# sailordiary/m3f.pytorch

Measured on AMD Instinct MI355X. Metric: clips/sec (300-frame A+V, fwd+bwd), higher is better.
Workload: dtype f32 (fp32-accurate products, fp32 accumulate: GEMMs as fp16x3 -- two fp16 terms per scaled operand, three MFMAs, error vs fp64 no larger than an fp32 GEMM's; the forward and backward recurrences at H=512 and H=256 as fp16x3 too (h is bounded; the backward producers split their values under a power-o

## Files before the change

### include/m3t_hip.h

```cpp
#ifndef M3T_HIP_H
#define M3T_HIP_H

#include <stddef.h>
#include <stdint.h>

#ifdef __cplusplus
extern "C" {
#endif

#define M3T_EINVAL 10001
#define M3T_MAX_SCANS 8
#define M3T_ESPIN 10002
#define M3T_SCAN_NO_PERSIST 1
#define M3T_SCAN_WHH 8
#define M3T_SCAN_FP32 4
#define M3T_SCAN_FAULT 16
#define M3T_SCAN_WIDE 32
#define M3T_BF16 2
#define M3T_GEMM_BACKGROUND 1
#define M3T_GEMM_BF16 2
#define M3T_GEMM_HIGH 256
#define M3T_GEMM_F16X3 1024
#define M3T_GEMM_BESIDE_SCAN 512
#define M3T_GEMM_EXCLUSIVE 8
#define M3T_CONV_IMAGES 4096

int m3t_im2col3d(const float* x, int N, int Ci, int T, int H, int W, int kt, int kh, int kw, int st, int sh, int sw,
                 int pt, int ph, int pw, float* out, long long rows_pad, int Kp, unsigned long long* amax_slot, void* stream);

int m3t_conv3d_taps(const float* src, const float* w_taps, float* dst, int N, int C_src, int C_dst, int T, int H, int W,
                    int To, int Ho, int Wo, int kt, int kh, int kw, int base_t, int base_h, int base_w, int sign, int flags,
                    const unsigned long long* amax_src, const unsigned long long* amax_w, float* ws, size_t ws_bytes, float* dst_planes,
                    void* stream);

int m3t_f16x3_split(const float* x, size_t rows, int cols, size_t ld, float* out, size_t ldo, const unsigned long long* slot, void* stream);
int m3t_f16x3_split_perm(const float* w, size_t R, int T, int Cc, size_t sR, size_t sT, size_t sC, float* out, const unsigned long long* slot,
                         void* stream);
int m3t_sgemm_pre(int M, int N, int K, const float* A_img, int lda, const float* B_img, int ldb, float* C, int ldc,
                  const float* bias, int act, int accumulate, const unsigned long long* amax_a, const unsigned long long* amax_b, void* stream);
int m3t_f16x3_image_b(const float* w, int N, int K, size_t ld, float* img, const unsigned long long* slot, void* stream);
int m3t_sgemm_bimg(int M, int N, int K, const float* A, int lda, const float* B_img, float* C, int ldc, const float* bias, int act,
                   int accumulate, float* ws, size_t ws_bytes, const unsigned long long* amax_a, const unsigned long long* amax_b, void* stream);
int m3t_sgemm_ring(int transA, int transB, int M, int N, int K, const float* A, int lda, const float* B, int ldb, float* C, int ldc,
                   const float* bias, int act, int accumulate, int seg_len, int seg_stride, int a_off, int b_off, float* ws, size_t ws_bytes,
                   int splits, const unsigned long long* amax_a, const unsigned long long* amax_b, int variant, void* stream);
int m3t_conv3d_taps_pre(const float* src_img, const float* w_img, float* dst, int N, int C_src, int C_dst, int T, int H, int W,
                        int To, int Ho, int Wo, int kt, int kh, int kw, int base_t, int base_h, int base_w, int sign,
                        const unsigned long long* amax_src, const unsigned long long* amax_w, float* ws, size_t ws_bytes, float* dst_planes,
                    void* stream);

int m3t_planes_to_cl4(const float* x, float* out, int N, int C, long long S, void* stream);
int m3t_conv3d_fwd_taps4(const float* x_img4, const float* w_img, const float* bias, float* y_cl, int N, int Co, int T, int H, int W,
                         int kt, int kh, int kw, int st, int sh, int sw, int pt, int ph, int pw, const unsigned long long* amax_x,
                         const unsigned long long* amax_w, float* ws, size_t ws_bytes, float* y_planes, void* stream);
int m3t_conv3d_fwd_taps(const float* x_img, const float* w_img, const float* bias, float* y_cl, int N, int Ci, int Co, int T, int H, int W,
                        int kt, int kh, int kw, int st, int sh, int sw, int pt, int ph, int pw, const unsigned long long* amax_x,
                        const unsigned long long* amax_w, float* ws, size_t ws_bytes, float* y_planes, void* stream);
int m3t_conv3d_wgrad_taps(const float* x_cl, const float* dy_cl, float* dwt, int N, int Ci, int Co, int T, int H, int W, int kt, int kh, int kw,
                          int st, int sh, int sw, int pt, int ph, int pw, int flags, const unsigned long long* amax_x,
                          const unsigned long long* amax_dy, float* ws, size_t ws_bytes, void* stream);

int m3t_amax_out(unsigned long long* slot);

int m3t_version(void);
int m3t_device_arch(char* arch, int cap);

int m3t_sgemm(int transA, int transB, int M, int N, int K,
              const float* A, int lda, const float* B, int ldb,
              float* C, int ldc, const float* bias, int act, int accumulate,
              int seg_len, int seg_stride, int a_off, int b_off,
              float* ws, size_t ws_bytes, int flags, void* stream);

int m3t_sgemm_scaled(int transA, int transB, int M, int N, int K,
                     const float* A, int lda, const float* B, int ldb,
                     float* C, int ldc, const float* bias, int act, int accumulate,
                     int seg_len, int seg_stride, int a_off, int b_off,
                     float* ws, size_t ws_bytes, int flags,
                     const unsigned long long* amax_a, const unsigned long long* amax_b, void* stream);

int m3t_sgemm_window(int transB, int n_seg, int win_len, int win_stride, int win_off, int N, int K,
                     const float* A, int lda, const float* B, int ldb, float* C, int ldc, const float* bias,
                     int act, int accumulate, int flags, const unsigned long long* amax_a, const unsigned long long* amax_b, void* stream);
#define M3T_WINDOW_BATCH 8
typedef struct {
    const float* A; const float* B; float* C; const float* bias;
    const unsigned long long* amax_a; const unsigned long long* amax_b;
    int accumulate;
} m3t_window_problem;
int m3t_sgemm_window_batch(int n, const m3t_window_problem* problems, int transB, int n_seg, int win_len, int win_stride, int win_off,
                           int N, int K, int lda, int ldb, int ldc, int act, int flags, void* stream);

int m3t_absmax(int n, const float* const* x, const size_t* rows, const int* cols, const size_t* ld,
               unsigned long long* const* slots, void* stream);

int m3t_sgemm_plan(int transA, int M, int N, int K, int seg_len, size_t ws_bytes, int flags, int* kernel, int* splits);

int m3t_colsum(const float* X, int M, int N, int ld, float* out, int accumulate,
               float* ws, size_t ws_bytes, void* stream);

int m3t_transpose(const float* src, int R, int C, int lds, float* dst, int ldd, void* stream);

int m3t_relu_bwd(const float* a, float* dy, size_t n, void* stream);

typedef struct {
    const float* xproj;
    const float* w_hh;
    const float* b_hh;
    float* out;
    float* gates;
    float* h_n;
    int H, reverse, ldx, xoff, ldo, ooff;
} m3t_gru_fwd_desc;

int m3t_gru_scan_fwd(const m3t_gru_fwd_desc* scans, int n_scans, int B, int T,
                     float* ws, size_t ws_bytes, int flags, void* stream);

typedef struct {
    const float* dout;
    const float* out;
    const float* gates;
    const float* w_hh_t;
    const float* dh_n;
    float* dgx;
    float* dgh;
    float* dh;
    float* db_part;
    float* db_ih;
    float* db_hh;
    int H, reverse, ldo, ooff, ldg, goff;
    unsigned long long* amax;
    const float* wfrag;
} m3t_gru_bwd_desc;

size_t m3t_gru_bwd_prepare_floats(int H);
int m3t_gru_bwd_prepare(const float* const* w, int n, int H, int whh_direct, float* const* out, void* stream);

int m3t_gru_scan_workgroups(int n_scans, int H, int B, int T, int flags, int backward);
int m3t_gru_persist_count(void);
int m3t_gru_poll_error(void);
int m3t_gru_error_reset(void);
int m3t_gru_error_defer(int on);
int m3t_gru_inject_error(void* stream);
int m3t_gru_persist_owner(void);
int m3t_gru_scan_arena(void* arena, size_t bytes);
int m3t_gru_scan_arena_reset(void* arena);
int m3t_gru_scan_progress(unsigned* counters, int n_marks, const int* time_bounds, unsigned* need);
int m3t_gru_scan_progress_reset(unsigned* counters);
int m3t_gru_scan_progress_ok(int n_scans, int H, int B, int T, int flags, int backward);
int m3t_stream_wait_progress(const unsigned* counter, unsigned need, void* stream);
int m3t_gru_scan_after(void* event);
int m3t_gru_scan_events(void* start, void* end);
int m3t_gru_persist_profile(unsigned long long* out6);

int m3t_gru_scan_bwd(const m3t_gru_bwd_desc* scans, int n_scans, int B, int T,
                     float* ws, size_t ws_bytes, int flags, void* stream);

int m3t_att_fuse_fwd(const float* s_v, const float* s_a, const float* x_v, const float* x_a,
                     float* f, int rows, int D, void* stream);
int m3t_att_fuse_bwd(const float* df, const float* s_v, const float* s_a,
                     const float* x_v, const float* x_a,
                     float* ds_v, float* ds_a, float* dx_v, float* dx_a,
                     int rows, int D, void* stream);

int m3t_va_loss(const float* y_hat, int rows, int C, int iv, int ia,
                const float* valence, const float* arousal,
                const int64_t* class_expr, const uint8_t* expr_valid, int n_expr,
                float w_v, float w_a, float expr_w, int use_mse,
                float* out_scalars, float* dy, float* ws, size_t ws_bytes, void* stream);
size_t m3t_va_loss_ws_bytes(int rows);

// ... 295 lines not shown
```

### m3f.pytorch_amd/csrc/gru_persist.hip

```cpp
#include "gru_common.h"
#include <cstdio>
#include <cstdlib>
#include <cstring>
#include <mutex>
#include <unordered_map>
#include <fcntl.h>
#include <sys/file.h>
#include <sys/stat.h>
#include <unistd.h>

namespace m3t_gru {

namespace {

constexpr int SPIN_LIMIT_DEFAULT = 1 << 21;
typedef unsigned u32x4 __attribute__((ext_vector_type(4)));

struct ExPtrs {
    void* gran[M3T_MAX_SCANS];
    size_t slot[M3T_MAX_SCANS];
    int poll_fixed;
    int poll_align;
    int spin_limit;
    int fault_step;
// ... 97 lines not shown
    constexpr int ROWS = 16 * RT;
    constexpr int NB = RT == 1 ? 2 : 1;
    constexpr int H = 128 * NC, nch = H >> 4;
    __shared__ float red[NB][NW][3][ROWS][UB + 1];
    const int tid = threadIdx.x, lane = tid & 63, wave = tid >> 6;
    int gid, ub;
    if (!persist_map((int)blockIdx.x, G, ex.slot_map, gid, ub)) return;
    const int s = gid / nrb, rb = gid % nrb;
    const m3t_gru_fwd_desc d = g.d[s];
    const int j0 = ub * UB, r0 = rb * ROWS;

    float4 wf[NC][3];
    {
        const float4* Wf = reinterpret_cast<const float4*>(fp.wfrag[s] + (size_t)ub * nch * 3 * 256);
#pragma unroll
        for (int m = 0; m < NC; ++m)
#pragma unroll
            for (int ct = 0; ct < 3; ++ct) wf[m][ct] = Wf[((size_t)(wave + m * NW) * 3 + ct) * 64 + lane];
    }
    const bool pw = tid < ROWS * UB;
    const int prow = (tid >> 8) * 16 + (tid & 15), pu = ((tid >> 4) & 3) * 4 + ((tid >> 6) & 3);
    const int pb = r0 + prow, pj = j0 + pu;
    const bool pok = pw && pb < B;
    float br = 0.f, bz = 0.f, bn = 0.f, hprev = 0.f;
    if (pw) { br = d.b_hh[pj]; bz = d.b_hh[H + pj]; bn = d.b_hh[2 * H + pj]; }

    constexpr size_t TILE = (size_t)RT * 256;
    unsigned long long* gran = reinterpret_cast<unsigned long long*>(ex.gran[s]);
    const size_t slot = ex.slot[s];
    const size_t grp = (size_t)rb * nch * TILE;
    const size_t pub = grp + (size_t)ub * TILE + tid;
    bool dead = false;
    int poll_delay = ex.poll_fixed >= 0 ? ex.poll_fixed : POLL_DELAY_INIT;
    __shared__ unsigned poll_fail[2];
    __shared__ int pub_step;
    const int l2mode = persist_handshake(ex, gid, ub, H >> 4, tid, err);
    if (tid == 0) pub_step = 0;
    if (tid < 2) poll_fail[tid] = 0;
    const bool stamp = ex.prof != nullptr && blockIdx.x == 0 && tid == ex.prof_tid;
    long long psum[6] = {0, 0, 0, 0, 0, 0}, last = stamp ? clock64() : 0;

    float xrA, xzA, xnA, xrB, xzB, xnB;
    const float* xq = d.xproj + (size_t)(pb < B ? pb : B - 1) * T * d.ldx + d.xoff + pj;
#define M3T_FWD_LOAD_X(step_, XR, XZ, XN)                                                                             \
    do {                                                                                                               \
        const int ls_ = (step_) < T ? (step_) : T - 1;                                                                 \
        const float* xa_ = xq + (size_t)(d.reverse ? T - 1 - ls_ : ls_) * d.ldx;                                       \
        asm volatile("global_load_dword %0, %3, off\n\t"                                                               \
                     "global_load_dword %1, %4, off\n\t"                                                               \
                     "global_load_dword %2, %5, off"                                                                   \
                     : "=&v"(XR), "=&v"(XZ), "=&v"(XN) : "v"(xa_), "v"(xa_ + H), "v"(xa_ + 2 * H) : "memory");         \
    } while (0)
    M3T_FWD_LOAD_X(0, xrA, xzA, xnA);
    asm volatile("s_waitcnt vmcnt(0)" : "+v"(xrA), "+v"(xzA), "+v"(xnA) :: "memory");
    __builtin_amdgcn_s_waitcnt(0x0F70);

    for (int step2 = 0; step2 < T; step2 += 2) {
#define STEPV step2
#define CUR(x) x##A
#define NXT(x) x##B
#include "gru_persist_fwd_step.inc"
#undef STEPV
#undef CUR
#undef NXT
        if (step2 + 1 >= T) break;
#define STEPV (step2 + 1)
#define CUR(x) x##B
#define NXT(x) x##A
#include "gru_persist_fwd_step.inc"
#undef STEPV
#undef CUR
#undef NXT
    }
#undef M3T_FWD_LOAD_X
    asm volatile("s_waitcnt vmcnt(0)" ::: "memory");
    if (stamp)
        for (int i = 0; i < 6; ++i) ex.prof[i] = (unsigned long long)psum[i];
}

typedef __bf16 pbf16x8 __attribute__((ext_vector_type(8)));
typedef unsigned pu32x4 __attribute__((ext_vector_type(4)));

__global__ void wfrag6_prep_kernel(const float* __restrict__ w_hh, unsigned short* __restrict__ wf, int H, int bf16) {
    const int nch = H >> 4, ks = nch >> 4;
    const size_t total = (size_t)3 * H * H;
    for (size_t i = blockIdx.x * (size_t)blockDim.x + threadIdx.x; i < total; i += (size_t)gridDim.x * blockDim.x) {
        const int e = i & 7, l = (i >> 3) & 63;
        size_t r = i >> 9;
        const int ct = r % 3; r /= 3;
        const int s = r % ks; r /= ks;
        const int w = r % NW, ub = r / NW;
        const int q = l >> 4;
        const int unit = 16 * (w + NW * (2 * s + (q >> 1))) + 8 * (q & 1) + e;
        float x = w_hh[((size_t)ct * H + ub * 16 + (l & 15)) * H + unit];
        if (bf16) x = rbf(x);
        const __bf16 b1 = (__bf16)x;
        const float r1 = x - (float)b1;
        const __bf16 b2 = (__bf16)r1;
        const __bf16 b3 = (__bf16)(r1 - (float)b2);
        const size_t base = ((((size_t)(ub * NW + w) * ks + s) * 3 + ct) * 3) * 512 + (size_t)l * 8 + e;
        wf[base] = __builtin_bit_cast(unsigned short, b1);
        wf[base + 512] = __builtin_bit_cast(unsigned short, b2);
        wf[base + 1024] = __builtin_bit_cast(unsigned short, b3);
    }
}

struct Prep3hArgs { const float* w_hh[M3T_MAX_SCANS]; unsigned short* wf[M3T_MAX_SCANS]; float* inv[M3T_MAX_SCANS]; };
constexpr int PREP3H_SPLIT = 8;
__global__ __launch_bounds__(256) void wfrag3h_prep_kernel(Prep3hArgs a, int H) {
    const float* __restrict__ w_hh = a.w_hh[blockIdx.z];
    unsigned short* __restrict__ wf = a.wf[blockIdx.z];
    const int ub = blockIdx.x, nch = H >> 4, ks = nch >> 4;
    __shared__ float red[4];
    float m = 0.f;
    const int h4 = H >> 2, tot4 = 48 * h4;
    auto ld = [&](int i) {
        const int rr = i / h4, c = i - rr * h4;
        return *reinterpret_cast<const float4*>(w_hh + ((size_t)(rr >> 4) * H + ub * 16 + (rr & 15)) * H + 4 * c);
    };
    auto fold = [&](const float4& v) {
        m = fmaxf(fmaxf(m, m3t_fin_abs(v.x)), fmaxf(m3t_fin_abs(v.y), fmaxf(m3t_fin_abs(v.z), m3t_fin_abs(v.w))));
    };
    int i = threadIdx.x;
    for (; i + 768 < tot4; i += 1024) {
        const float4 v0 = ld(i), v1 = ld(i + 256), v2 = ld(i + 512), v3 = ld(i + 768);
        fold(v0); fold(v1); fold(v2); fold(v3);
    }
    for (; i < tot4; i += 256) fold(ld(i));
    m = wave_max(m);
    if ((threadIdx.x & 63) == 0) red[threadIdx.x >> 6] = m;
    __syncthreads();
    m = fmaxf(fmaxf(red[0], red[1]), fmaxf(red[2], red[3]));
    float sc, inv;
    m3t_f16_scale(__float_as_uint(m), sc, inv);
    if (threadIdx.x == 0 && blockIdx.y == 0) a.inv[blockIdx.z][ub] = inv * 6.103515625e-05f;
    const int per = 3 * 16 * H;
    for (int j = blockIdx.y * 256 + threadIdx.x; j < per; j += 256 * PREP3H_SPLIT) {
        const int e = j & 7, l = (j >> 3) & 63;
        int r = j >> 9;
        const int ct = r % 3; r /= 3;
        const int s = r % ks; const int w = r / ks;
        const int q = l >> 4;
        const int unit = 16 * (w + NW * (2 * s + (q >> 1))) + 8 * (q & 1) + e;
        const float x = w_hh[((size_t)ct * H + ub * 16 + (l & 15)) * H + unit] * sc;
        const _Float16 h1 = (_Float16)x;
        const _Float16 h2 = (_Float16)(x - (float)h1);
        const size_t base = ((((size_t)(ub * NW + w) * ks + s) * 3 + ct) * 2) * 512 + (size_t)l * 8 + e;
        wf[base] = __builtin_bit_cast(unsigned short, h1);
        wf[base + 512] = __builtin_bit_cast(unsigned short, h2);
    }
}
typedef _Float16 pf16x8 __attribute__((ext_vector_type(8)));

template <int NC, bool F16 = false, int UW = 1>
__global__ __launch_bounds__(NT) void gru_persist_fwd6_kernel(FwdGroup g, FragPtrs fp, ExPtrs ex, int B, int T, int G, int nrb,
                                                              unsigned* err) {
    constexpr bool CO = UW == 2;
    constexpr int ROWS = 16, KS = NC / 2, NTERM = F16 ? 2 : 3;
    constexpr int H = 128 * NC, nch = H >> 4;
    constexpr int RED_FLOATS = 2 * NW * UW * 3 * ROWS * (UB + 1);
    __shared__ float red_s[UW == 1 ? RED_FLOATS : 1];
    extern __shared__ __attribute__((aligned(16))) float red_d[];
    float* const red = UW == 1 ? red_s : red_d;
#define M3T_RED(par_, w_, u_, ct_, r_, c_) red[(((((par_) * NW + (w_)) * UW + (u_)) * 3 + (ct_)) * ROWS + (r_)) * (UB + 1) + (c_)]
    const int tid = threadIdx.x, lane = tid & 63, wave = tid >> 6;
    int gid, ubw;
    if (!persist_map((int)blockIdx.x, G, ex.slot_map, gid, ubw)) return;
    const int s = gid / nrb, rb = gid % nrb;
    const m3t_gru_fwd_desc d = g.d[s];
    const int tu = UW == 1 ? 0 : (tid >> 8);
    const int ub = ubw * UW + tu;
    const int j0 = ub * UB, r0 = rb * ROWS;

    pbf16x8 wf[UW][KS][3][NTERM];
    float winv = 1.f;
    if (F16 && ex.inline_prep) {
        __shared__ float s_wmax[2][NW];
        const int q_ = lane >> 4;
        float mx[UW];
#pragma unroll
        for (int u = 0; u < UW; ++u) {
            mx[u] = 0.f;
#pragma unroll
            for (int k = 0; k < KS; ++k)
#pragma unroll
                for (int ct = 0; ct < 3; ++ct) {
                    const float4* wp = reinterpret_cast<const float4*>(d.w_hh + ((size_t)ct * H + (ubw * UW + u) * 16 + (lane & 15)) * H +
                                                                       16 * (wave + NW * (2 * k + (q_ >> 1))) + 8 * (q_ & 1));
                    const float4 a = wp[0], b = wp[1];
                    mx[u] = fmaxf(fmaxf(fmaxf(mx[u], m3t_fin_abs(a.x)), fmaxf(m3t_fin_abs(a.y), m3t_fin_abs(a.z))),
                                  fmaxf(fmaxf(m3t_fin_abs(a.w), m3t_fin_abs(b.x)), fmaxf(m3t_fin_abs(b.y), fmaxf(m3t_fin_abs(b.z), m3t_fin_abs(b.w)))));
                }
            mx[u] = wave_max(mx[u]);
            if (lane == 0) s_wmax[u][wave] = mx[u];
        }
        __syncthreads();
#pragma unroll
        for (int u = 0; u < UW; ++u) {
            float m = 0.f;
#pragma unroll
            for (int w = 0; w < NW; ++w) m = fmaxf(m, s_wmax[u][w]);
            float sc, inv;
            m3t_f16_scale(__float_as_uint(m), sc, inv);
            if (u == tu) winv = inv * 6.103515625e-05f;
#pragma unroll
            for (int k = 0; k < KS; ++k)
#pragma unroll
                for (int ct = 0; ct < 3; ++ct) {
                    const float4* wp = reinterpret_cast<const float4*>(d.w_hh + ((size_t)ct * H + (ubw * UW + u) * 16 + (lane & 15)) * H +
                                                                       16 * (wave + NW * (2 * k + (q_ >> 1))) + 8 * (q_ & 1));
                    const float4 a = wp[0], b = wp[1];
                    const float xv[8] = {a.x * sc, a.y * sc, a.z * sc, a.w * sc, b.x * sc, b.y * sc, b.z * sc, b.w * sc};
                    pf16x8 h1, h2;
#pragma unroll
                    for (int e = 0; e < 8; ++e) {
                        h1[e] = (_Float16)xv[e];
                        h2[e] = (_Float16)(xv[e] - (float)h1[e]);
                    }
                    wf[u][k][ct][0] = __builtin_bit_cast(pbf16x8, h1);
                    wf[u][k][ct][1] = __builtin_bit_cast(pbf16x8, h2);
                }
        }
    } else {
#pragma unroll
        for (int u = 0; u < UW; ++u) {
            const pu32x4* Wf = reinterpret_cast<const pu32x4*>(fp.wfrag[s]) + ((size_t)((ubw * UW + u) * NW + wave) * KS * 3 * NTERM) * 64 + lane;
#pragma unroll
            for (int k = 0; k < KS; ++k)
#pragma unroll
                for (int ct = 0; ct < 3; ++ct)
#pragma unroll
                    for (int t = 0; t < NTERM; ++t) wf[u][k][ct][t] = __builtin_bit_cast(pbf16x8, Wf[((k * 3 + ct) * NTERM + t) * 64]);
        }
        if (F16) winv = reinterpret_cast<const float*>(fp.wfrag[s])[(size_t)4 * H * H + ub];
    }
    const int ti = tid & 255;
    const bool pw = tid < ROWS * UB * UW;
    const int prow = (ti >> 1) & 15, pu = ((ti >> 5) & 1) * 8 + 2 * ((ti >> 6) & 3) + (ti & 1);
    const int pb = r0 + prow, pj = j0 + pu;
    const bool pok = pw && pb < B;
    float br = 0.f, bz = 0.f, bn = 0.f, hprev = 0.f;
    if (pw) { br = d.b_hh[pj]; bz = d.b_hh[H + pj]; bn = d.b_hh[2 * H + pj]; }

    constexpr size_t TILE = 256;
    unsigned long long* gran = reinterpret_cast<unsigned long long*>(ex.gran[s]);
    const size_t slot = ex.slot[s];
    const size_t grp = (size_t)rb * nch * TILE;
    const size_t pub = grp + (size_t)ubw * UW * TILE + tid;
    const int q = lane >> 4;
    const size_t lane_off = (size_t)(wave + NW * (q >> 1)) * TILE + 2 * ((q & 1) * 16 + (lane & 15));
    bool dead = false;
    int poll_delay = ex.poll_fixed >= 0 ? ex.poll_fixed : POLL_DELAY_INIT;
    __shared__ unsigned poll_fail[2];
    __shared__ int pub_step;
    const int l2mode = persist_handshake(ex, gid, ubw, (H >> 4) / UW, tid, err);
    if (tid == 0) pub_step = 0;
    if (tid < 2) poll_fail[tid] = 0;
    const bool stamp = ex.prof != nullptr && blockIdx.x == 0 && tid == ex.prof_tid;
    long long psum[6] = {0, 0, 0, 0, 0, 0}, last = stamp ? clock64() : 0;

    const bool MARK_ASC = !d.reverse;
    M3T_MARK_STATE();
    float xrA, xzA, xnA, xrB, xzB, xnB;
    const int hrow = CO ? (ti >> 4) : prow, hun = CO ? (ti & 15) : pu;
    const int hb = r0 + hrow, hj = j0 + hun;
    const bool hok = pw && hb < B;
    const int hg = 64 * ((hun >> 1) & 3) + 2 * (hrow + 16 * (hun >> 3)) + (hun & 1);
    constexpr int SLOTS = 272;
    const int slot_h = tu * SLOTS + hg + (hg >> 4), slot_c = tu * SLOTS + ti + (ti >> 4);
    f32x4* const sx = reinterpret_cast<f32x4*>(red_d + (UW == 1 ? 0 : RED_FLOATS));
    f32x4* const so = sx + 2 * UW * SLOTS;
    float* const sh = reinterpret_cast<float*>(so + 2 * UW * SLOTS);
    const float* xq = d.xproj + (size_t)(hb < B ? hb : B - 1) * T * d.ldx + d.xoff + hj;
    auto store_results = [&](int step_of, const f32x4& g4, float hv) {
        const int t_ = d.reverse ? T - 1 - step_of : step_of;
        d.out[((size_t)hb * T + t_) * d.ldo + d.ooff + hj] = hv;
        if (d.gates) *reinterpret_cast<f32x4*>(d.gates + ((size_t)hb * T + t_) * 4 * H + 4 * (size_t)hj) = g4;
        if (d.h_n && step_of == T - 1) d.h_n[(size_t)hb * H + hj] = hv;
    };
#define M3T_FWD_LOAD_X(step_, XR, XZ, XN)                                                                             \
    do {                                                                                                               \
        const int ls_ = (step_) < T ? (step_) : T - 1;                                                                 \
        const float* xa_ = xq + (size_t)(d.reverse ? T - 1 - ls_ : ls_) * d.ldx;                                       \
        asm volatile("global_load_dword %0, %3, off\n\t"                                                               \
                     "global_load_dword %1, %4, off\n\t"                                                               \
                     "global_load_dword %2, %5, off"                                                                   \
                     : "=&v"(XR), "=&v"(XZ), "=&v"(XN) : "v"(xa_), "v"(xa_ + H), "v"(xa_ + 2 * H) : "memory");         \
    } while (0)
    M3T_FWD_LOAD_X(0, xrA, xzA, xnA);
    asm volatile("s_waitcnt vmcnt(0)" : "+v"(xrA), "+v"(xzA), "+v"(xnA) :: "memory");
    __builtin_amdgcn_s_waitcnt(0x0F70);

    for (int step2 = 0; step2 < T; step2 += 2) {
#define STEPV step2
#define PARV 0
#define CUR(x) x##A
#define NXT(x) x##B
#include "gru_persist_fwd6_step.inc"
#undef STEPV
#undef PARV
#undef CUR
#undef NXT
        if (step2 + 1 >= T) break;
#define STEPV (step2 + 1)
#define PARV 1
#define CUR(x) x##B
#define NXT(x) x##A
#include "gru_persist_fwd6_step.inc"
#undef STEPV
#undef PARV
#undef CUR
#undef NXT
    }
#undef M3T_FWD_LOAD_X
#undef M3T_RED
    asm volatile("s_waitcnt vmcnt(0)" ::: "memory");
    if (CO) {
        __syncthreads();
        if (hok) store_results(T - 1, so[((T - 1) & 1) * UW * SLOTS + slot_h], sh[((T - 1) & 1) * UW * SLOTS + slot_h]);
    }
    if (stamp)
        for (int i = 0; i < 6; ++i) ex.prof[i] = (unsigned long long)psum[i];
}

__global__ void wfrag_bwd16_prep_kernel(const float* __restrict__ w_hh_t, unsigned short* __restrict__ wf, int H, int direct) {
    const int ks = H >> 8;
    const size_t total = (size_t)3 * H * H;
    for (size_t i = blockIdx.x * (size_t)blockDim.x + threadIdx.x; i < total; i += (size_t)gridDim.x * blockDim.x) {
        const int e = i & 7, l = (i >> 3) & 63;
        size_t r = i >> 9;
        const int gt = r % 3; r /= 3;
        const int sk = r % ks; r /= ks;
        const int w = r % NW, ub = r / NW;
        const int q = l >> 4;
        const int unit = 16 * (w + NW * (2 * sk + (q >> 1))) + 8 * (q & 1) + e;
        const float x = rbf(direct ? w_hh_t[((size_t)gt * H + unit) * H + ub * 16 + (l & 15)]
                                   : w_hh_t[((size_t)ub * 16 + (l & 15)) * 3 * H + (size_t)gt * H + unit]);
        wf[i] = (unsigned short)(__float_as_uint(x) >> 16);
    }
}

template <int NC>
__global__ __launch_bounds__(NT) void gru_persist_bwd16_kernel(BwdGroup g, FragPtrs fp, ExPtrs ex, int B, int T, int G, int nrb,
                                                             unsigned* err) {
    constexpr int ROWS = 16, RT = 1, KS = NC / 2;
    constexpr int H = 128 * NC, H3 = 3 * H, nchh = H >> 4;
    __shared__ float red[2][NW][ROWS][UB + 1];
    const int tid = threadIdx.x, lane = tid & 63, wave = tid >> 6;
    int gid, ub;
    if (!persist_map((int)blockIdx.x, G, ex.slot_map, gid, ub)) return;
    const int s = gid / nrb, rb = gid % nrb;
    const m3t_gru_bwd_desc d = g.d[s];
    const int j0 = ub * UB, r0 = rb * ROWS;

    pbf16x8 wb[KS][3];
    {
        const pu32x4* Wf = reinterpret_cast<const pu32x4*>(fp.wfrag[s]) + ((size_t)(ub * NW + wave) * KS * 3) * 64 + lane;
#pragma unroll
        for (int k = 0; k < KS; ++k)
#pragma unroll
            for (int gt = 0; gt < 3; ++gt) wb[k][gt] = __builtin_bit_cast(pbf16x8, Wf[(k * 3 + gt) * 64]);
    }
    const bool pw = tid < ROWS * UB;
    const int prow = (tid >> 1) & 15, pu = ((tid >> 5) & 1) * 8 + 2 * ((tid >> 6) & 3) + (tid & 1);
    const int pb = r0 + prow, pj = j0 + pu;
    const bool pok = pw && pb < B;
    float dh_carry = 0.f, z_next = 0.f;
    float sb_r = 0.f, sb_z = 0.f, sb_n = 0.f, sb_nr = 0.f;
    if (pok && d.dh_n) dh_carry = d.dh_n[(size_t)pb * H + pj];

    constexpr size_t TILE = (size_t)RT * 256;
    unsigned long long* gran = reinterpret_cast<unsigned long long*>(ex.gran[s]);
    const int q = lane >> 4;
    const size_t lane_off = (size_t)(wave + NW * (q >> 1)) * TILE + 2 * ((q & 1) * 16 + (lane & 15));
    const size_t slot = ex.slot[s];
    const size_t grp = (size_t)rb * nchh * TILE;
    const size_t pub = grp + (size_t)ub * TILE + tid;
    bool dead = false;
    int poll_delay = ex.poll_fixed >= 0 ? ex.poll_fixed : POLL_DELAY_INIT;
    __shared__ unsigned poll_fail[2];
    __shared__ int pub_step;
    const int l2mode = persist_handshake(ex, gid, ub, H >> 4, tid, err);
    if (tid == 0) pub_step = 0;
    if (tid < 2) poll_fail[tid] = 0;
    const bool stamp = ex.prof != nullptr && blockIdx.x == 0 && tid == ex.prof_tid;
    long long psum[6] = {0, 0, 0, 0, 0, 0}, last = stamp ? clock64() : 0;

    float doutA, hprevA, doutB, hprevB;
    f32x4 g4A, g4B;
    const int pbc = pb < B ? pb : B - 1;
    const float* pd0 = d.dout + (size_t)pbc * T * d.ldo + d.ooff + pj;
    const float* pg0 = d.gates + (size_t)pbc * T * 4 * H + 4 * (size_t)pj;
    const float* ph0 = d.out + (size_t)pbc * T * d.ldo + d.ooff + pj;
#define M3T_BWD_LOAD_STEP(step_, DOUT, G4, HPREV)                                                                     \
    do {                                                                                                               \
        const int ls_ = (step_) < T ? (step_) : T - 1;                                                                 \
        const int lt_ = d.reverse ? ls_ : T - 1 - ls_;                                                                 \
        const int ltp_ = ls_ < T - 1 ? (d.reverse ? lt_ + 1 : lt_ - 1) : lt_;                                          \
        asm volatile("global_load_dword %0, %3, off\n\t"                                                               \
                     "global_load_dwordx4 %1, %4, off\n\t"                                                             \
                     "global_load_dword %2, %5, off"                                                                   \
                     : "=&v"(DOUT), "=&v"(G4), "=&v"(HPREV)                                                            \
                     : "v"(pd0 + (size_t)lt_ * d.ldo), "v"(pg0 + (size_t)lt_ * 4 * H), "v"(ph0 + (size_t)ltp_ * d.ldo)  \
                     : "memory");                                                                                      \
    } while (0)
    M3T_BWD_LOAD_STEP(0, doutA, g4A, hprevA);
    asm volatile("s_waitcnt vmcnt(0)" : "+v"(doutA), "+v"(g4A), "+v"(hprevA) :: "memory");
    __builtin_amdgcn_s_waitcnt(0x0F70);
    float st_dr = 0.f, st_dz = 0.f, st_dn = 0.f, st_dnr = 0.f;
    auto store_results = [&](int step_of) {
        const int t = d.reverse ? step_of : T - 1 - step_of;
        float* gx = d.dgx + ((size_t)pb * T + t) * d.ldg + d.goff;
        gx[pj] = st_dr; gx[H + pj] = st_dz; gx[2 * H + pj] = st_dn;
        float* gh = d.dgh + ((size_t)pb * T + t) * H3;
        gh[pj] = st_dr; gh[H + pj] = st_dz; gh[2 * H + pj] = st_dnr;
    };

    for (int step2 = 0; step2 < T; step2 += 2) {
#define STEPV step2
// ... 191 lines not shown
    float sb_r = 0.f, sb_z = 0.f, sb_n = 0.f, sb_nr = 0.f;
    float amx = 0.f;
    if (pok && d.dh_n) dh_carry = d.dh_n[(size_t)pb * H + pj];

    constexpr size_t TILE = (size_t)RT * 256;
    u32x4* gran = reinterpret_cast<u32x4*>(ex.gran[s]);
    const size_t slot = ex.slot[s];
    const size_t grp = (size_t)rb * nchh * TILE;
    const size_t pub = grp + (size_t)ub * TILE + tid;
    bool dead = false;
    int poll_delay = ex.poll_fixed >= 0 ? ex.poll_fixed : POLL_DELAY_INIT;
    __shared__ unsigned poll_fail[2];
    __shared__ int pub_step;
    const int l2mode = persist_handshake(ex, gid, ub, H >> 4, tid, err);
    if (tid == 0) pub_step = 0;
    if (tid < 2) poll_fail[tid] = 0;
    const bool stamp = ex.prof != nullptr && blockIdx.x == 0 && tid == ex.prof_tid;
    long long psum[6] = {0, 0, 0, 0, 0, 0}, last = stamp ? clock64() : 0;

    float doutA, hprevA, doutB, hprevB;
    f32x4 g4A, g4B;
    const int pbc = pb < B ? pb : B - 1;
    const float* pd0 = d.dout + (size_t)pbc * T * d.ldo + d.ooff + pj;
    const float* pg0 = d.gates + (size_t)pbc * T * 4 * H + 4 * (size_t)pj;
    const float* ph0 = d.out + (size_t)pbc * T * d.ldo + d.ooff + pj;
#define M3T_BWD_LOAD_STEP(step_, DOUT, G4, HPREV)                                                                     \
    do {                                                                                                               \
        const int ls_ = (step_) < T ? (step_) : T - 1;                                                                 \
        const int lt_ = d.reverse ? ls_ : T - 1 - ls_;                                                                 \
        const int ltp_ = ls_ < T - 1 ? (d.reverse ? lt_ + 1 : lt_ - 1) : lt_;                                          \
        asm volatile("global_load_dword %0, %3, off\n\t"                                                               \
                     "global_load_dwordx4 %1, %4, off\n\t"                                                             \
                     "global_load_dword %2, %5, off"                                                                   \
                     : "=&v"(DOUT), "=&v"(G4), "=&v"(HPREV)                                                            \
                     : "v"(pd0 + (size_t)lt_ * d.ldo), "v"(pg0 + (size_t)lt_ * 4 * H), "v"(ph0 + (size_t)ltp_ * d.ldo)  \
                     : "memory");                                                                                      \
    } while (0)
    M3T_BWD_LOAD_STEP(0, doutA, g4A, hprevA);
    asm volatile("s_waitcnt vmcnt(0)" : "+v"(doutA), "+v"(g4A), "+v"(hprevA) :: "memory");
    __builtin_amdgcn_s_waitcnt(0x0F70);
    float st_dr = 0.f, st_dz = 0.f, st_dn = 0.f, st_dnr = 0.f;
    auto store_results = [&](int step_of) {
        const int t = d.reverse ? step_of : T - 1 - step_of;
        float* gx = d.dgx + ((size_t)pb * T + t) * d.ldg + d.goff;
        gx[pj] = st_dr; gx[H + pj] = st_dz; gx[2 * H + pj] = st_dn;
        float* gh = d.dgh + ((size_t)pb * T + t) * H3;
        gh[pj] = st_dr; gh[H + pj] = st_dz; gh[2 * H + pj] = st_dnr;
    };

    for (int step2 = 0; step2 < T; step2 += 2) {
#define STEPV step2
#define CUR(x) x##A
#define NXT(x) x##B
#include "gru_persist_bwd6_step.inc"
#undef STEPV
#undef CUR
#undef NXT
        if (step2 + 1 >= T) break;
#define STEPV (step2 + 1)
#define CUR(x) x##B
#define NXT(x) x##A
#include "gru_persist_bwd6_step.inc"
#undef STEPV
#undef CUR
#undef NXT
    }
#undef M3T_BWD_LOAD_STEP
    asm volatile("s_waitcnt vmcnt(0)" ::: "memory");
    if (pok) d.dh[(size_t)pb * H + pj] = dh_carry;
    if (pok && d.db_part) {
        float* q = d.db_part + (size_t)pb * 4 * H + pj;
        q[0] = sb_r; q[H] = sb_z; q[2 * H] = sb_n; q[3 * H] = sb_nr;
    }
    if (d.amax && pw) {
        const float m = wave_max(pok ? amx : 0.f);
        if (lane == 0) atomicMax(d.amax, (unsigned long long)__float_as_uint(m));
    }
    if (stamp)
        for (int i = 0; i < 6; ++i) ex.prof[i] = (unsigned long long)psum[i];
}

typedef unsigned pu32x2 __attribute__((ext_vector_type(2)));
typedef _Float16 pf16x4 __attribute__((ext_vector_type(4)));
struct PrepBwd3pArgs { const float* w[M3T_MAX_SCANS]; unsigned short* wf[M3T_MAX_SCANS]; float* inv[M3T_MAX_SCANS]; };
__device__ __forceinline__ unsigned wave_umax_dpp(unsigned v) {
    v = max(v, (unsigned)__builtin_amdgcn_update_dpp(0, (int)v, 0x111, 0xf, 0xf, false));
    v = max(v, (unsigned)__builtin_amdgcn_update_dpp(0, (int)v, 0x112, 0xf, 0xf, false));
    v = max(v, (unsigned)__builtin_amdgcn_update_dpp(0, (int)v, 0x114, 0xf, 0xf, false));
    v = max(v, (unsigned)__builtin_amdgcn_update_dpp(0, (int)v, 0x118, 0xf, 0xf, false));
    const unsigned a = (unsigned)__builtin_amdgcn_readlane((int)v, 15), b = (unsigned)__builtin_amdgcn_readlane((int)v, 31);
    const unsigned c = (unsigned)__builtin_amdgcn_readlane((int)v, 47), d = (unsigned)__builtin_amdgcn_readlane((int)v, 63);
    return max(max(a, b), max(c, d));
}
__device__ __forceinline__ unsigned bwd3p_split(float xs) {
    const _Float16 h1 = (_Float16)xs;
    const _Float16 h2 = (_Float16)(xs - (float)h1);
    return (unsigned)__builtin_bit_cast(unsigned short, h1) | ((unsigned)__builtin_bit_cast(unsigned short, h2) << 16);
}

__global__ __launch_bounds__(256) void wfrag_bwd3q_prep_kernel(PrepBwd3pArgs a, int H, int direct) {
    const float* __restrict__ w = a.w[blockIdx.z];
    unsigned short* __restrict__ wf = a.wf[blockIdx.z];
    const int ub = blockIdx.x, np = H >> 8;
    __shared__ float red[4];
    float m = 0.f;
    const int tot4 = 3 * H * 4;
    auto ld = [&](int i) {
        return direct ? *reinterpret_cast<const float4*>(w + (size_t)(i >> 2) * H + ub * 16 + 4 * (i & 3))
                      : *reinterpret_cast<const float4*>(w + ((size_t)ub * 16 + i / (3 * H / 4)) * 3 * H + 4 * (i % (3 * H / 4)));
    };
    auto fold = [&](const float4& v) {
        m = fmaxf(fmaxf(m, m3t_fin_abs(v.x)), fmaxf(m3t_fin_abs(v.y), fmaxf(m3t_fin_abs(v.z), m3t_fin_abs(v.w))));
    };
    int i0 = threadIdx.x;
    for (; i0 + 768 < tot4; i0 += 1024) {
        const float4 v0 = ld(i0), v1 = ld(i0 + 256), v2 = ld(i0 + 512), v3 = ld(i0 + 768);
        fold(v0); fold(v1); fold(v2); fold(v3);
    }
    for (; i0 < tot4; i0 += 256) fold(ld(i0));
    m = wave_max(m);
    if ((threadIdx.x & 63) == 0) red[threadIdx.x >> 6] = m;
    __syncthreads();
    m = fmaxf(fmaxf(red[0], red[1]), fmaxf(red[2], red[3]));
    float sc, inv;
    m3t_f16_scale(__float_as_uint(m), sc, inv);
    if (threadIdx.x == 0 && blockIdx.y == 0) a.inv[blockIdx.z][ub] = inv;
    const int items = 3 * np * NW * 64;
    for (int j = blockIdx.y * 256 + threadIdx.x; j < items; j += 256 * PREP3H_SPLIT) {
        const int l = j & 63;
        int r = j >> 6;
        const int pm = r % np; r /= np;
        const int wv = r % NW, gt = r / NW;
        const int unit0 = 32 * (wv + NW * pm) + 8 * (l >> 4), n = l & 15;
        unsigned h1[4], h2[4];
#pragma unroll
        for (int i = 0; i < 4; ++i) {
            unsigned short a1[2], a2[2];
#pragma unroll
            for (int k = 0; k < 2; ++k) {
                const float x = (direct ? w[((size_t)gt * H + unit0 + 2 * i + k) * H + ub * 16 + n]
                                        : w[((size_t)ub * 16 + n) * 3 * H + (size_t)gt * H + unit0 + 2 * i + k]) * sc;
                const _Float16 f1 = (_Float16)x;
                const _Float16 f2 = (_Float16)(x - (float)f1);
                a1[k] = __builtin_bit_cast(unsigned short, f1); a2[k] = __builtin_bit_cast(unsigned short, f2);
            }
            h1[i] = (unsigned)a1[0] | ((unsigned)a1[1] << 16); h2[i] = (unsigned)a2[0] | ((unsigned)a2[1] << 16);
        }
        const size_t base = (((((size_t)(ub * NW + wv) * 3 + gt) * np + pm) * 2) * 64 + l) * 8;
        *reinterpret_cast<uint4*>(wf + base) = make_uint4(h1[0], h1[1], h1[2], h1[3]);
        *reinterpret_cast<uint4*>(wf + base + 512) = make_uint4(h2[0], h2[1], h2[2], h2[3]);
    }
}

template <int NC, bool PROF = false>
__global__ __launch_bounds__(NT) void gru_persist_bwd3q_kernel(BwdGroup g, FragPtrs fp, ExPtrs ex, int B, int T, int G, int nrb,
                                                             unsigned* err) {
    constexpr int ROWS = 16, NP = NC / 2;
    constexpr int H = 128 * NC, H3 = 3 * H, nchh = H >> 4;
    __shared__ float red[2][NW][2][ROWS][UB + 1];
    const int tid = threadIdx.x, lane = tid & 63, wave = tid >> 6;
    int gid, ubw;
    if (!persist_map((int)blockIdx.x, G, ex.slot_map, gid, ubw)) return;
    const int s = gid / nrb, rb = gid % nrb;
    const m3t_gru_bwd_desc d = g.d[s];
    const int tu = tid >> 8;
    const int ub = ubw * 2 + tu;
    const int j0 = ub * UB, r0 = rb * ROWS;

    pu32x4 wb[2][3][NP][2];
    float winv[2];
#pragma unroll
    for (int u = 0; u < 2; ++u) {
        const pu32x4* Wf = reinterpret_cast<const pu32x4*>(fp.wfrag[s]) + ((size_t)((ubw * 2 + u) * NW + wave) * 3 * NP * 2) * 64 + lane;
#pragma unroll
        for (int gt = 0; gt < 3; ++gt)
#pragma unroll
            for (int m = 0; m < NP; ++m)
#pragma unroll
                for (int t = 0; t < 2; ++t) wb[u][gt][m][t] = Wf[((gt * NP + m) * 2 + t) * 64];
        winv[u] = reinterpret_cast<const float*>(fp.wfrag[s])[(size_t)4 * H * H + ubw * 2 + u];
    }
    __shared__ __attribute__((aligned(16))) unsigned pmx8[8];
    if (tid < 8) pmx8[tid] = 0u;
    const unsigned pmx8_addr = (unsigned)(uintptr_t)pmx8;
    const int ti = tid & 255;
    const int prow = ti & 15, pu = 8 * ((ti >> 4) & 1) + (ti >> 5);
    const int pb = r0 + prow, pj = j0 + pu;
    const bool pok = pb < B;
    float dh_carry = 0.f, z_next = 0.f;
    float sb_r = 0.f, sb_z = 0.f, sb_n = 0.f, sb_nr = 0.f;
    float amx = 0.f;
    if (pok && d.dh_n) dh_carry = d.dh_n[(size_t)pb * H + pj];

    constexpr size_t TILE = 256;
    u32x4* gran = reinterpret_cast<u32x4*>(ex.gran[s]);
    const size_t slot = ex.slot[s];
    const size_t grp = (size_t)rb * nchh * TILE;
    const size_t pub = grp + (size_t)ubw * 2 * TILE + tid;
    const size_t lane_src = (size_t)(2 * wave + (lane >> 5)) * TILE + ((lane >> 4) & 1) * 16 + (lane & 15);
    bool dead = false;
    int poll_delay = ex.poll_fixed >= 0 ? ex.poll_fixed : POLL_DELAY_INIT;
    __shared__ unsigned poll_fail[2];
    const int l2mode = persist_handshake(ex, gid, ubw, (H >> 4) / 2, tid, err);
    if (tid < 2) poll_fail[tid] = 0;
    const bool stamp = PROF && ex.prof != nullptr && blockIdx.x == 0 && tid == ex.prof_tid;
    long long psum[PROF ? 6 : 1] = {0}, last = stamp ? clock64() : 0;
    const bool MARK_ASC = d.reverse != 0;
    M3T_MARK_STATE();
    int amk = 0, amk_step = nmarks > 0 ? mark0 : -1;
#define M3T_QSTAMP(i)                                                        \
    do {                                                                     \
        if (PROF && stamp) { const long long now = clock64(); psum[PROF ? (i) : 0] += now - last; last = now; } \
    } while (0)

    float doutA, hprevA, doutB, hprevB;
    f32x4 g4A, g4B;
    const int hrow = ti >> 4, hun = ti & 15;
    const int hb = r0 + hrow, hj = j0 + hun;
    const bool hok = hb < B;
    const int hg = (hun & 7) * 32 + (hun >> 3) * 16 + hrow;
    constexpr int SLOTS = 272;
    const int slot_h = tu * SLOTS + hg + (hg >> 4), slot_c = tu * SLOTS + ti + (ti >> 4);
    extern __shared__ __attribute__((aligned(16))) unsigned char stage_raw[];
    f32x4* const sin4 = reinterpret_cast<f32x4*>(stage_raw);
    f32x4* const sout = sin4 + 2 * 2 * SLOTS;
    float2* const sin2 = reinterpret_cast<float2*>(sout + 2 * 2 * SLOTS);
    const int pbc = hb < B ? hb : B - 1;
    const float* pd0 = d.dout + (size_t)pbc * T * d.ldo + d.ooff + hj;
    const float* pg0 = d.gates + (size_t)pbc * T * 4 * H + 4 * (size_t)hj;
    const float* ph0 = d.out + (size_t)pbc * T * d.ldo + d.ooff + hj;
#define M3T_BWD_LOAD_STEP(step_, DOUT, G4, HPREV)                                                                     \
    do {                                                                                                               \
        const int ls_ = (step_) < T ? (step_) : T - 1;                                                                 \
        const int lt_ = d.reverse ? ls_ : T - 1 - ls_;                                                                 \
        const int ltp_ = ls_ < T - 1 ? (d.reverse ? lt_ + 1 : lt_ - 1) : lt_;                                          \
        asm volatile("global_load_dword %0, %3, off\n\t"                                                               \
                     "global_load_dwordx4 %1, %4, off\n\t"                                                             \
                     "global_load_dword %2, %5, off"                                                                   \
                     : "=&v"(DOUT), "=&v"(G4), "=&v"(HPREV)                                                            \
                     : "v"(pd0 + (size_t)lt_ * d.ldo), "v"(pg0 + (size_t)lt_ * 4 * H), "v"(ph0 + (size_t)ltp_ * d.ldo)  \
                     : "memory");                                                                                      \
    } while (0)
    M3T_BWD_LOAD_STEP(0, doutA, g4A, hprevA);
    asm volatile("s_waitcnt vmcnt(0)" : "+v"(doutA), "+v"(g4A), "+v"(hprevA) :: "memory");
    __builtin_amdgcn_s_waitcnt(0x0F70);
    float st_dr = 0.f, st_dz = 0.f, st_dn = 0.f, st_dnr = 0.f;
    auto store_results = [&](int step_of) {
        const int t = d.reverse ? step_of : T - 1 - step_of;
        float* gx = d.dgx + ((size_t)hb * T + t) * d.ldg + d.goff;
        gx[hj] = st_dr; gx[H + hj] = st_dz; gx[2 * H + hj] = st_dn;
        float* gh = d.dgh + ((size_t)hb * T + t) * H3;
        gh[hj] = st_dr; gh[H + hj] = st_dz; gh[2 * H + hj] = st_dnr;
    };

    for (int step2 = 0; step2 < T; step2 += 2) {
#define STEPV step2
#define PARV 0
#define CUR(x) x##A
#define NXT(x) x##B
#include "gru_persist_bwd3q_step.inc"
#undef STEPV
#undef PARV
#undef CUR
#undef NXT
        if (step2 + 1 >= T) break;
#define STEPV (step2 + 1)
#define PARV 1
#define CUR(x) x##B
#define NXT(x) x##A
#include "gru_persist_bwd3q_step.inc"
#undef STEPV
#undef PARV
#undef CUR
#undef NXT
    }
#undef M3T_BWD_LOAD_STEP
    asm volatile("s_waitcnt vmcnt(0)" ::: "memory");
    __syncthreads();
    if (hok) {
        const f32x4 r4 = sout[((T - 1) & 1) * 2 * SLOTS + slot_h];
        st_dr = r4[0]; st_dz = r4[1]; st_dn = r4[2]; st_dnr = r4[3];
        store_results(T - 1);
    }
    if (pok) d.dh[(size_t)pb * H + pj] = dh_carry;
    if (pok && d.db_part) {
        float* q = d.db_part + (size_t)pb * 4 * H + pj;
        q[0] = sb_r; q[H] = sb_z; q[2 * H] = sb_n; q[3 * H] = sb_nr;
    }
    if (d.amax) {
        const float m = wave_max(pok ? amx : 0.f);
        if (lane == 0) {
            atomicMax(d.amax, (unsigned long long)__float_as_uint(m));
            if (nmarks > 0) atomicMax(d.amax + 1 + amk, (unsigned long long)__float_as_uint(m));
        }
    }
    if (PROF && stamp)
        for (int i = 0; i < 6; ++i) ex.prof[i] = (unsigned long long)psum[PROF ? i : 0];
#undef M3T_QSTAMP
}

unsigned long long* g_prof = nullptr;
int g_launches = 0;
unsigned* g_err_host = nullptr;
unsigned* g_err_dev = nullptr;

bool ensure_err_word() {
    if (g_err_host) return true;
    void* h = nullptr;
    if (hipHostMalloc(&h, 64, hipHostMallocMapped) != hipSuccess) { (void)hipGetLastError(); return false; }
    std::memset(h, 0, 64);
    void* dptr = nullptr;
    if (hipHostGetDevicePointer(&dptr, h, 0) != hipSuccess) { (void)hipGetLastError(); (void)hipHostFree(h); return false; }
    g_err_host = static_cast<unsigned*>(h);
    g_err_dev = static_cast<unsigned*>(dptr);
    return true;
}

int device_cus() {
    static int cus = -1;
    if (cus < 0) {
        int dev = 0;
        hipDeviceProp_t prop;
        if (hipGetDevice(&dev) != hipSuccess || hipGetDeviceProperties(&prop, dev) != hipSuccess) { (void)hipGetLastError(); cus = 0; }
        else cus = prop.multiProcessorCount;
    }
    return cus;
}

template <typename K>
int resident_capacity(K kernel) {
    int occ = 0;
    if (hipOccupancyMaxActiveBlocksPerMultiprocessor(&occ, kernel, NT, 0) != hipSuccess) { (void)hipGetLastError(); return 0; }
    const int per_cu = occ >= 3 ? 2 : (occ >= 1 ? 1 : 0);
    return per_cu * device_cus();
}

static int poll_env_early(const char* name, int dflt) {
    const char* e = std::getenv(name);
    return e ? atoi(e) : dflt;
}

struct Shape { int nc, rt, G, nrb, grid, active, slot_map; };

template <typename D>
bool level_shape(const D* d, int n, int B, Shape& sh, int uw = 1) {
    const int maxh = d[0].H;
    if (maxh % 128 != 0 || maxh > 512) return false;
    for (int i = 1; i < n; ++i)
        if (d[i].H != maxh) return false;
    sh.nc = maxh / 128;
    sh.rt = 0;
    for (int rt = 1; rt <= 2; ++rt) {
        if (uw > 1 && rt > 1) break;
        const int members = maxh / 16 / uw;
        const int nrb = cdiv(B, 16 * rt), G = n * nrb, active = G * members;
        if (active <= device_cus()) {
#ifndef M3T_SCAN_L2_MODE
#define M3T_SCAN_L2_MODE 2
#endif
            constexpr int l2 = M3T_SCAN_L2_MODE;
            sh.rt = rt; sh.nrb = nrb; sh.G = G; sh.active = active;
            sh.slot_map = (l2 == 1 || (l2 == 2 && G % 8 == 0) || (uw > 1 && G <= 8)) ? 1 : 0;
            sh.grid = sh.slot_map ? 8 * cdiv(G, 8) * members : active;
            break;
        }
    }
    return sh.rt != 0;
}

typedef void (*FwdKernel)(FwdGroup, FragPtrs, ExPtrs, int, int, int, int, unsigned*);
typedef void (*BwdKernel)(BwdGroup, FragPtrs, ExPtrs, int, int, int, int, unsigned*);

FwdKernel pick_fwd(const Shape& sh) {
    static const FwdKernel k[2][4] = {
        {gru_persist_fwd_kernel<1, 1>, gru_persist_fwd_kernel<2, 1>, gru_persist_fwd_kernel<3, 1>, gru_persist_fwd_kernel<4, 1>},
        {gru_persist_fwd_kernel<1, 2>, gru_persist_fwd_kernel<2, 2>, gru_persist_fwd_kernel<3, 2>, gru_persist_fwd_kernel<4, 2>}};
    return k[sh.rt - 1][sh.nc - 1];
}
BwdKernel pick_bwd(const Shape& sh) {
    static const BwdKernel k[2][4] = {
        {gru_persist_bwd_kernel<1, 1>, gru_persist_bwd_kernel<2, 1>, gru_persist_bwd_kernel<3, 1>, gru_persist_bwd_kernel<4, 1>},
        {gru_persist_bwd_kernel<1, 2>, gru_persist_bwd_kernel<2, 2>, gru_persist_bwd_kernel<3, 2>, gru_persist_bwd_kernel<4, 2>}};
    return k[sh.rt - 1][sh.nc - 1];
}


template <typename K>
static size_t exclusive_lds(K kernel, int grid, size_t need = 0) {
    if (grid > 192 && need == 0) return 0;
    hipFuncAttributes a;
    if (hipFuncGetAttributes(&a, reinterpret_cast<const void*>(kernel)) != hipSuccess) { (void)hipGetLastError(); return 0; }
    const size_t want = (size_t)152 * 1024;
    if (a.sharedSizeBytes >= want && need == 0) return 0;
    size_t dyn = grid > 192 ? need : (want > a.sharedSizeBytes ? want - a.sharedSizeBytes : 0);
    if (dyn < need) dyn = need;
    if (hipFuncSetAttribute(reinterpret_cast<const void*>(kernel), hipFuncAttributeMaxDynamicSharedMemorySize, (int)dyn) != hipSuccess) {
        (void)hipGetLastError();
        return 0;
    }
    return dyn;
}

constexpr size_t ARENA_OFF[4] = {0, (size_t)2 << 20, (size_t)3 << 20, (size_t)4 << 20};
constexpr size_t ARENA_SIZE[4] = {(size_t)2 << 20, (size_t)1 << 20, (size_t)1 << 20, (size_t)4 << 20};
constexpr size_t ARENA_HS_OFF = (size_t)8 << 20, ARENA_HS_SIZE = (size_t)64 << 10;
constexpr size_t ARENA_BYTES = ARENA_HS_OFF + ARENA_HS_SIZE;
struct ArenaState { unsigned long long next[5]; int fmt[4]; bool known; };
std::mutex g_arena_mu;
std::unordered_map<uintptr_t, ArenaState> g_arenas;
thread_local void* g_arena = nullptr;
thread_local size_t g_arena_bytes = 0;

template <typename G>
int prepare_exchange(const G& g, const FragPtrs& fp, const Shape& sh, int kind, size_t gran_bytes, unsigned long long tag_max,
                     int T, ExPtrs& ex, hipStream_t s, int fmt = 0) {
    size_t bytes[M3T_MAX_SCANS], total = 0;
    for (int i = 0; i < g.n; ++i) {
        ex.slot[i] = (size_t)sh.nrb * (g.d[i].H / 16) * sh.rt * 256;
        bytes[i] = 2 * ex.slot[i] * gran_bytes;
        total += bytes[i];
    }
    ex.tag_base = 0;
    void* arena = g_arena;
    const size_t arena_bytes = g_arena_bytes;
    g_arena = nullptr; g_arena_bytes = 0;
    if (arena && arena_bytes >= ARENA_BYTES && ((uintptr_t)arena % 16) == 0 && total <= ARENA_SIZE[kind] &&
        (unsigned long long)T + 1 < tag_max) {
        char* base = static_cast<char*>(arena) + ARENA_OFF[kind];
        size_t off = 0;
        for (int i = 0; i < g.n; ++i) { ex.gran[i] = base + off; off += bytes[i]; }
        std::lock_guard<std::mutex> lock(g_arena_mu);
        ArenaState& st = g_arenas[(uintptr_t)arena];
        if (!st.known) {
            const hipError_t e = hipMemsetAsync(arena, 0, ARENA_BYTES, s);
            if (e != hipSuccess) return (int)e;
            st.known = true;
            for (int q = 0; q < 5; ++q) st.next[q] = 0;
            for (int q = 0; q < 4; ++q) st.fmt[q] = 0;
        }
        if (st.fmt[kind] != fmt) {
            const hipError_t e = hipMemsetAsync(base, 0, ARENA_SIZE[kind], s);
            if (e != hipSuccess) return (int)e;
            st.next[kind] = 0;
            st.fmt[kind] = fmt;
        }
        if (st.next[kind] + (unsigned long long)T + 1 >= tag_max) {
            const hipError_t e = hipMemsetAsync(base, 0, ARENA_SIZE[kind], s);
            if (e != hipSuccess) return (int)e;
            st.next[kind] = 0;
        }
        ex.tag_base = (unsigned)st.next[kind];
        st.next[kind] += (unsigned long long)T;
        if (sh.slot_map && (size_t)sh.G * HS_STRIDE * 8 <= ARENA_HS_SIZE) {
            if (st.next[4] + 2 >= 0xffffffffull) {
                const hipError_t e = hipMemsetAsync(static_cast<char*>(arena) + ARENA_HS_OFF, 0, ARENA_HS_SIZE, s);
                if (e != hipSuccess) return (int)e;
                st.next[4] = 0;
            }
            ex.hs = reinterpret_cast<unsigned long long*>(static_cast<char*>(arena) + ARENA_HS_OFF);
            ex.hs_tag = (unsigned)(++st.next[4]);
        }
        return 0;
    }
    for (int i = 0; i < g.n; ++i) {
        ex.gran[i] = fp.xfrag[i];
        const hipError_t e = hipMemsetAsync(ex.gran[i], 0, bytes[i], s);
        if (e != hipSuccess) return (int)e;
    }
    return 0;
}

template <typename G>
void fill_exchange(const G& g, const FragPtrs& fp, const Shape& sh, size_t gran_bytes, ExPtrs& ex, size_t (&bytes)[M3T_MAX_SCANS]) {
    std::memset(&ex, 0, sizeof(ex));
    static int prof_on = -1;
    if (prof_on < 0) {
        const char* e = std::getenv("M3T_SCAN_PROF");
        prof_on = (e && (e[0] == '1' || e[0] == '2')) ? (e[0] - '0') : 0;
        if (prof_on && hipMalloc(reinterpret_cast<void**>(&g_prof), 64) != hipSuccess) { (void)hipGetLastError(); g_prof = nullptr; }
    }
    ex.prof = g_prof;
    ex.prof_tid = prof_on == 2 ? 256 : 0;
    ex.poll_fixed = -1;
    ex.poll_align = 0;
    static const int spin_limit = poll_env_early("M3T_SCAN_SPIN_LIMIT", SPIN_LIMIT_DEFAULT);
    ex.spin_limit = spin_limit > 0 ? spin_limit : SPIN_LIMIT_DEFAULT;
    ex.fault_step = -1;
    ex.slot_map = sh.slot_map;
    for (int i = 0; i < g.n; ++i) bytes[i] = 0;
}

}

bool persist_enabled() {
    static int on = -1;
    if (on < 0) {
        const char* e = std::getenv("M3T_SCAN_PERSIST");
        on = (e && e[0] == '0') ? 0 : 1;
    }
    return on == 1;
}

int persist_poll_error() {
    if (!g_err_host) return 0;
    if (__atomic_load_n(g_err_host + 1, __ATOMIC_RELAXED) == 0u) return 0;
    const unsigned step1 = __atomic_load_n(g_err_host, __ATOMIC_RELAXED);
    return (int)(step1 ? step1 : 1u);
}

static int g_defer = 0;
void persist_set_defer(int on) { g_defer = on ? 1 : 0; }
bool persist_deferred() { return g_defer != 0; }

void persist_reset_error() {
// ... 51 lines not shown
    struct stat st;
    if (fstat(fd, &st) != 0 || !S_ISREG(st.st_mode) || st.st_uid != geteuid()) { close(fd); state[dev] = 1; return true; }
    if (flock(fd, LOCK_EX | LOCK_NB) == 0) { state[dev] = 1; return true; }
    close(fd);
    state[dev] = 2;
    std::fprintf(stderr, "m3t: another process owns the persistent GRU scans of GPU %s (%s); this process uses the "
                         "launch-per-step scans (several times slower; m3t_gru_persist_owner() == 2)\n", bus, path);
    return false;
}

int persist_owner_state() {
    int dev = 0;
    if (hipGetDevice(&dev) != hipSuccess) { (void)hipGetLastError(); return 0; }
    return (dev >= 0 && dev < 64) ? g_owner_state[dev] : 0;
}

size_t persist_exchange_bytes(int H, int B, bool backward) {
    const size_t rows = (size_t)cdiv(B, 32) * 32;
    return 2 * rows * (size_t)H * (backward ? 16 : 8);
}

static bool x6_scan_enabled() {
    static int on = -1;
    if (on < 0) {
        const char* e = std::getenv("M3T_SCAN_X6");
        on = (e && e[0] == '0') ? 0 : 1;
    }
    return on == 1;
}

bool persist_fwd_uses_x6(const FwdGroup& g, int B, int T, int flags) {
    Shape sh;
    if ((flags & M3T_SCAN_FP32) || !x6_scan_enabled() || T >= 65535 || !level_shape(g.d, g.n, B, sh)) return false;
    return sh.rt == 1 && (sh.nc == 2 || sh.nc == 4);
}

bool persist_fwd_check(const FwdGroup& g, int B, int T) {
    Shape sh;
    return persist_enabled() && T >= 2 && level_shape(g.d, g.n, B, sh) && ensure_err_word() &&
           sh.active <= resident_capacity(pick_fwd(sh)) && persist_owner();
}

bool persist_bwd_check(const BwdGroup& g, int B, int T) {
    Shape sh;
    return persist_enabled() && T >= 2 && level_shape(g.d, g.n, B, sh) && ensure_err_word() &&
           sh.active <= resident_capacity(pick_bwd(sh)) && persist_owner();
}

bool persist_bwd_uses_16(const BwdGroup& g, int B, int T, int flags) {
    Shape sh;
    if (!g.bf16 || (flags & M3T_SCAN_FP32) || !x6_scan_enabled() || T >= 65535 || !level_shape(g.d, g.n, B, sh)) return false;
    return sh.rt == 1 && (sh.nc == 2 || sh.nc == 4);
}

bool persist_bwd_uses_x6(const BwdGroup& g, int B, int T, int flags) {
    Shape sh;
    if (g.bf16 || (flags & M3T_SCAN_FP32) || !x6_scan_enabled() || !level_shape(g.d, g.n, B, sh)) return false;
    return sh.rt == 1 && (sh.nc == 2 || sh.nc == 4);
}

struct ProgressArm { unsigned* ctr; int n; int tb[3]; unsigned* need; };
static thread_local ProgressArm g_prog = {nullptr, 0, {0, 0, 0}, nullptr};
struct ProgressPending { unsigned* ctr; unsigned up, down; };
static thread_local ProgressPending g_prog_pending = {nullptr, 0, 0};
struct ProgressTxn { void commit(); ~ProgressTxn(); };
static std::mutex g_prog_mu;
static std::unordered_map<uintptr_t, std::pair<unsigned, unsigned>> g_prog_total;
void persist_set_progress(unsigned* ctr, int n, const int* tb, unsigned* need) {
    g_prog.ctr = ctr; g_prog.n = n; g_prog.need = need;
    for (int i = 0; i < 3; ++i) g_prog.tb[i] = (tb && i < n) ? tb[i] : 0;
}
void persist_drop_progress() { g_prog.ctr = nullptr; g_prog.n = 0; g_prog.need = nullptr; }
bool persist_progress_armed() { return g_prog.ctr != nullptr; }
void persist_forget_progress(unsigned* ctr) {
    std::lock_guard<std::mutex> lock(g_prog_mu);
    if (ctr) g_prog_total.erase((uintptr_t)ctr); else g_prog_total.clear();
}
template <typename G>
static int apply_progress(const G& g, const bool* up, int wg_per_scan, int T, ExPtrs& ex) {
    if (!g_prog.ctr) return 0;
    const ProgressArm a = g_prog;
    persist_drop_progress();
    if (a.n < 1 || a.n > 3 || !a.need) return M3T_EINVAL;
    for (int k = 0; k < a.n; ++k)
        if (a.tb[k] < 4 || a.tb[k] > T - 4 || (k > 0 && a.tb[k] < a.tb[k - 1] + 4)) return M3T_EINVAL;
    int n_up = 0, n_down = 0;
    for (int i = 0; i < g.n; ++i) (up[i] ? n_up : n_down) += 1;
    ex.prog = a.ctr; ex.nmarks = a.n;
    for (int k = 0; k < a.n; ++k) { ex.marks[0][k] = a.tb[k]; ex.marks[1][k] = T - a.tb[a.n - 1 - k]; }
    std::lock_guard<std::mutex> lock(g_prog_mu);
    std::pair<unsigned, unsigned>& tot = g_prog_total[(uintptr_t)a.ctr];
    for (int k = 0; k < a.n; ++k) {
        a.need[k] = tot.first + (unsigned)(n_up * wg_per_scan * (k + 1));
        a.need[a.n + k] = tot.second + (unsigned)(n_down * wg_per_scan * (k + 1));
    }
    g_prog_pending.ctr = a.ctr;
    g_prog_pending.up = (unsigned)(n_up * wg_per_scan * a.n);
    g_prog_pending.down = (unsigned)(n_down * wg_per_scan * a.n);
    return 0;
}
void ProgressTxn::commit() {
    if (!g_prog_pending.ctr) return;
    std::lock_guard<std::mutex> lock(g_prog_mu);
    std::pair<unsigned, unsigned>& tot = g_prog_total[(uintptr_t)g_prog_pending.ctr];
    tot.first += g_prog_pending.up; tot.second += g_prog_pending.down;
    g_prog_pending.ctr = nullptr;
}
ProgressTxn::~ProgressTxn() { g_prog_pending.ctr = nullptr; }

int persist_bwd_prepare(const float* const* w, int n, int H, int direct, float* const* out, hipStream_t s) {
    if (n <= 0) return 0;
    if (n > M3T_MAX_SCANS || !w || !out || H <= 0 || H % 256 != 0 || H > 512) return M3T_EINVAL;
    PrepBwd3pArgs pa;
    for (int i = 0; i < M3T_MAX_SCANS; ++i) {
        const int j = i < n ? i : 0;
        if (!w[j] || !out[j] || ((uintptr_t)out[j] % 16) != 0) return M3T_EINVAL;
        pa.w[i] = w[j]; pa.wf[i] = reinterpret_cast<unsigned short*>(out[j]); pa.inv[i] = out[j] + (size_t)4 * H * H;
    }
    wfrag_bwd3q_prep_kernel<<<dim3(H / 16, PREP3H_SPLIT, n), 256, 0, s>>>(pa, H, direct ? 1 : 0);
    M3T_LAUNCH_CHECK();
    return 0;
}

__global__ void progress_gate_kernel(const unsigned* ctr, unsigned need, int spin_limit, unsigned* err) {
    if (threadIdx.x != 0) return;
    for (int spins = 0;; ++spins) {
        unsigned v;
        asm volatile("global_load_dword %0, %1, off sc1\n\ts_waitcnt vmcnt(0)" : "=v"(v) : "v"(ctr) : "memory");
        if ((int)(v - need) >= 0) return;
        if (spins > spin_limit) { raise_spin(err, 0); return; }
        __builtin_amdgcn_s_sleep(32);
    }
}
int persist_wait_progress(const unsigned* ctr, unsigned need, hipStream_t s) {
    if (!ctr || !ensure_err_word()) return M3T_EINVAL;
    static const int spin_limit = poll_env_early("M3T_SCAN_SPIN_LIMIT", SPIN_LIMIT_DEFAULT);
    progress_gate_kernel<<<1, 64, 0, s>>>(ctr, need, spin_limit > 0 ? spin_limit : SPIN_LIMIT_DEFAULT, g_err_dev);
    M3T_LAUNCH_CHECK();
    return 0;
}

static bool wide_enabled() {
    static int on = -1;
    if (on < 0) { const char* e = getenv("M3T_SCAN_WIDE"); on = (e && e[0] == '0') ? 0 : 1; }
    return on == 1;
}
static bool fwd_is_f16(const FwdGroup& g, int B, int T, int flags) {
    return persist_fwd_uses_x6(g, B, T, flags) && !g.bf16 && (flags & M3T_GEMM_F16X3) && m3t_f16x3_enabled();
}
static int fwd_uw(const FwdGroup& g, int B, int T, int flags, const Shape& sh) {
    return ((flags & M3T_SCAN_WIDE) && fwd_is_f16(g, B, T, flags) && (sh.nc == 4 || sh.nc == 2) && sh.rt == 1 && wide_enabled()) ? 2 : 1;
}

static int persist_fwd_launch_impl(const FwdGroup& g, const FragPtrs& fp, int B, int T, int flags, hipStream_t s);
int persist_fwd_launch(const FwdGroup& g, const FragPtrs& fp, int B, int T, int flags, hipStream_t s) {
    ProgressTxn txn;
    const int rc = persist_fwd_launch_impl(g, fp, B, T, flags, s);
    if (rc == 0) txn.commit();
    return rc;
}
static int persist_fwd_launch_impl(const FwdGroup& g, const FragPtrs& fp, int B, int T, int flags, hipStream_t s) {
    Shape sh;
    if (!level_shape(g.d, g.n, B, sh) || !ensure_err_word()) return M3T_EINVAL;
    const int uw = fwd_uw(g, B, T, flags, sh);
    if (uw > 1 && !level_shape(g.d, g.n, B, sh, uw)) return M3T_EINVAL;
    {
        if (uw == 1 && !sh.slot_map && sh.G < 8 && fwd_is_f16(g, B, T, flags)) {
            sh.slot_map = 1;
            sh.grid = 8 * (g.d[0].H / 16);
        }
    }
    ExPtrs ex;
    size_t bytes[M3T_MAX_SCANS];
    fill_exchange(g, fp, sh, 8, ex, bytes);
    if (flags & M3T_SCAN_FAULT) ex.fault_step = T / 2;
    {
        ex.poll_fixed = persist_fwd_uses_x6(g, B, T, flags) ? -1 : (sh.nc == 1 ? 0 : 12);
        ex.poll_align = persist_fwd_uses_x6(g, B, T, flags) ? 0 : 1;
        if (persist_fwd_uses_x6(g, B, T, flags) && !g.bf16 && (flags & M3T_GEMM_F16X3) && m3t_f16x3_enabled() && sh.nc == 2) ex.poll_align = 1;
    }
    const bool x6 = persist_fwd_uses_x6(g, B, T, flags);
    if (persist_progress_armed()) {
        if (!fwd_is_f16(g, B, T, flags)) { persist_drop_progress(); return M3T_EINVAL; }
        bool up[M3T_MAX_SCANS];
        for (int i = 0; i < g.n; ++i) up[i] = !g.d[i].reverse;
        const int e = apply_progress(g, up, sh.active / g.n, T, ex);
        if (e) return e;
    }
    { const int e = prepare_exchange(g, fp, sh, x6 ? 1 : 0, 8, x6 ? 65535ull : 0xffffffffull, T, ex, s); if (e) return e; }
    ++g_launches;
    if (!x6) { const int e = persist_take_after(s); if (e) return e; }
    if (x6) {
        const bool f16 = !g.bf16 && (flags & M3T_GEMM_F16X3) && m3t_f16x3_enabled();
        bool inline_ok = f16;
        for (int i = 0; i < g.n; ++i) inline_ok = inline_ok && ((uintptr_t)g.d[i].w_hh % 16) == 0;
        ex.inline_prep = inline_ok ? 1 : 0;
        if (f16 && !inline_ok) {
            Prep3hArgs pa;
            const int H = g.d[0].H;
            for (int i = 0; i < g.n; ++i) {
                pa.w_hh[i] = g.d[i].w_hh; pa.wf[i] = reinterpret_cast<unsigned short*>(fp.wfrag[i]); pa.inv[i] = fp.wfrag[i] + (size_t)4 * H * H;
            }
            for (int i = g.n; i < M3T_MAX_SCANS; ++i) { pa.w_hh[i] = pa.w_hh[0]; pa.wf[i] = pa.wf[0]; pa.inv[i] = pa.inv[0]; }
            wfrag3h_prep_kernel<<<dim3(H / 16, PREP3H_SPLIT, g.n), 256, 0, s>>>(pa, H);
        }
        for (int i = 0; i < g.n && !f16; ++i) {
            const int H = g.d[i].H;
            int blk = (3 * H * H + 255) / 256;
            if (blk > 1024) blk = 1024;
            wfrag6_prep_kernel<<<blk, 256, 0, s>>>(g.d[i].w_hh, reinterpret_cast<unsigned short*>(fp.wfrag[i]), H, g.bf16);
        }
        M3T_LAUNCH_CHECK();
        { const int e = persist_take_after(s); if (e) return e; }
        persist_record_start(s);
        if (f16) {
            if (uw == 2) {
                const size_t need = (size_t)2 * NW * 2 * 3 * 16 * (UB + 1) * sizeof(float)
                                    + (size_t)2 * 2 * 272 * 36;
                const FwdKernel kk = sh.nc == 2 ? gru_persist_fwd6_kernel<2, true, 2> : gru_persist_fwd6_kernel<4, true, 2>;
                const size_t dyn = exclusive_lds(kk, sh.active, need);
                if (dyn < need) return M3T_EINVAL;
                hipLaunchKernelGGL(kk, dim3(sh.grid), dim3(NT), dyn, s, g, fp, ex, B, T, sh.G, sh.nrb, g_err_dev);
            }
            else if (sh.nc == 2) hipLaunchKernelGGL((gru_persist_fwd6_kernel<2, true>), dim3(sh.grid), dim3(NT), exclusive_lds(gru_persist_fwd6_kernel<2, true>, sh.active), s, g, fp, ex, B, T, sh.G, sh.nrb, g_err_dev);
            else hipLaunchKernelGGL((gru_persist_fwd6_kernel<4, true>), dim3(sh.grid), dim3(NT), exclusive_lds(gru_persist_fwd6_kernel<4, true>, sh.active), s, g, fp, ex, B, T, sh.G, sh.nrb, g_err_dev);
        }
        else if (sh.nc == 2) hipLaunchKernelGGL(gru_persist_fwd6_kernel<2>, dim3(sh.grid), dim3(NT), exclusive_lds(gru_persist_fwd6_kernel<2>, sh.active), s, g, fp, ex, B, T, sh.G, sh.nrb, g_err_dev);
        else hipLaunchKernelGGL(gru_persist_fwd6_kernel<4>, dim3(sh.grid), dim3(NT), exclusive_lds(gru_persist_fwd6_kernel<4>, sh.active), s, g, fp, ex, B, T, sh.G, sh.nrb, g_err_dev);
        persist_record_end(s);
        M3T_LAUNCH_CHECK();
        return 0;
    }
    persist_record_start(s);
    hipLaunchKernelGGL(pick_fwd(sh), dim3(sh.grid), dim3(NT), exclusive_lds(pick_fwd(sh), sh.active), s, g, fp, ex, B, T, sh.G, sh.nrb, g_err_dev);
    persist_record_end(s);
    M3T_LAUNCH_CHECK();
    return 0;
}

static bool bwd3p_enabled() {
    static int on = -1;
    if (on < 0) { const char* e = getenv("M3T_SCAN_BWD3P"); on = (e && e[0] == '0') ? 0 : 1; }
    return on == 1;
}

static int persist_bwd_launch_impl(const BwdGroup& g, const FragPtrs& fp, int B, int T, int flags, hipStream_t s);
int persist_bwd_launch(const BwdGroup& g, const FragPtrs& fp, int B, int T, int flags, hipStream_t s) {
    ProgressTxn txn;
    const int rc = persist_bwd_launch_impl(g, fp, B, T, flags, s);
    if (rc == 0) txn.commit();
    return rc;
}
static int persist_bwd_launch_impl(const BwdGroup& g, const FragPtrs& fp, int B, int T, int flags, hipStream_t s) {
    Shape sh;
    if (!level_shape(g.d, g.n, B, sh) || !ensure_err_word()) return M3T_EINVAL;
    ExPtrs ex;
    size_t bytes[M3T_MAX_SCANS];
    const bool b16 = persist_bwd_uses_16(g, B, T, flags);
    fill_exchange(g, fp, sh, b16 ? 8 : 16, ex, bytes);
    if (flags & M3T_SCAN_FAULT) ex.fault_step = T / 2;
    {
        ex.poll_fixed = 12;
        ex.poll_align = 1;
    }
    const bool wide256 = (flags & M3T_SCAN_WIDE) && sh.rt == 1 && wide_enabled();
    const bool p3 = !b16 && persist_bwd_uses_x6(g, B, T, flags) && (flags & M3T_GEMM_F16X3) && m3t_f16x3_enabled() && bwd3p_enabled() &&
                    wide256 && (sh.nc == 4 || sh.nc == 2) && (unsigned long long)T + 1 < 0xffffffull;
    const int uw = p3 ? 2 : 1;
    if (uw > 1) {
        if (!level_shape(g.d, g.n, B, sh, uw)) return M3T_EINVAL;
        ex.slot_map = sh.slot_map;
    }
    if (persist_progress_armed()) {
        if (!(p3 && uw == 2)) { persist_drop_progress(); return M3T_EINVAL; }
        bool up[M3T_MAX_SCANS];
        for (int i = 0; i < g.n; ++i) up[i] = g.d[i].reverse != 0;
        const int e = apply_progress(g, up, sh.active / g.n, T, ex);
        if (e) return e;
    }
    { const int e = prepare_exchange(g, fp, sh, b16 ? 2 : 3, b16 ? 8 : 16, b16 ? 65535ull : (p3 ? 0xffffffull : 0xffffffffull), T, ex, s, p3 ? 1 : 0); if (e) return e; }
    ++g_launches;
    if (p3) {
        PrepBwd3pArgs pa;
        const int H = g.d[0].H;
        for (int i = 0; i < M3T_MAX_SCANS; ++i) {
            const int j = i < g.n ? i : 0;
            pa.w[i] = g.d[j].w_hh_t; pa.wf[i] = reinterpret_cast<unsigned short*>(fp.wfrag[j]); pa.inv[i] = fp.wfrag[j] + (size_t)4 * H * H;
        }
        if (uw == 2) {
            bool ready = true;
            for (int i = 0; i < g.n; ++i) ready = ready && g.d[i].wfrag != nullptr && ((uintptr_t)g.d[i].wfrag % 16) == 0;
            FragPtrs fq = fp;
            if (ready) {
                for (int i = 0; i < g.n; ++i) fq.wfrag[i] = const_cast<float*>(g.d[i].wfrag);
            } else {
                wfrag_bwd3q_prep_kernel<<<dim3(H / 16, PREP3H_SPLIT, g.n), 256, 0, s>>>(pa, H, (flags & M3T_SCAN_WHH) ? 1 : 0);
                M3T_LAUNCH_CHECK();
            }
            { const int e = persist_take_after(s); if (e) return e; }
            persist_record_start(s);
            const BwdKernel kq = sh.nc == 2 ? gru_persist_bwd3q_kernel<2> : (ex.prof ? gru_persist_bwd3q_kernel<4, true> : gru_persist_bwd3q_kernel<4>);
            const size_t need = (size_t)2 * 2 * 272 * 40;
            const size_t dyn = exclusive_lds(kq, sh.active, need);
            if (dyn < need) return M3T_EINVAL;
            hipLaunchKernelGGL(kq, dim3(sh.grid), dim3(NT), dyn, s, g, fq, ex, B, T, sh.G, sh.nrb, g_err_dev);
            persist_record_end(s);
            M3T_LAUNCH_CHECK();
            return 0;
        }
        return M3T_EINVAL;
    }
    if (b16) {
        for (int i = 0; i < g.n; ++i) {
            const int H = g.d[i].H;
            int blk = (3 * H * H + 255) / 256;
            if (blk > 1024) blk = 1024;
            wfrag_bwd16_prep_kernel<<<blk, 256, 0, s>>>(g.d[i].w_hh_t, reinterpret_cast<unsigned short*>(fp.wfrag[i]), H, (flags & M3T_SCAN_WHH) ? 1 : 0);
        }
        M3T_LAUNCH_CHECK();
        { const int e = persist_take_after(s); if (e) return e; }
        persist_record_start(s);
        if (sh.nc == 2) hipLaunchKernelGGL(gru_persist_bwd16_kernel<2>, dim3(sh.grid), dim3(NT), exclusive_lds(gru_persist_bwd16_kernel<2>, sh.active), s, g, fp, ex, B, T, sh.G, sh.nrb, g_err_dev);
        else hipLaunchKernelGGL(gru_persist_bwd16_kernel<4>, dim3(sh.grid), dim3(NT), exclusive_lds(gru_persist_bwd16_kernel<4>, sh.active), s, g, fp, ex, B, T, sh.G, sh.nrb, g_err_dev);
        persist_record_end(s);
        M3T_LAUNCH_CHECK();
        return 0;
    }
    if (persist_bwd_uses_x6(g, B, T, flags)) {
        {
            PrepBwd6Args pa;
            const int H = g.d[0].H;
            for (int i = 0; i < M3T_MAX_SCANS; ++i) {
                const int j = i < g.n ? i : 0;
                pa.w[i] = g.d[j].w_hh_t; pa.wf[i] = reinterpret_cast<unsigned short*>(fp.wfrag[j]);
            }
            int blk = (3 * H * H + 255) / 256;
            if (blk > 1024) blk = 1024;
            wfrag_bwd6_prep_kernel<<<dim3(blk, g.n), 256, 0, s>>>(pa, H, (flags & M3T_SCAN_WHH) ? 1 : 0);
        }
        M3T_LAUNCH_CHECK();
        { const int e = persist_take_after(s); if (e) return e; }
        persist_record_start(s);
        const BwdKernel kk = sh.nc == 2 ? gru_persist_bwd6_kernel<2> : gru_persist_bwd6_kernel<4>;
        hipLaunchKernelGGL(kk, dim3(sh.grid), dim3(NT), exclusive_lds(kk, sh.active), s, g, fp, ex, B, T, sh.G, sh.nrb, g_err_dev);
        persist_record_end(s);
        M3T_LAUNCH_CHECK();
        return 0;
    }
    { const int e = persist_take_after(s); if (e) return e; }
    persist_record_start(s);
    hipLaunchKernelGGL(pick_bwd(sh), dim3(sh.grid), dim3(NT), exclusive_lds(pick_bwd(sh), sh.active), s, g, fp, ex, B, T, sh.G, sh.nrb, g_err_dev);
    persist_record_end(s);
    M3T_LAUNCH_CHECK();
    return 0;
}

static thread_local hipEvent_t g_ev_start = nullptr, g_ev_end = nullptr;
void persist_set_events(hipEvent_t a, hipEvent_t b) { g_ev_start = a; g_ev_end = b; }
void persist_drop_events() { g_ev_start = g_ev_end = nullptr; }
void persist_record_start(hipStream_t s) { if (g_ev_start) { (void)hipEventRecord(g_ev_start, s); g_ev_start = nullptr; } }
void persist_record_end(hipStream_t s) { if (g_ev_end) { (void)hipEventRecord(g_ev_end, s); g_ev_end = nullptr; } }

static thread_local hipEvent_t g_after = nullptr;
void persist_set_after(hipEvent_t ev) { g_after = ev; }
void persist_drop_after() { g_after = nullptr; }
int persist_take_after(hipStream_t s) {
    if (!g_after) return 0;
    const hipError_t e = hipStreamWaitEvent(s, g_after, 0);
    g_after = nullptr;
    return (int)e;
}

void persist_set_arena(void* arena, size_t bytes) { g_arena = arena; g_arena_bytes = bytes; }
void persist_drop_arena() { g_arena = nullptr; g_arena_bytes = 0; }
void persist_forget_arena(void* arena) {
    std::lock_guard<std::mutex> lock(g_arena_mu);
    if (arena) g_arenas.erase((uintptr_t)arena); else g_arenas.clear();
}

int persist_launch_count() { return g_launches; }
void persist_count_launch() { ++g_launches; }

int persist_profile(unsigned long long* out6) {
    if (!g_prof || !out6) return M3T_EINVAL;
    return (int)hipMemcpy(out6, g_prof, 6 * sizeof(unsigned long long), hipMemcpyDeviceToHost);
}

}

extern "C" int m3t_gru_persist_count(void) { return m3t_gru::persist_launch_count(); }

namespace m3t_gru {
int persist_workgroups(int n, int H, int B, int T, int flags, bool backward) {
    if (n < 1 || n > M3T_MAX_SCANS || H < 1 || B < 1 || T < 2 || (flags & M3T_SCAN_NO_PERSIST) || !persist_enabled()) return 0;
    Shape sh;
    if (backward) {
        BwdGroup g;
        std::memset(&g, 0, sizeof(g));
        g.n = n; g.bf16 = (flags & M3T_BF16) ? 1 : 0;
        for (int i = 0; i < n; ++i) { g.d[i].H = H; g.d[i].gates = reinterpret_cast<const float*>(16); g.d[i].w_hh_t = reinterpret_cast<const float*>(16); }
        if (solo_bwd_ok(g, B, T, flags) || !level_shape(g.d, g.n, B, sh)) return 0;
        const bool b16 = persist_bwd_uses_16(g, B, T, flags);
        const bool wide256 = (flags & M3T_SCAN_WIDE) && sh.rt == 1 && wide_enabled();
        const bool p3 = !b16 && persist_bwd_uses_x6(g, B, T, flags) && (flags & M3T_GEMM_F16X3) && m3t_f16x3_enabled() && bwd3p_enabled() &&
                        wide256 && (sh.nc == 4 || sh.nc == 2) && (unsigned long long)T + 1 < 0xffffffull;
        if (p3 && !level_shape(g.d, g.n, B, sh, 2)) return 0;
        return sh.active;
    }
    FwdGroup g;
    std::memset(&g, 0, sizeof(g));
    g.n = n; g.bf16 = (flags & M3T_BF16) ? 1 : 0;
    for (int i = 0; i < n; ++i) { g.d[i].H = H; g.d[i].w_hh = reinterpret_cast<const float*>(16); }
    if (solo_fwd_ok(g, B, T, flags) || !level_shape(g.d, g.n, B, sh)) return 0;
    if (fwd_uw(g, B, T, flags, sh) == 2 && !level_shape(g.d, g.n, B, sh, 2)) return 0;
    return sh.active;
}
}

namespace m3t_gru {
int persist_progress_ok(int n, int H, int B, int T, int flags, bool backward) {
    if (persist_workgroups(n, H, B, T, flags, backward) <= 0) return 0;
    Shape sh;
    if (backward) {
        BwdGroup g;
        std::memset(&g, 0, sizeof(g));
        g.n = n; g.bf16 = (flags & M3T_BF16) ? 1 : 0;
        for (int i = 0; i < n; ++i) { g.d[i].H = H; g.d[i].gates = reinterpret_cast<const float*>(16); g.d[i].w_hh_t = reinterpret_cast<const float*>(16); }
        if (!level_shape(g.d, g.n, B, sh)) return 0;
        const bool b16 = persist_bwd_uses_16(g, B, T, flags);
        const bool wide256 = (flags & M3T_SCAN_WIDE) && sh.rt == 1 && wide_enabled();
        const bool p3 = !b16 && persist_bwd_uses_x6(g, B, T, flags) && (flags & M3T_GEMM_F16X3) && m3t_f16x3_enabled() && bwd3p_enabled() &&
                        wide256 && (sh.nc == 4 || sh.nc == 2) && (unsigned long long)T + 1 < 0xffffffull;
        return p3 ? 1 : 0;
    }
    FwdGroup g;
    std::memset(&g, 0, sizeof(g));
    g.n = n; g.bf16 = (flags & M3T_BF16) ? 1 : 0;
    for (int i = 0; i < n; ++i) { g.d[i].H = H; g.d[i].w_hh = reinterpret_cast<const float*>(16); }
    return fwd_is_f16(g, B, T, flags) ? 1 : 0;
}
}

extern "C" int m3t_gru_scan_workgroups(int n_scans, int H, int B, int T, int flags, int backward) {
    return m3t_gru::persist_workgroups(n_scans, H, B, T, flags, backward != 0);
}

extern "C" int m3t_gru_poll_error(void) { return m3t_gru::persist_poll_error(); }

extern "C" int m3t_gru_error_reset(void) { m3t_gru::persist_reset_error(); return 0; }

extern "C" int m3t_gru_error_defer(int on) { m3t_gru::persist_set_defer(on); return 0; }

extern "C" int m3t_gru_inject_error(void* stream) { return m3t_gru::persist_inject_error((hipStream_t)stream); }

extern "C" int m3t_gru_persist_owner(void) { return m3t_gru::persist_owner_state(); }

extern "C" int m3t_gru_scan_events(void* start, void* end) {
    m3t_gru::persist_set_events((hipEvent_t)start, (hipEvent_t)end);
    return 0;
}

extern "C" int m3t_gru_scan_arena(void* arena, size_t bytes) {
    m3t_gru::persist_set_arena(arena, bytes);
    return 0;
}

extern "C" int m3t_gru_scan_arena_reset(void* arena) {
    m3t_gru::persist_forget_arena(arena);
    return 0;
}

extern "C" int m3t_gru_scan_progress(unsigned* counters, int n_marks, const int* time_bounds, unsigned* need) {
    if (!counters) { m3t_gru::persist_drop_progress(); return 0; }
    if (n_marks < 1 || n_marks > 3 || !time_bounds || !need || ((uintptr_t)counters % 8) != 0) return M3T_EINVAL;
    m3t_gru::persist_set_progress(counters, n_marks, time_bounds, need);
    return 0;
}

extern "C" int m3t_gru_scan_progress_reset(unsigned* counters) {
    m3t_gru::persist_forget_progress(counters);
    return 0;
}

extern "C" int m3t_gru_scan_progress_ok(int n_scans, int H, int B, int T, int flags, int backward) {
    return m3t_gru::persist_progress_ok(n_scans, H, B, T, flags, backward != 0);
}

extern "C" int m3t_stream_wait_progress(const unsigned* counter, unsigned need, void* stream) {
    return m3t_gru::persist_wait_progress(counter, need, (hipStream_t)stream);
}

extern "C" size_t m3t_gru_bwd_prepare_floats(int H) { return H > 0 ? (size_t)4 * H * H + 64 : 0; }

extern "C" int m3t_gru_bwd_prepare(const float* const* w, int n, int H, int whh_direct, float* const* out, void* stream) {
    return m3t_gru::persist_bwd_prepare(w, n, H, whh_direct, out, (hipStream_t)stream);
}

extern "C" int m3t_gru_scan_after(void* event) {
    m3t_gru::persist_set_after((hipEvent_t)event);
    return 0;
}

extern "C" int m3t_gru_persist_profile(unsigned long long* out6) {
    return m3t_gru::persist_profile(out6);
}
```

### m3f.pytorch_amd/csrc/gru_persist_bwd3q_step.inc

```
{
    const int step = STEPV;
    const bool has_next = step > 0;
    M3T_QSTAMP(0);
    M3T_MARK_STEP_TOP(step);
    if (has_next) {
        const unsigned tag = (ex.tag_base + (unsigned)step) & 0xffffffu;
        const u32x4* src = gran + (size_t)(1 - PARV) * slot + grp + lane_src;
        u32x4 v[NP][8];
        int spins = 0;
        for (int z = 0; z < poll_delay; ++z) __builtin_amdgcn_s_sleep(1);
        for (;;) {
#pragma unroll
            for (int m = 0; m < NP; ++m) {
                const u32x4* q = src + (size_t)m * NW * 2 * TILE;
                asm volatile("global_load_dwordx4 %0, %8, off sc1\n\t"
                             "global_load_dwordx4 %1, %8, off offset:512 sc1\n\t"
                             "global_load_dwordx4 %2, %8, off offset:1024 sc1\n\t"
                             "global_load_dwordx4 %3, %8, off offset:1536 sc1\n\t"
                             "global_load_dwordx4 %4, %8, off offset:2048 sc1\n\t"
                             "global_load_dwordx4 %5, %8, off offset:2560 sc1\n\t"
                             "global_load_dwordx4 %6, %8, off offset:3072 sc1\n\t"
                             "global_load_dwordx4 %7, %8, off offset:3584 sc1"
                             : "=&v"(v[m][0]), "=&v"(v[m][1]), "=&v"(v[m][2]), "=&v"(v[m][3]),
                               "=&v"(v[m][4]), "=&v"(v[m][5]), "=&v"(v[m][6]), "=&v"(v[m][7])
                             : "v"(q) : "memory");
            }
            asm volatile("s_waitcnt vmcnt(0)" ::: "memory");
            bool ok = true;
#pragma unroll
            for (int m = 0; m < NP; ++m)
#pragma unroll
                for (int e = 0; e < 8; ++e) {
                    asm volatile("" : "+v"(v[m][e]));
                    ok = ok && ((v[m][e].w & 0xffffffu) == tag);
                }
            if (__all(ok) || dead) break;
            if (++spins > ex.spin_limit) { dead = true; if (lane == 0) raise_spin(err, step); break; }
            __builtin_amdgcn_s_sleep(1);
        }
        if (spins > 0 && lane == 0) atomicOr(&poll_fail[PARV], 1u);
        M3T_QSTAMP(1);
        f32x4 acc[2];
        acc[0] = acc[1] = (f32x4){0.f, 0.f, 0.f, 0.f};
#pragma unroll
        for (int m = 0; m < NP; ++m) {
            f32x4 at[2];
            at[0] = at[1] = (f32x4){0.f, 0.f, 0.f, 0.f};
#pragma unroll
            for (int gt = 0; gt < 3; ++gt) {
                pu32x4 ah, al;
#pragma unroll
                for (int i = 0; i < 4; ++i) {
                    ah[i] = __builtin_amdgcn_perm(v[m][2 * i + 1][gt], v[m][2 * i][gt], 0x05040100u);
                    al[i] = __builtin_amdgcn_perm(v[m][2 * i + 1][gt], v[m][2 * i][gt], 0x07060302u);
                }
                const pf16x8 AH = __builtin_bit_cast(pf16x8, ah), AL = __builtin_bit_cast(pf16x8, al);
#pragma unroll
                for (int u = 0; u < 2; ++u) {
                    at[u] = __builtin_amdgcn_mfma_f32_16x16x32_f16(AL, __builtin_bit_cast(pf16x8, wb[u][gt][m][0]), at[u], 0, 0, 0);
                    at[u] = __builtin_amdgcn_mfma_f32_16x16x32_f16(AH, __builtin_bit_cast(pf16x8, wb[u][gt][m][1]), at[u], 0, 0, 0);
                    at[u] = __builtin_amdgcn_mfma_f32_16x16x32_f16(AH, __builtin_bit_cast(pf16x8, wb[u][gt][m][0]), at[u], 0, 0, 0);
                }
                __builtin_amdgcn_sched_barrier(0);
            }
            const float pinv = __uint_as_float((254u - (v[m][0].w >> 24)) << 23);
#pragma unroll
            for (int u = 0; u < 2; ++u)
#pragma unroll
                for (int r = 0; r < 4; ++r) acc[u][r] = fmaf(at[u][r], pinv, acc[u][r]);
        }
#pragma unroll
        for (int u = 0; u < 2; ++u)
#pragma unroll
            for (int r = 0; r < 4; ++r) red[PARV][wave][u][(lane >> 4) * 4 + r][lane & 15] = acc[u][r] * winv[u];
    }
    asm volatile("s_waitcnt vmcnt(0)" ::: "memory");
    asm volatile("" : "+v"(CUR(dout)), "+v"(CUR(g4)), "+v"(CUR(hprev)));
    sin4[PARV * 2 * SLOTS + slot_h] = CUR(g4);
    sin2[PARV * 2 * SLOTS + slot_h] = make_float2(CUR(dout), CUR(hprev));
    M3T_BWD_LOAD_STEP(step + 1, NXT(dout), NXT(g4), NXT(hprev));
    M3T_QSTAMP(2);
    __syncthreads();
    M3T_MARK_AFTER_BARRIER(step);
    if (ex.poll_fixed < 0) {
        const bool wg_failed = poll_fail[PARV] != 0;
        if (tid == 0) poll_fail[(1 - PARV)] = 0;
        poll_delay = wg_failed ? min(poll_delay + 2, POLL_DELAY_MAX) : ((step & 7) == 0 && poll_delay > 0 ? poll_delay - 1 : poll_delay);
    }
    M3T_QSTAMP(3);
    {
        float mm = 0.f;
        if (has_next) {
#pragma unroll
            for (int w = 0; w < NW; ++w) mm += red[PARV][w][tu][prow][pu];
        }
        const f32x4 c_g4 = sin4[PARV * 2 * SLOTS + slot_c];
        const float2 dh2 = sin2[PARV * 2 * SLOTS + slot_c];
        const float c_dout = dh2.x, c_hprev = dh2.y;
        const float gr = c_g4[0], gz = c_g4[1], gn = c_g4[2], ghn = c_g4[3];
        const float carry0 = has_next ? fmaf(dh_carry, z_next, mm) : dh_carry;
        const float bnd = pok ? m3t_fin_abs((c_dout + carry0) * fmaxf(1.f, 0.25f * fabsf(ghn))) : 0.f;
        unsigned mxb = wave_umax_dpp(__float_as_uint(bnd));
        const unsigned want = (unsigned)(step + 1) & 3u;
        if (lane == 0) __hip_atomic_store(&pmx8[wave], (mxb & ~3u) | want, __ATOMIC_RELAXED, __HIP_MEMORY_SCOPE_WORKGROUP);
        const GateBwd c = gru_cell_bwd(c_dout, dh_carry, z_next, mm, has_next, gr, gz, gn, ghn, step < T - 1 ? c_hprev : 0.f);
        const float p0 = pok ? c.dr : 0.f, p1 = pok ? c.dz : 0.f, p2 = pok ? c.dnr : 0.f;
        {
            int w = 0;
            for (;;) {
                u32x4 qa, qb;
                asm volatile("ds_read_b128 %0, %2\n\tds_read_b128 %1, %2 offset:16\n\ts_waitcnt lgkmcnt(0)" : "=&v"(qa), "=&v"(qb) : "v"(pmx8_addr) : "memory");
                const bool all8 = ((qa.x & 3u) == want) && ((qa.y & 3u) == want) && ((qa.z & 3u) == want) && ((qa.w & 3u) == want) &&
                                  ((qb.x & 3u) == want) && ((qb.y & 3u) == want) && ((qb.z & 3u) == want) && ((qb.w & 3u) == want);
                if (all8 || dead) {
                    mxb = max(max(max(qa.x, qa.y), max(qa.z, qa.w)), max(max(qb.x, qb.y), max(qb.z, qb.w)));
                    break;
                }
                if (++w > ex.spin_limit) { dead = true; if (lane == 0) raise_spin(err, step); break; }
            }
        }
        float psc, pisc;
        m3t_f16_scale(mxb, psc, pisc);
        if (step + 1 < T && !(step == ex.fault_step && blockIdx.x == 0)) {
            u32x4 gq;
            gq.x = bwd3p_split(p0 * psc); gq.y = bwd3p_split(p1 * psc); gq.z = bwd3p_split(p2 * psc);
            gq.w = ((ex.tag_base + (unsigned)step + 1u) & 0xffffffu) | ((__float_as_uint(psc) >> 23) << 24);
            u32x4* q = gran + (size_t)PARV * slot + pub;
            if (l2mode) asm volatile("global_store_dwordx4 %0, %1, off" :: "v"(q), "v"(gq) : "memory");
            else asm volatile("global_store_dwordx4 %0, %1, off sc1" :: "v"(q), "v"(gq) : "memory");
        }
        M3T_QSTAMP(4);
        dh_carry = c.dht; z_next = gz;
        sb_r += c.dr; sb_z += c.dz; sb_n += c.dn; sb_nr += c.dnr;
        if (step == amk_step) {
            if (d.amax) {
                const float m_ = wave_max(pok ? amx : 0.f);
                if (lane == 0) {
                    atomicMax(d.amax + 1 + amk, (unsigned long long)__float_as_uint(m_));
                    atomicMax(d.amax, (unsigned long long)__float_as_uint(m_));
                }
            }
            amx = 0.f;
            ++amk;
            amk_step = M3T_MARK_AT(amk);
        }
        amx = fmaxf(fmaxf(amx, m3t_fin_abs(c.dr)), fmaxf(m3t_fin_abs(c.dz), m3t_fin_abs(c.dn)));
        sout[PARV * 2 * SLOTS + slot_c] = (f32x4){pok ? c.dr : 0.f, pok ? c.dz : 0.f, pok ? c.dn : 0.f, pok ? c.dnr : 0.f};
        if (step > 0 && hok) {
            const f32x4 r4 = sout[(1 - PARV) * 2 * SLOTS + slot_h];
            st_dr = r4[0]; st_dz = r4[1]; st_dn = r4[2]; st_dnr = r4[3];
            store_results(step - 1);
        }
    }
    M3T_QSTAMP(5);
}
```

### m3f.pytorch_amd/csrc/gru_persist_fwd6_step.inc

```
    {
        const int step = STEPV;
        const int t = d.reverse ? T - 1 - step : step;
        M3T_STAMP(0);
        M3T_MARK_STEP_TOP(step);
        if (step > 0) {
            const unsigned tag = (ex.tag_base + (unsigned)step) & 0xffffu;
            const unsigned long long* src = gran + (size_t)(1 - PARV) * slot + grp + lane_off;
            pu32x4 v[KS][4];
            int spins = 0;
            if (!pw && (ex.poll_align & 1)) {
                int w = 0;
                while (__hip_atomic_load(&pub_step, __ATOMIC_RELAXED, __HIP_MEMORY_SCOPE_WORKGROUP) < step && ++w < ex.spin_limit) __builtin_amdgcn_s_sleep(1);
            }
            for (int z = 0; z < poll_delay; ++z) __builtin_amdgcn_s_sleep(1);
            for (;;) {
#pragma unroll
                for (int k = 0; k < KS; ++k) {
                    const unsigned long long* qp = src + (size_t)(2 * k) * NW * TILE;
                    asm volatile("global_load_dwordx4 %0, %4, off sc1\n\t"
                                 "global_load_dwordx4 %1, %4, off offset:512 sc1\n\t"
                                 "global_load_dwordx4 %2, %4, off offset:1024 sc1\n\t"
                                 "global_load_dwordx4 %3, %4, off offset:1536 sc1"
                                 : "=&v"(v[k][0]), "=&v"(v[k][1]), "=&v"(v[k][2]), "=&v"(v[k][3])
                                 : "v"(qp) : "memory");
                }
                asm volatile("s_waitcnt vmcnt(0)" ::: "memory");
                bool ok = true;
#pragma unroll
                for (int k = 0; k < KS; ++k)
#pragma unroll
                    for (int jp = 0; jp < 4; ++jp) {
                        asm volatile("" : "+v"(v[k][jp]));
                        ok = ok && ((v[k][jp].y >> 16) == tag) && ((v[k][jp].w >> 16) == tag);
                    }
                if (__all(ok) || dead) break;
                if (++spins > ex.spin_limit) { dead = true; if (lane == 0) raise_spin(err, step); break; }
                __builtin_amdgcn_s_sleep(1);
            }
            if (spins > 0 && lane == 0) atomicOr(&poll_fail[PARV], 1u);
            M3T_STAMP(1);
            if (F16) {
                pf16x8 F1[KS], F2[KS];
#pragma unroll
                for (int k = 0; k < KS; ++k) {
                    pu32x4 a1, a2;
#pragma unroll
                    for (int jj = 0; jj < 4; ++jj) {
                        a1[jj] = __builtin_amdgcn_perm(v[k][jj].z, v[k][jj].x, 0x05040100u);
                        a2[jj] = __builtin_amdgcn_perm(v[k][jj].z, v[k][jj].x, 0x07060302u);
                    }
                    F1[k] = __builtin_bit_cast(pf16x8, a1); F2[k] = __builtin_bit_cast(pf16x8, a2);
                }
#pragma unroll
                for (int u = 0; u < UW; ++u) {
                    f32x4 acc[3];
#pragma unroll
                    for (int ct = 0; ct < 3; ++ct) acc[ct] = (f32x4){0.f, 0.f, 0.f, 0.f};
#pragma unroll
                    for (int k = 0; k < KS; ++k)
#pragma unroll
                        for (int ct = 0; ct < 3; ++ct) {
                            acc[ct] = __builtin_amdgcn_mfma_f32_16x16x32_f16(F2[k], __builtin_bit_cast(pf16x8, wf[u][k][ct][0]), acc[ct], 0, 0, 0);
                            acc[ct] = __builtin_amdgcn_mfma_f32_16x16x32_f16(F1[k], __builtin_bit_cast(pf16x8, wf[u][k][ct][1]), acc[ct], 0, 0, 0);
                            acc[ct] = __builtin_amdgcn_mfma_f32_16x16x32_f16(F1[k], __builtin_bit_cast(pf16x8, wf[u][k][ct][0]), acc[ct], 0, 0, 0);
                        }
#pragma unroll
                    for (int ct = 0; ct < 3; ++ct)
#pragma unroll
                        for (int r = 0; r < 4; ++r) M3T_RED(PARV, wave, u, ct, (lane >> 4) * 4 + r, lane & 15) = acc[ct][r];
                }
            } else {
                f32x4 acc[UW][3];
#pragma unroll
                for (int u = 0; u < UW; ++u)
#pragma unroll
                    for (int ct = 0; ct < 3; ++ct) acc[u][ct] = (f32x4){0.f, 0.f, 0.f, 0.f};
#pragma unroll
                for (int k = 0; k < KS; ++k) {
                    pu32x4 a1, a2, a3;
#pragma unroll
                    for (int jj = 0; jj < 4; ++jj) {
                        a1[jj] = __builtin_amdgcn_perm(v[k][jj].z, v[k][jj].x, 0x05040100u);
                        a2[jj] = __builtin_amdgcn_perm(v[k][jj].z, v[k][jj].x, 0x07060302u);
                        a3[jj] = __builtin_amdgcn_perm(v[k][jj].w, v[k][jj].y, 0x05040100u);
                    }
                    const pbf16x8 A1 = __builtin_bit_cast(pbf16x8, a1), A2 = __builtin_bit_cast(pbf16x8, a2),
                                  A3 = __builtin_bit_cast(pbf16x8, a3);
#pragma unroll
                    for (int u = 0; u < UW; ++u)
#pragma unroll
                        for (int ct = 0; ct < 3; ++ct) {
                            acc[u][ct] = __builtin_amdgcn_mfma_f32_16x16x32_bf16(A3, wf[u][k][ct][0], acc[u][ct], 0, 0, 0);
                            acc[u][ct] = __builtin_amdgcn_mfma_f32_16x16x32_bf16(A2, wf[u][k][ct][1], acc[u][ct], 0, 0, 0);
                            acc[u][ct] = __builtin_amdgcn_mfma_f32_16x16x32_bf16(A1, wf[u][k][ct][NTERM - 1], acc[u][ct], 0, 0, 0);
                            acc[u][ct] = __builtin_amdgcn_mfma_f32_16x16x32_bf16(A2, wf[u][k][ct][0], acc[u][ct], 0, 0, 0);
                            acc[u][ct] = __builtin_amdgcn_mfma_f32_16x16x32_bf16(A1, wf[u][k][ct][1], acc[u][ct], 0, 0, 0);
                            acc[u][ct] = __builtin_amdgcn_mfma_f32_16x16x32_bf16(A1, wf[u][k][ct][0], acc[u][ct], 0, 0, 0);
                        }
                }
#pragma unroll
                for (int u = 0; u < UW; ++u)
#pragma unroll
                    for (int ct = 0; ct < 3; ++ct)
#pragma unroll
                        for (int r = 0; r < 4; ++r) M3T_RED(PARV, wave, u, ct, (lane >> 4) * 4 + r, lane & 15) = acc[u][ct][r];
            }
        }
        asm volatile("s_waitcnt vmcnt(0)" ::: "memory");
        asm volatile("" : "+v"(CUR(xr)), "+v"(CUR(xz)), "+v"(CUR(xn)));
        if (CO && pw) sx[PARV * UW * SLOTS + slot_h] = (f32x4){CUR(xr), CUR(xz), CUR(xn), 0.f};
        M3T_FWD_LOAD_X(step + 1, NXT(xr), NXT(xz), NXT(xn));
        M3T_STAMP(2);
        __syncthreads();
        M3T_MARK_AFTER_BARRIER(step);
        if (ex.poll_fixed < 0) {
            const bool wg_failed = poll_fail[PARV] != 0;
            if (tid == 0) poll_fail[(1 - PARV)] = 0;
            poll_delay = wg_failed ? min(poll_delay + 2, POLL_DELAY_MAX) : ((step & 7) == 0 && poll_delay > 0 ? poll_delay - 1 : poll_delay);
        }
        M3T_STAMP(3);
        if (pw) {
            float hr = br, hz = bz, hn = bn;
            if (step > 0) {
                if (F16) {
                    float sr = 0.f, sz = 0.f, sn = 0.f;
#pragma unroll
                    for (int w = 0; w < NW; ++w) {
                        sr += M3T_RED(PARV, w, tu, 0, prow, pu);
                        sz += M3T_RED(PARV, w, tu, 1, prow, pu);
                        sn += M3T_RED(PARV, w, tu, 2, prow, pu);
                    }
                    hr = fmaf(sr, winv, br); hz = fmaf(sz, winv, bz); hn = fmaf(sn, winv, bn);
                } else {
#pragma unroll
                    for (int w = 0; w < NW; ++w) {
                        hr += M3T_RED(PARV, w, tu, 0, prow, pu);
                        hz += M3T_RED(PARV, w, tu, 1, prow, pu);
                        hn += M3T_RED(PARV, w, tu, 2, prow, pu);
                    }
                }
            }
            float c_xr = CUR(xr), c_xz = CUR(xz), c_xn = CUR(xn);
            if (CO) { const f32x4 x4 = sx[PARV * UW * SLOTS + slot_c]; c_xr = x4[0]; c_xz = x4[1]; c_xn = x4[2]; }
            const GateFwd c = gru_cell_fwd(c_xr, c_xz, c_xn, hr, hz, hn, hprev);
            if (step + 1 < T && !(step == ex.fault_step && blockIdx.x == 0)) {
                const float hv = pok ? (g.bf16 ? rbf(c.h) : c.h) : 0.f;
                unsigned long long gq;
                if (F16) {
                    const float hs = hv * 16384.f;
                    const _Float16 f1 = (_Float16)hs;
                    const _Float16 f2 = (_Float16)(hs - (float)f1);
                    gq = (unsigned long long)__builtin_bit_cast(unsigned short, f1) |
                         ((unsigned long long)__builtin_bit_cast(unsigned short, f2) << 16) |
                         ((unsigned long long)((ex.tag_base + (unsigned)step + 1u) & 0xffffu) << 48);
                } else {
                    const __bf16 h1 = (__bf16)hv;
                    const float r1 = hv - (float)h1;
                    const __bf16 h2 = (__bf16)r1;
                    const __bf16 h3 = (__bf16)(r1 - (float)h2);
                    gq = (unsigned long long)__builtin_bit_cast(unsigned short, h1) |
                         ((unsigned long long)__builtin_bit_cast(unsigned short, h2) << 16) |
                         ((unsigned long long)__builtin_bit_cast(unsigned short, h3) << 32) |
                         ((unsigned long long)((ex.tag_base + (unsigned)step + 1u) & 0xffffu) << 48);
                }
                {
                    unsigned long long* q_ = gran + (size_t)PARV * slot + pub;
                    if (l2mode) asm volatile("global_store_dwordx2 %0, %1, off" :: "v"(q_), "v"(gq) : "memory");
                    else asm volatile("global_store_dwordx2 %0, %1, off sc1" :: "v"(q_), "v"(gq) : "memory");
                }
            }
            if (tid == 0) __hip_atomic_store(&pub_step, step + 1, __ATOMIC_RELAXED, __HIP_MEMORY_SCOPE_WORKGROUP);
            M3T_STAMP(4);
            hprev = c.h;
            if (CO) {
                so[PARV * UW * SLOTS + slot_c] = (f32x4){c.r, c.z, c.n, hn};
                sh[PARV * UW * SLOTS + slot_c] = c.h;
                if (step > 0 && hok) store_results(step - 1, so[(1 - PARV) * UW * SLOTS + slot_h], sh[(1 - PARV) * UW * SLOTS + slot_h]);
            } else if (pok) {
                d.out[((size_t)pb * T + t) * d.ldo + d.ooff + pj] = c.h;
                if (d.gates) {
                    float* gp = d.gates + ((size_t)pb * T + t) * 4 * H;
                    *reinterpret_cast<float4*>(gp + 4 * (size_t)pj) = make_float4(c.r, c.z, c.n, hn);
                }
                if (d.h_n && step == T - 1) d.h_n[(size_t)pb * H + pj] = c.h;
            }
        }
        M3T_STAMP(5);
    }
```

### m3f.pytorch_amd/m3t/_lib.py

```python
import ctypes as C
import os

_HERE = os.path.dirname(os.path.abspath(__file__))
LIB_PATH = os.environ.get("M3T_LIB_PATH") or os.path.join(os.path.dirname(_HERE), "lib", "libm3t_hip.so")
CSRC_DIR = os.path.join(os.path.dirname(_HERE), "csrc")

M3T_EINVAL = 10001
M3T_ESPIN = 10002
M3T_SCAN_NO_PERSIST = 1
M3T_BF16 = 2
M3T_GEMM_BESIDE_SCAN = 512
M3T_GEMM_F16X3 = 1024
M3T_GEMM_HIGH = 256
M3T_GEMM_EXCLUSIVE = 8
M3T_CONV_IMAGES = 4096
M3T_SCAN_FP32 = 4
M3T_SCAN_WHH = 8
M3T_SCAN_FAULT = 16
M3T_SCAN_WIDE = 32
M3T_MAX_SCANS = 8
M3T_JPEG_TRUNC, M3T_JPEG_CODE, M3T_JPEG_RST, M3T_JPEG_EXTRA = 1, 2, 4, 8

_f = C.c_void_p
_i = C.c_int
_z = C.c_size_t
_s = C.c_void_p


class GruFwdDesc(C.Structure):
    _fields_ = [("xproj", _f), ("w_hh", _f), ("b_hh", _f), ("out", _f), ("gates", _f), ("h_n", _f),
                ("H", _i), ("reverse", _i), ("ldx", _i), ("xoff", _i), ("ldo", _i), ("ooff", _i)]


class GruBwdDesc(C.Structure):
    _fields_ = [("dout", _f), ("out", _f), ("gates", _f), ("w_hh_t", _f), ("dh_n", _f),
                ("dgx", _f), ("dgh", _f), ("dh", _f), ("db_part", _f), ("db_ih", _f), ("db_hh", _f),
                ("H", _i), ("reverse", _i), ("ldo", _i), ("ooff", _i), ("ldg", _i), ("goff", _i), ("amax", _f), ("wfrag", _f)]


class WindowProblem(C.Structure):
    _fields_ = [("A", _f), ("B", _f), ("C", _f), ("bias", _f), ("amax_a", _f), ("amax_b", _f), ("accumulate", _i)]


class AttDecArgs(C.Structure):
    _fields_ = [(n, _f) for n in ("enc", "P", "h0", "w_a", "v", "w_ih", "w_hh", "b_ih", "b_hh", "w_o", "b_o", "y0", "trg", "tf",
                                  "out", "h_last", "G", "alpha", "a_save", "x", "gates", "hs", "dout", "dh_last", "dgi", "dgh",
                                  "dc", "da", "dy", "dP", "dv_acc", "dh", "dy0", "w_iht", "wt", "dyin", "dhz")] + \
        [(n, _i) for n in ("B", "T", "L", "H", "save")]


M3T_WINDOW_BATCH = 8

SIGNATURES = {
    "m3t_version": [],
    "m3t_device_arch": [C.c_char_p, _i],
    "m3t_sgemm": [_i, _i, _i, _i, _i, _f, _i, _f, _i, _f, _i, _f, _i, _i, _i, _i, _i, _i, _f, _z, _i, _s],
    "m3t_sgemm_scaled": [_i, _i, _i, _i, _i, _f, _i, _f, _i, _f, _i, _f, _i, _i, _i, _i, _i, _i, _f, _z, _i, _f, _f, _s],
    "m3t_sgemm_window": [_i, _i, _i, _i, _i, _i, _i, _f, _i, _f, _i, _f, _i, _f, _i, _i, _i, _f, _f, _s],
    "m3t_sgemm_window_batch": [_i, C.POINTER(WindowProblem), _i, _i, _i, _i, _i, _i, _i, _i, _i, _i, _i, _i, _s],
    "m3t_absmax": [_i, C.POINTER(C.c_void_p), C.POINTER(C.c_size_t), C.POINTER(C.c_int), C.POINTER(C.c_size_t), C.POINTER(C.c_void_p), _s],
    "m3t_sgemm_plan": [_i, _i, _i, _i, _i, _z, _i, C.POINTER(C.c_int), C.POINTER(C.c_int)],
    "m3t_im2col3d": [_f] + [_i] * 14 + [_f, C.c_longlong, _i, C.c_void_p, _s],
    "m3t_conv3d_taps": [_f, _f, _f] + [_i] * 17 + [_f, _f, _f, _z, _f, _s],
    "m3t_sgemm_pre": [_i, _i, _i, _f, _i, _f, _i, _f, _i, _f, _i, _i, _f, _f, _s],
    "m3t_f16x3_split": [_f, _z, _i, _z, _f, _z, _f, _s],
    "m3t_f16x3_split_perm": [_f, _z, _i, _i, _z, _z, _z, _f, _f, _s],
    "m3t_f16x3_image_b": [_f, _i, _i, _z, _f, _f, _s],
    "m3t_sgemm_bimg": [_i, _i, _i, _f, _i, _f, _f, _i, _f, _i, _i, _f, _z, _f, _f, _s],
    "m3t_sgemm_ring": [_i, _i, _i, _i, _i, _f, _i, _f, _i, _f, _i, _f, _i, _i, _i, _i, _i, _i, _f, _z, _i, _f, _f, _i, _s],
    "m3t_conv3d_taps_pre": [_f, _f, _f] + [_i] * 16 + [_f, _f, _f, _z, _f, _s],
    "m3t_conv3d_fwd_taps": [_f, _f, _f, _f] + [_i] * 15 + [_f, _f, _f, _z, _f, _s],
    "m3t_conv3d_fwd_taps4": [_f, _f, _f, _f] + [_i] * 14 + [_f, _f, _f, _z, _f, _s],
    "m3t_planes_to_cl4": [_f, _f, _i, _i, C.c_longlong, _s],
    "m3t_conv3d_wgrad_taps": [_f, _f, _f] + [_i] * 16 + [_f, _f, _f, _z, _s],
    "m3t_amax_out": [C.c_void_p],
    "m3t_colsum": [_f, _i, _i, _i, _f, _i, _f, _z, _s],
    "m3t_transpose": [_f, _i, _i, _i, _f, _i, _s],
    "m3t_relu_bwd": [_f, _f, _z, _s],
    "m3t_gru_scan_fwd": [C.POINTER(GruFwdDesc), _i, _i, _i, _f, _z, _i, _s],
    "m3t_gru_scan_bwd": [C.POINTER(GruBwdDesc), _i, _i, _i, _f, _z, _i, _s],
    "m3t_gru_bwd_prepare_floats": [_i],
    "m3t_gru_bwd_prepare": [C.POINTER(C.c_void_p), _i, _i, _i, C.POINTER(C.c_void_p), _s],
    "m3t_gru_persist_count": [],
    "m3t_gru_scan_workgroups": [_i, _i, _i, _i, _i, _i],
    "m3t_gru_poll_error": [],
    "m3t_gru_error_reset": [],
    "m3t_gru_error_defer": [_i],
    "m3t_gru_inject_error": [_s],
    "m3t_gru_persist_owner": [],
    "m3t_gru_scan_arena": [C.c_void_p, _z],
    "m3t_gru_scan_arena_reset": [C.c_void_p],
    "m3t_gru_scan_after": [C.c_void_p],
    "m3t_gru_scan_progress": [C.c_void_p, _i, C.POINTER(C.c_int), C.POINTER(C.c_uint)],
    "m3t_gru_scan_progress_reset": [C.c_void_p],
    "m3t_gru_scan_progress_ok": [_i, _i, _i, _i, _i, _i],
    "m3t_stream_wait_progress": [C.c_void_p, C.c_uint, _s],
    "m3t_gru_scan_events": [C.c_void_p, C.c_void_p],
    "m3t_gru_persist_profile": [C.c_void_p],
    "m3t_att_fuse_fwd": [_f, _f, _f, _f, _f, _i, _i, _s],
    "m3t_att_fuse_bwd": [_f, _f, _f, _f, _f, _f, _f, _f, _f, _i, _i, _s],
    "m3t_bn_cl_ws_bytes": [_z, _i],
    "m3t_bn_cl_fwd": [_f, _z, _i, _f, _f, _f, _f, C.c_float, C.c_float, _i, _i, _f, _f, _f, _f, _z, _s],
    "m3t_bn_cl_bwd": [_f, _f, _f, _f, _f, _f, _z, _i, _i, _i, _f, _f, _f, _f, _f, _z, _s],
    "m3t_bn_pool_cl_fwd": [_f, _z, _i, _i, _i, _i, _f, _f, _f, _f, C.c_float, C.c_float, _i, _f, C.c_void_p, _f, _f, _f, _z, _s],
    "m3t_bn_pool_cl_bwd": [_f, _f, _f, C.c_void_p, _f, _f, _f, _z, _i, _i, _i, _i, _i, _f, _f, _f, _f, _f, _z, _s],
    "m3t_pool_cl_fwd": [_f, _z, _i, _i, _i, _i, _i, _i, _i, _i, _i, _f, C.c_void_p, _s],
    "m3t_pool_cl_bwd": [_f, C.c_void_p, _z, _i, _i, _i, _i, _i, _i, _i, _i, _i, _f, _s],
    "m3t_bn_add_relu_cl_fwd": [_f, _f, _z, _i, _f, _f, _f, _f, C.c_float, C.c_float, _i, _f, _f, _f, _f, _z, _s],
    "m3t_bn_add_relu_cl_bwd": [_f, _f, _f, _f, _f, _f, _z, _i, _i, _f, _f, _f, _f, _f, _f, _z, _s],
    "m3t_mean_cl_fwd": [_f, _z, _i, _i, _f, _s],
    "m3t_mean_cl_bwd": [_f, _z, _i, _i, _f, _s],
    "m3t_add_bn_relu_cl_fwd": [_f, _f, _z, _i, _f, _f, _f, _f, C.c_float, C.c_float, _i, _f, _f, _f, _f, _f, _z, _s],
    "m3t_add_bn_relu_cl_bwd": [_f, _f, _f, _f, _f, _f, _f, _z, _i, _i, _f, _f, _f, _f, _f, _z, _s],
    "m3t_gn_cl_ws_bytes": [_i, _z, _i],
    "m3t_gn_cl_fwd": [_f, _i, _z, _i, _i, _f, _f, C.c_float, _i, _f, _f, _f, _f, _z, _s],
    "m3t_gn_cl_bwd": [_f, _f, _f, _f, _f, _f, _i, _z, _i, _i, _i, _f, _f, _f, _f, _f, _z, _s],
    "m3t_gn_pool_cl_fwd": [_f, _i, _i, _i, _i, _i, _i, _i, _f, _f, C.c_float, _f, C.c_void_p, _f, _f, _f, _z, _s],
    "m3t_gn_pool_cl_bwd": [_f, _f, _f, C.c_void_p, _f, _f, _f, _i, _i, _i, _i, _i, _i, _i, _f, _f, _f, _f, _f, _z, _s],
    "m3t_relu_cl_ws_bytes": [_z, _i],
    "m3t_relu_cl_fwd": [_f, _z, _i, _f, _s],
    "m3t_relu_cl_bwd": [_f, _f, _z, _i, _f, _f, _f, _z, _s],
    "m3t_relu_pool_cl_fwd": [_f, _z, _i, _i, _i, _i, _f, C.c_void_p, _s],
    "m3t_relu_pool_cl_bwd": [_f, _f, C.c_void_p, _z, _i, _i, _i, _i, _f, _f, _f, _z, _s],
    "m3t_va_loss": [_f, _i, _i, _i, _i, _f, _f, _f, _f, _i, C.c_float, C.c_float, C.c_float, _i, _f, _f, _f, _z, _s],
    "m3t_va_loss_ws_bytes": [_i],
    "m3t_weight_norm_fwd": [_f, _f, _f, _f, _i, _i, _i, _s],
    "m3t_weight_norm_bwd": [_f, _f, _f, _f, _f, _f, _i, _i, _i, _s],
    "m3t_causal_conv_fwd": [_f, _f, _f, _f, _f, _f, _f, _i, _i, _i, _i, _i, _i, _i, _i, _s],
    "m3t_causal_conv_wgrad": [_f, _f, _f, _i, _i, _i, _i, _i, _i, _f, _z, _s],
    "m3t_conv1d_fwd": [_f, _f, _f, _f, _f, _f, _f, _i, _i, _i, _i, _i, _i, _i, _i, _i, C.c_float, C.c_ulonglong, _i, _s],
    "m3t_conv1d_fwd_scaled": [_f, _f, _f, _f, _f, _f, _f, _i, _i, _i, _i, _i, _i, _i, _i, _i, C.c_float, C.c_ulonglong, _i, _f, _f, _s],
    "m3t_conv1d_wgrad": [_f, _f, _f, _i, _i, _i, _i, _i, _i, _i, _f, _z, _i, _s],
    "m3t_conv1d_wgrad_scaled": [_f, _f, _f, _i, _i, _i, _i, _i, _i, _i, _f, _z, _i, _f, _f, _s],
    "m3t_pool_planes_fwd": [_f, C.c_longlong, _i, _i, _i, _i, _i, _i, _i, _i, _f, C.c_void_p, _s],
    "m3t_pool_planes_bwd": [_f, C.c_void_p, C.c_longlong, _i, _i, _i, _i, _i, _i, _i, _i, _f, _s],
    "m3t_bn_planes_ws_bytes": [_i, _i, _i],
    "m3t_bn_planes_fwd": [_f, _i, _i, _i, _f, _f, _f, _f, C.c_float, C.c_float, _i, _i, _f, _f, _f, _f, _z, _s],
    "m3t_bn_planes_bwd": [_f, _f, _f, _f, _f, _f, _i, _i, _i, _i, _i, _f, _f, _f, _f, _z, _s],
    "m3t_bn_rows_ws_bytes": [_i, _i],
    "m3t_bn_rows_fwd": [_f, _i, _i, _f, _f, _f, _f, C.c_float, C.c_float, _i, _i, _f, _f, _f, _f, _z, _s],
    "m3t_bn_rows_bwd": [_f, _f, _f, _f, _f, _f, _i, _i, _i, _i, _f, _f, _f, _f, _z, _s],
    "m3t_bct_to_btc": [_f, _f, _i, _i, _i, _s],
    "m3t_bct_to_btc_sums": [_f, _f, _i, _i, _i, _f, _s],
    "m3t_bct_to_btc_img": [_f, _f, _i, _i, _i, C.c_void_p, _f, _s],
    "m3t_btc_to_bct": [_f, _f, _i, _i, _i, _s],
    "m3t_mask_pos": [_f, _f, _f, _f, _z, _s],
    "m3t_add_relu": [_f, _f, _f, _z, _s],
    "m3t_mask_pos_drop": [_f, _f, _f, _i, _i, C.c_float, C.c_ulonglong, _s],
    "m3t_cbam_channel_fwd": [_f, _f, _f, _f, _f, _f, _f, _f, _f, _f, _i, _i, _i, _i, _s],
    "m3t_cbam_channel_bwd": [_f, _f, _f, _f, _f, _f, _f, _f, _f, _f, _f, _f, _f, _i, _i, _i, _i, _f, _z, _s],
    "m3t_cbam_spatial_fwd": [_f, _f, _f, _f, _f, _f, _f, _f, _f, _f, _i, _i, _i, _i, _i, C.c_float, C.c_float, _f, _z, _s],
    "m3t_cbam_spatial_bwd": [_f, _f, _f, _f, _f, _f, _f, _f, _f, _f, _f, _f, _i, _i, _i, _i, _i, _f, _z, _s],
    "m3t_cbam_fused_ok": [_i, _i, _i, _i],
    "m3t_cbam_fused_ws_bytes": [_i, _i, _i, _i, _i],
    "m3t_cbam_fwd": [_f] * 20 + [_i] * 6 + [C.c_float, C.c_float, _f, _z, _s],
    "m3t_cbam_bwd": [_f] * 23 + [_i] * 6 + [_f, _z, _s],
    "m3t_smooth_tracks": [_f, _f, _i, _i, _i, _f, _s],
    "m3t_ccc_masked": [_f, _f, _f, C.c_longlong, _i, _f, _s],
    "m3t_eval_append": [_f, _i, _i, _i, _f, _f, _f, _f, _f, _s],
    "m3t_eval_gather": [_f, C.c_longlong, _i, _i, _f, _f, _f, _f, _f, _i, C.c_longlong, C.c_longlong, _f, _s],
    "m3t_eval_metrics": [_f, C.c_longlong, _f, _s],
    "m3t_ccc_tracks": [_f, _f, _f, _f, _i, _i, _f, _s],
    "m3t_frame_window": [_f, C.c_longlong, _i, _i, _i, _f, _f, C.c_longlong, _s],
    "m3t_power_spectrum": [_f, C.c_longlong, _i, _f, _s],
    "m3t_power_to_db": [_f, C.c_longlong, C.c_float, C.c_float, _f, _f, _z, _s],
    "m3t_stack_context": [_f, C.c_longlong, _i, C.c_longlong, _i, _i, _i, _f, _s],
    "m3t_audio_frame_batch": [_f, _i, C.c_longlong, _f, _i, C.c_longlong, _i, _i, _f, _f, _s],
    "m3t_audio_power_mel": [_f, C.c_longlong, _i, _i, _f, _f, _i, _f, _s],
    "m3t_audio_db_stack": [_f, C.c_longlong, _f, _i, _i, _i, _i, _i, C.c_float, C.c_float, _f, _s],
    "m3t_stack_context_batch": [_f, C.c_longlong, _i, _f, _i, _i, _i, _i, _f, _s],
    "m3t_video_ingest": [_f, _i, _i, _i, _i, _f, _i, _f, _f, _i, _i, _i, _i, _f, _s],
    "m3t_video_ingest_half": [_f, _i, _i, _i, _i, _f, _i, _f, _f, _i, _i, _i, _i, _f, _s],
# ... 97 lines not shown
```

### m3f.pytorch_amd/m3t/ops.py

```python
import ctypes as C
import os
import sys

import torch

from . import _lib
from ._lib import GruFwdDesc, GruBwdDesc, M3T_MAX_SCANS, M3THipError

_WS = {}
_WS_MIN = 64 << 20

PROFILE = []

import weakref

_GRAD_SINKS = {}


def register_grad_sink(param, view, owner=None):
    _GRAD_SINKS[id(param)] = [weakref.ref(param), view, False, id(owner) if owner is not None else None]


def clear_grad_sinks(owner=None):
    if owner is None:
# ... 503 lines not shown
                    sgemm(1, 0, N, K, M, dy, 0, N, x, 0, K, w_sink, 0, K, prec=ctx.prec, amax=(a_dy, a_x))
                    if slots is not None:
                        slots.record_stream(wg)
            else:
                dw = w_sink if w_sink is not None else torch.empty_like(w)
                sgemm(1, 0, N, K, M, dy, 0, N, x, 0, K, dw, 0, K, prec=ctx.prec, exclusive=True, amax=(a_dy, a_x))
                if w_sink is not None:
                    dw = None
        if ctx.has_bias and ctx.needs_input_grad[2]:
            if b_sink is not None and off_chain is not None:
                with off_chain:
                    colsum(dy, 0, M, N, N, b_sink)
            else:
                db = b_sink if b_sink is not None else torch.empty(N, dtype=x.dtype, device=x.device)
                colsum(dy, 0, M, N, N, db)
                if b_sink is not None:
                    db = None
        if off_chain is not None and (w_sink is not None or b_sink is not None):
            dy.record_stream(wg)
            x.record_stream(wg)
            _WGRAD_PENDING[(x.device.type, x.device.index)] = True
            _LINEAR_RR[0] += 1
        return dx, dw, db, None, None


_LINEAR_RR = [0]


_NBT_PENDING = [None, 0]


def count_batch(counter):
    if counter is None:
        return
    if _NBT_PENDING[0] is not None:
        _NBT_PENDING[0].append(counter)
    else:
        counter.add_(1)


class batch_counters:
    def __enter__(self):
        if _NBT_PENDING[1] == 0:
            _NBT_PENDING[0] = []
        _NBT_PENDING[1] += 1
        return self

    def __exit__(self, *exc):
        _NBT_PENDING[1] -= 1
        if _NBT_PENDING[1] == 0:
            pending, _NBT_PENDING[0] = _NBT_PENDING[0], None
            if pending:
                counts = {}
                for t in pending:
                    e = counts.setdefault((t.device, t.data_ptr()), [t, 0])
                    e[1] += 1
                ts, ks = [e[0] for e in counts.values()], [e[1] for e in counts.values()]
                if len(ts) > 1 and all(t.is_cuda for t in ts):
                    torch._foreach_add_(ts, 1 if max(ks) == 1 else ks)
                else:
                    for t, k in zip(ts, ks):
                        t.add_(k)
        return False


class _AddRelu(torch.autograd.Function):

    @staticmethod
    def forward(ctx, a, b):
        out = torch.empty_like(a)
        slot = amax_slots(1, a.device) if TRANSPOSE_IMAGES[0] else None
        _armed_call(_p(slot), "m3t_add_relu", _p(a), _p(b), _p(out), a.numel(), _stream())
        _OUT_SLOT[0] = slot
        ctx.save_for_backward(out)
        return out

    @staticmethod
    def backward(ctx, dout):
        out, = ctx.saved_tensors
        g = mask_pos(out, _req(dout.contiguous(), "dout"))
        return g, g


def add_relu(a, b):
    if (a.is_cuda and a.dtype == torch.float32 and b.dtype == torch.float32 and a.shape == b.shape and a.device == b.device
            and a.is_contiguous() and b.is_contiguous()):
        _OUT_SLOT[0] = None
        return _tag_out(_AddRelu.apply(a, b))
    return torch.relu(a + b)


class _ReluDropout(torch.autograd.Function):

    @staticmethod
    def forward(ctx, y, p, seed):
        y = _req(y.contiguous(), "y")
        ctx.save_for_backward(y)
        ctx.drop = (float(p), int(seed))
        return mask_pos(y, y, drop=ctx.drop)

    @staticmethod
    def backward(ctx, dy):
        (y,) = ctx.saved_tensors
        return mask_pos(y, _req(dy.contiguous(), "dy"), drop=ctx.drop), None, None


def relu_dropout(y, p, seed=None):
    if p <= 0:
        return y
    if seed is None:
        seed = int(torch.empty(1, dtype=torch.int64).random_().item())
    return _ReluDropout.apply(y, float(p), int(seed))


def linear(x, w, b=None, act=0):
    return _Linear.apply(x, w, b, act, _is_unit(x))


SCAN_PER_STEP = [False]
SCAN_FAULT = [False]
RANGE_PROBE = [[] if os.environ.get("M3T_F16X3_PROBE") == "1" else None]


def _probe_range(tag, t2d):
    a = t2d.abs()
    rmax, cmax, gmax = a.amax(1), a.amax(0), a.max()
    big = torch.full((), float("inf"), device=t2d.device)
    lim = gmax * 2.0 ** -17
    sq = t2d.double() ** 2
    tot = sq.sum()
    past_r, past_c = rmax < lim, cmax < lim
    RANGE_PROBE[0].append((tag, gmax, torch.where(rmax > 0, rmax, big).min(), torch.where(cmax > 0, cmax, big).min(),
                           past_r.sum(), past_c.sum(), sq.sum(1)[past_r].sum() / tot, sq.sum(0)[past_c].sum() / tot))


def range_probe_report(clear=True):
    keys = ("tag", "max", "row_spread", "col_spread", "rows_past", "cols_past", "row_energy_past", "col_energy_past")
    out = []
    for rec in (RANGE_PROBE[0] or []):
        v = [rec[0]] + [float(x) for x in rec[1:]]
        v[2], v[3] = v[1] / v[2], v[1] / v[3]
        out.append(dict(zip(keys, v)))
    if clear and RANGE_PROBE[0] is not None:
        RANGE_PROBE[0] = []
    return out


PREP_AHEAD = [os.environ.get("M3T_SCAN_PREP_AHEAD", "1") != "0"]
SCAN_FIRST = [os.environ.get("M3T_SCAN_FIRST", "0") == "1"]
FORCE_WIDE_FWD = [False]
SCAN_FP32 = [False]


_FENCED = [False]


def _scan_flags(device):
    if SCAN_PER_STEP[0] or (_ws_tag(device) == "side" and not _FENCED[0]):
        return _lib.M3T_SCAN_NO_PERSIST
    return (_lib.M3T_SCAN_FP32 if SCAN_FP32[0] else 0) | (_lib.M3T_SCAN_FAULT if SCAN_FAULT[0] else 0)


_DEFERRED = [False]


def defer_scan_errors(on=True):
    _DEFERRED[0] = bool(on)
    _lib.check(lib().m3t_gru_error_defer(1 if on else 0), "m3t_gru_error_defer")


_DEFER_OWNERS = [0]


def defer_scan_errors_acquire():
    _DEFER_OWNERS[0] += 1
    if _DEFER_OWNERS[0] == 1:
        defer_scan_errors(True)


def defer_scan_errors_release():
    if _DEFER_OWNERS[0] > 0:
        _DEFER_OWNERS[0] -= 1
        if _DEFER_OWNERS[0] == 0:
            defer_scan_errors(False)


def poll_scan_error(sync=False, force=False):
    if _DEFERRED[0] and not force:
        return
    if sync and torch.cuda.is_available():
        torch.cuda.synchronize()
    try:
        _lib.poll_scan_error()
    except M3THipError:
        reset_progress()
        raise


def inject_scan_error():
    _lib.check(lib().m3t_gru_inject_error(_stream()), "m3t_gru_inject_error")


def persist_owner():
    return int(lib().m3t_gru_persist_owner())


def grad_poison_(flat, dead):
    _lib.check(lib().m3t_grad_poison(_p(flat), _p(dead), _stream()), "m3t_grad_poison")


def grad_dead_check_(dead):
    _lib.check(lib().m3t_grad_dead_check(_p(dead), _stream()), "m3t_grad_dead_check")


def _scan_after(ev):
    if ev is not None:
        _lib.check(lib().m3t_gru_scan_after(C.c_void_p(ev.cuda_event)), "m3t_gru_scan_after")


_ARENAS = {}
_ARENA_BYTES = (8 << 20) + (64 << 10)


def _scan_arena(device):
    key = (device.type, device.index, _ws_tag(device))
    a = _ARENAS.get(key)
    if a is None:
        a = torch.empty(_ARENA_BYTES, dtype=torch.uint8, device=device)
        _ARENAS[key] = a
        _lib.check(lib().m3t_gru_scan_arena_reset(C.c_void_p(a.data_ptr())), "m3t_gru_scan_arena_reset")
    _lib.check(lib().m3t_gru_scan_arena(C.c_void_p(a.data_ptr()), _ARENA_BYTES), "m3t_gru_scan_arena")


_ce = os.environ.get("M3T_SCAN_CHUNKS", "0")
CHUNKS = [{"0": False, "1": True}.get(_ce, _ce)]
_CHUNK_WINDOWS = 4
_PROGRESS = {}


def _progress_counters(device):
    key = (device.type, device.index, _ws_tag(device))
    t = _PROGRESS.get(key)
    if t is None:
        t = _PROGRESS[key] = torch.zeros(2, dtype=torch.int32, device=device)
        _lib.check(lib().m3t_gru_scan_progress_reset(C.c_void_p(t.data_ptr())), "m3t_gru_scan_progress_reset")
    return t


def reset_progress():
    for t in _PROGRESS.values():
        t.zero_()
        _lib.check(lib().m3t_gru_scan_progress_reset(C.c_void_p(t.data_ptr())), "m3t_gru_scan_progress_reset")


def _chunk_bounds(B, T, n=None, backward=False):
    import math
    n = n or _CHUNK_WINDOWS
    q = 128 // math.gcd(B, 128)
    on = CHUNKS[0] is True or CHUNKS[0] == ("bwd" if backward else "fwd")
    if not on or (B * T) % 128 != 0 or T < 16 * n or B * T < 4096:
        return None
    tb = [int(round(k * T / n / q)) * q for k in range(1, n)]
    lo = [0] + tb
    hi = tb + [T]
    if any(b - a < 8 for a, b in zip(lo, hi)) or tb[0] < 4 or tb[-1] > T - 4 or (T - tb[-1]) * B % 128 != 0:
        return None
    return tb


def _arrivals(tb, T):
    n = len(tb)
    ev = []
    for w in range(n + 1):
        ev.append((tb[w] if w < n else T, 0, w if w < n else None, w))
        ev.append((T - tb[w - 1] if w > 0 else T, 1, (n - w) if w > 0 else None, w))
    ev.sort(key=lambda e: (e[0], e[1]))
    seen, out = set(), []
    for step, d, k, w in ev:
        out.append((d, k, w, w in seen))
        seen.add(w)
    return out


def _wait_progress(counters, dirn, need):
    _lib.check(lib().m3t_stream_wait_progress(C.c_void_p(counters.data_ptr() + 4 * dirn), int(need) & 0xffffffff, _stream()), "m3t_stream_wait_progress")


def sgemm_window(transB, n_seg, win_len, win_stride, win_off, N, K, A, a_off, lda, Bm, b_off, ldb, Cm, c_off, ldc, bias=None, act=0,
                 accumulate=False, prec=None, amax=(None, None)):
    flags = _PREC[0] if prec is None else prec
    rc = lib().m3t_sgemm_window(transB, n_seg, win_len, win_stride, win_off, N, K, _p(A, a_off), lda, _p(Bm, b_off), ldb, _p(Cm, c_off), ldc,
                                _p(bias), act, int(accumulate), flags, amax[0], amax[1], _stream())
    _lib.check(rc, "m3t_sgemm_window")


def sgemm_window_batch(problems, transB, n_seg, win_len, win_stride, win_off, N, K, lda, ldb, ldc, act=0, prec=None):
    flags = _PREC[0] if prec is None else prec
    WP = _lib.WindowProblem
    for i in range(0, len(problems), _lib.M3T_WINDOW_BATCH):
        chunk = problems[i:i + _lib.M3T_WINDOW_BATCH]
        arr = (WP * len(chunk))(*[WP(_vp(A, ao), _vp(Bm, bo), _vp(Cm, co), _vp(bias), aa, ab, int(acc))
                                  for A, ao, Bm, bo, Cm, co, bias, acc, aa, ab in chunk])
        _lib.check(lib().m3t_sgemm_window_batch(len(chunk), arr, transB, n_seg, win_len, win_stride, win_off, N, K, lda, ldb, ldc, act, flags,
                                                _stream()), "m3t_sgemm_window_batch")


# ... 3 lines not shown
        assert len(descs) <= M3T_MAX_SCANS
        ctr, tb = progress
        need = (C.c_uint * (2 * len(tb)))()
        _lib.check(lib().m3t_gru_scan_progress(C.c_void_p(ctr.data_ptr()), len(tb), (C.c_int * len(tb))(*tb), need), "m3t_gru_scan_progress")
    _scan_fwd_(descs, B, T, prec, after)
    return None if need is None else list(need)


def _scan_fwd_(descs, B, T, prec=0, after=None):
    for i in range(0, len(descs), M3T_MAX_SCANS):
        chunk = descs[i:i + M3T_MAX_SCANS]
        arr = (GruFwdDesc * len(chunk))(*chunk)
        flops = (T - 1) * sum(2.0 * B * 3 * d.H * d.H for d in chunk)
        with _Timed("gru_step_fwd_kernel", T, flops, kernel_side=True) as tm:
            dev = torch.device("cuda", _CUR_DEV())
            ws = workspace(dev)
            n0 = lib().m3t_gru_persist_count() if tm.rec is not None else 0
            _scan_after(after if i == 0 else None)
            _scan_arena(dev)
            rc = lib().m3t_gru_scan_fwd(arr, len(chunk), B, T, _p(ws), ws.numel() * 4, _scan_flags(dev) | prec, _stream())
            if tm.rec is not None and lib().m3t_gru_persist_count() != n0:
                tm.rec.update(kernel="gru_persist_fwd_kernel", launches=1, steps=T)
        _lib.check(rc, "m3t_gru_scan_fwd")


def _scan_bwd(descs, B, T, prec=0, after=None, progress=None):
    need = None
    if progress is not None:
        assert len(descs) <= M3T_MAX_SCANS
        ctr, tb = progress
        need = (C.c_uint * (2 * len(tb)))()
        _lib.check(lib().m3t_gru_scan_progress(C.c_void_p(ctr.data_ptr()), len(tb), (C.c_int * len(tb))(*tb), need), "m3t_gru_scan_progress")
    _scan_bwd_(descs, B, T, prec, after)
    return None if need is None else list(need)


def _scan_bwd_(descs, B, T, prec=0, after=None):
    for i in range(0, len(descs), M3T_MAX_SCANS):
        chunk = descs[i:i + M3T_MAX_SCANS]
        arr = (GruBwdDesc * len(chunk))(*chunk)
        flops = (T - 1) * sum(2.0 * B * 3 * d.H * d.H for d in chunk)
        with _Timed("gru_step_bwd_kernel", T, flops, kernel_side=True) as tm:
            dev = torch.device("cuda", _CUR_DEV())
            ws = workspace(dev)
            n0 = lib().m3t_gru_persist_count() if tm.rec is not None else 0
            _scan_after(after if i == 0 else None)
            _scan_arena(dev)
            rc = lib().m3t_gru_scan_bwd(arr, len(chunk), B, T, _p(ws), ws.numel() * 4, _scan_flags(dev) | prec, _stream())
            if tm.rec is not None and lib().m3t_gru_persist_count() != n0:
                tm.rec.update(kernel="gru_persist_bwd_kernel", launches=1, steps=T)
        _lib.check(rc, "m3t_gru_scan_bwd")


def _vp(t, off=0):
    return t.data_ptr() + 4 * off if t is not None else None


def _stream_groups(Hs, B):
    if _PERSIST_ENABLED and not SCAN_PER_STEP[0] and len(set(Hs)) > 1 and all(h % 128 == 0 and h <= 512 for h in Hs):
        return [("main", [i for i, h in enumerate(Hs) if h == hh]) for hh in sorted(set(Hs), reverse=True)]
    hmax = max(Hs)
    heavy = [i for i, h in enumerate(Hs) if h == hmax]
    light = [i for i, h in enumerate(Hs) if h != hmax]
    wgs = sum(2 * (Hs[i] // 16) * ((B + 15) // 16) for i in heavy)
    if light and wgs >= 192:
        return [("side", light), ("main", heavy)]
    return [("main", list(range(len(Hs))))]


def _interleaved(groups):
    return (_PERSIST_ENABLED and not SCAN_PER_STEP[0] and len(groups) == 2
            and all(kind == "main" for kind, _ in groups))


_CONCURRENT_ENABLED = os.environ.get("M3T_SCAN_CONCURRENT", "1") != "0"
_CUS = {}


def _pair_fits(dev, n_heavy, H_heavy, n_light, H_light, B, T, prec):
    if not _CONCURRENT_ENABLED:
        return False
    key = (dev.type, dev.index)
    cus = _CUS.get(key)
    if cus is None:
        cus = _CUS[key] = torch.cuda.get_device_properties(dev).multi_processor_count
    base = _scan_flags(dev) | prec
    if base & _lib.M3T_SCAN_NO_PERSIST:
        return False
    for bwd in (0, 1):
        a = lib().m3t_gru_scan_workgroups(n_heavy, H_heavy, B, T, base | _lib.M3T_SCAN_WIDE, bwd)
        b = lib().m3t_gru_scan_workgroups(n_light, H_light, B, T, base | _lib.M3T_SCAN_WIDE, bwd)
        if a <= 0 or b <= 0 or a + b > cus or (a + 7) // 8 + (b + 7) // 8 > cus // 8:
            return False
    return True


class _MultiBiGRU(torch.autograd.Function):

    @staticmethod
    def forward(ctx, n_stacks, L, cat_lo, cat_hi, unit_mask, *tensors):
        per = 1 + 8 * L
        assert len(tensors) == n_stacks * per
        xs, params = [], []
        for s in range(n_stacks):
            xs.append(_req(tensors[s * per].contiguous(), "x"))
            params.append([_req(t, "gru parameter") for t in tensors[s * per + 1:(s + 1) * per]])
        B, T = xs[0].shape[0], xs[0].shape[1]
        dev = xs[0].device
        for x in xs:
            if x.shape[0] != B or x.shape[1] != T:
                raise M3THipError("grouped GRU stacks must share batch and length")
        Hs = [params[s][1].shape[1] for s in range(n_stacks)]
        new = lambda *shape: torch.empty(*shape, dtype=torch.float32, device=dev)
        h_ns = [new(2 * L, B, Hs[s]) for s in range(n_stacks)]
        outs = [[new(B, T, 2 * Hs[s]) for s in range(n_stacks)] for _ in range(L)]
        cat_buf = None
        if cat_hi - cat_lo >= 2:
            cat_buf = new(B, T, sum(2 * Hs[s] for s in range(cat_lo, cat_hi)))
            off = 0
            for s in range(cat_lo, cat_hi):
                outs[L - 1][s] = cat_buf[..., off:off + 2 * Hs[s]]
                off += 2 * Hs[s]
        gates = [[new(2, B, T, 4 * Hs[s]) for s in range(n_stacks)] for _ in range(L)]
        xprojs = [[new(B, T, 6 * Hs[s]) for s in range(n_stacks)] for _ in range(L)]
        main = cur_stream()
        prec = _PREC[0]
        groups = _stream_groups(Hs, B)
        fslots = None
        if (prec & _lib.M3T_GEMM_F16X3) and all(h % 4 == 0 for h in Hs):
            fslots = amax_slots(n_stacks * (1 + 2 * L), dev)
            items = [(xs[s], fslots.data_ptr() + 8 * s) for s in range(n_stacks) if not (unit_mask >> s) & 1]
            wslot = {}
            ctx.w_keep = []
            for l in range(L):
                for s in range(n_stacks):
                    for d in (0, 1):
                        a = weight_amax(params[s][(2 * l + d) * 4], ctx.w_keep)
                        if a is None:
                            a = fslots.data_ptr() + 8 * (n_stacks + (l * n_stacks + s) * 2 + d)
                            items.append((params[s][(2 * l + d) * 4], a))
                        wslot[(l, s, d)] = a
            if not measure_amax(items):
                fslots = None
        one = amax_one(dev)

        def fslot_x(l, s):
            return None if fslots is None else (fslots.data_ptr() + 8 * s if (l == 0 and not (unit_mask >> s) & 1) else one)

        def fslot_w(l, s, d):
            return None if fslots is None else wslot[(l, s, d)]

        alone = not _interleaved(groups) and all(kind == "main" for kind, _ in groups)

        def level_fwd(l, idxs, scan, after=None, wide=False, progress=None):
            descs = []
            for s in idxs:
                H = Hs[s]
                inp = xs[s] if l == 0 else outs[l - 1][s]
                I = inp.shape[-1]
                for d in (0, 1):
                    w_ih, w_hh, b_ih, b_hh = params[s][(2 * l + d) * 4:(2 * l + d) * 4 + 4]
                    if not scan:
                        sgemm(0, 1, B * T, 3 * H, I, inp, 0, I, w_ih, 0, I, xprojs[l][s], d * 3 * H, 6 * H, bias=b_ih, prec=prec,
                              exclusive=alone, amax=(fslot_x(l, s), fslot_w(l, s, d)))
                    else:
                        descs.append(GruFwdDesc(_vp(xprojs[l][s]), _vp(w_hh), _vp(b_hh), _vp(outs[l][s]),
                                                _vp(gates[l][s], d * B * T * 4 * H), _vp(h_ns[s], (2 * l + d) * B * H),
                                                H, d, 6 * H, d * 3 * H, outs[l][s].stride(1), d * H))
            if scan:
                return _scan_fwd(descs, B, T, prec | (_lib.M3T_SCAN_WIDE if (wide or FORCE_WIDE_FWD[0]) else 0), after,
                                 None if progress is None else (_progress_counters(dev), progress))

        def chunk_plan(idxs, wide):
            if L < 2 or fslots is None or len({Hs[i] for i in idxs}) != 1 or 2 * len(idxs) > M3T_MAX_SCANS:
                return None
            H = Hs[idxs[0]]
            if H % 64 != 0:
                return None
            fl = _scan_flags(dev) | prec | (_lib.M3T_SCAN_WIDE if (wide or FORCE_WIDE_FWD[0]) else 0)
            if not lib().m3t_gru_scan_progress_ok(2 * len(idxs), H, B, T, fl, 0):
                return None
            return _chunk_bounds(B, T)

        def proj_pieces(l, idxs, tb, need, scan_stream):
            wg = wgrad_stream(dev, 0)
            ctr = _progress_counters(dev)
            ev_end = torch.cuda.Event()
            ev_end.record(scan_stream)
            lo, hi = [0] + tb, tb + [T]
            with on_stream(wg):
                ended = False
                for dirn, k, w, second in _arrivals(tb, T):
                    if k is None:
                        if not ended:
                            wg.wait_event(ev_end)
                            ended = True
                    else:
                        _wait_progress(ctr, dirn, need[dirn * len(tb) + k])
                    H = Hs[idxs[0]]
                    lda = outs[l - 1][idxs[0]].stride(1)
                    probs = []
                    for si in idxs:
                        src = outs[l - 1][si]
                        assert src.stride(1) == lda
                        for d in (0, 1):
                            w_ih, _, b_ih, _ = params[si][(2 * l + d) * 4:(2 * l + d) * 4 + 4]
                            probs.append((src, dirn * H, w_ih, dirn * H, xprojs[l][si], d * 3 * H, None if second else b_ih, second,
                                          one, fslot_w(l, si, d)))
                    sgemm_window_batch(probs, 1, B, hi[w] - lo[w], T, lo[w], 3 * H, H, lda, 2 * H, 6 * H, prec=prec)
                ev = torch.cuda.Event()
                ev.record(wg)
            scan_stream.wait_event(ev)

        concurrent = (_interleaved(groups) and len({Hs[i] for i in groups[0][1]}) == 1 and len({Hs[i] for i in groups[1][1]}) == 1
                      and _pair_fits(dev, 2 * len(groups[0][1]), Hs[groups[0][1][0]], 2 * len(groups[1][1]), Hs[groups[1][1][0]], B, T, prec))
        if concurrent:
            heavy, light = groups[0][1], groups[1][1]
            side = side_stream(dev)
            side.wait_stream(main)
            _FENCED[0] = True
            try:
                tb = chunk_plan(heavy, True)
                if tb is not None:
                    wgrad_stream(dev, 0).wait_stream(main)
                for l in range(L):
                    if l == 0 or tb is None:
                        level_fwd(l, heavy, False)
                    ev_al = None
                    if ALIGN_LIGHT[0] and l > 0:
                        ev_al = torch.cuda.Event()
                        ev_al.record(main)
                    with on_stream(side):
                        level_fwd(l, light, False)
                        level_fwd(l, light, True, ev_al, True)
                    need = level_fwd(l, heavy, True, None, True, tb if l + 1 < L else None)
                    if tb is not None and l + 1 < L:
                        proj_pieces(l + 1, heavy, tb, need, main)
            finally:
                _FENCED[0] = False
            main.wait_stream(side)
        elif _interleaved(groups):
            heavy, light = groups[0][1], groups[1][1]
            side = side_stream(dev)
            side.wait_stream(main)
            ev_light = None
            _FENCED[0] = True
            try:
                if L == 2:
                    level_fwd(0, heavy, False)
                    with on_stream(side):
                        level_fwd(0, light, False)
                    level_fwd(0, heavy, True, None)
                    ev_h0 = torch.cuda.Event()
                    ev_h0.record(main)
                    with on_stream(side):
                        level_fwd(0, light, True, ev_h0)
                        level_fwd(1, light, False)
                        level_fwd(1, light, True)
                        ev_light = torch.cuda.Event()
                        ev_light.record(side)
                    level_fwd(1, heavy, False)
                    level_fwd(1, heavy, True, ev_light)
                else:
                  for l in range(L):
                    level_fwd(l, heavy, False)
                    with on_stream(side):
                        level_fwd(l, light, False)
                    level_fwd(l, heavy, True, ev_light)
                    ev_heavy = torch.cuda.Event()
                    ev_heavy.record(main)
                    with on_stream(side):
                        level_fwd(l, light, True, ev_heavy)
                        ev_light = torch.cuda.Event()
                        ev_light.record(side)
            finally:
                _FENCED[0] = False
            main.wait_stream(side)
        else:
            for kind, idxs in groups:
                stream = main
                if kind == "side":
                    stream = side_stream(dev)
                    stream.wait_stream(main)
                with on_stream(stream):
                    tb = chunk_plan(idxs, False) if (kind == "main" and alone) else None
                    if tb is not None:
                        wgrad_stream(dev, 0).wait_stream(stream)
                    for l in range(L):
                        if l == 0 or tb is None:
                            level_fwd(l, idxs, False)
                        need = level_fwd(l, idxs, True, progress=tb if l + 1 < L else None)
                        if tb is not None and l + 1 < L:
                            proj_pieces(l + 1, idxs, tb, need, stream)
            for kind, _ in groups:
                if kind == "side":
                    main.wait_stream(side_stream(dev))
        del xprojs
        ctx.wfq, ctx.wfq_ev = None, None
        if PREP_AHEAD[0] and any(ctx.needs_input_grad) and fslots is not None and all(p_.is_contiguous() for prm in params for p_ in prm):
            wfq = {}
            bfl = _scan_flags(dev) | prec | _lib.M3T_SCAN_WHH | _lib.M3T_SCAN_WIDE
            jobs = []
            for _, idxs in groups:
                H = Hs[idxs[0]]
                if len({Hs[i] for i in idxs}) == 1 and H % 256 == 0 and 2 * len(idxs) <= M3T_MAX_SCANS \
                        and lib().m3t_gru_scan_progress_ok(2 * len(idxs), H, B, T, bfl, 1):
                    nfl = int(lib().m3t_gru_bwd_prepare_floats(H))
                    for l in range(L):
                        ws_, outs_ = [], []
                        for si in idxs:
                            for d in (0, 1):
                                buf = new(nfl)
                                wfq[(l, si, d)] = buf
                                ws_.append(params[si][(2 * l + d) * 4 + 1])
                                outs_.append(buf)
                        jobs.append((H, ws_, outs_))
            if jobs:
                wg1 = wgrad_streams(dev)[1]
                wg1.wait_stream(main)
                with on_stream(wg1):
                    for H, ws_, outs_ in jobs:
                        n_ = len(ws_)
                        _lib.check(lib().m3t_gru_bwd_prepare((C.c_void_p * n_)(*[t.data_ptr() for t in ws_]), n_, H, 1,
                                                             (C.c_void_p * n_)(*[t.data_ptr() for t in outs_]), _stream()), "m3t_gru_bwd_prepare")
                    ctx.wfq_ev = torch.cuda.Event()
                    ctx.wfq_ev.record(wg1)
                ctx.wfq = wfq
        ctx.n_stacks, ctx.L, ctx.Hs, ctx.B, ctx.T, ctx.prec = n_stacks, L, Hs, B, T, prec
        ctx.unit_mask = unit_mask
        ctx.concurrent = concurrent
        ctx.cat = (cat_lo, cat_hi) if cat_buf is not None else (0, 0)
        saved = []
        for l in range(L):
            for s in range(n_stacks):
                saved += [outs[l][s], gates[l][s]]
        ctx.has_fslots = fslots is not None
        ctx.wslot = wslot if fslots is not None else None
        if fslots is not None:
            for st_ in (side_stream(dev),):
                fslots.record_stream(st_)
            saved.append(fslots)
        ctx.save_for_backward(*(list(tensors) + saved))
        result = []
        for s in range(n_stacks):
            if cat_buf is not None and cat_lo <= s < cat_hi:
                result += [cat_buf if s == cat_lo else new(0), h_ns[s]]
            else:
                result += [outs[L - 1][s], h_ns[s]]
        return tuple(result)

    @staticmethod
    def backward(ctx, *grads):
        n_stacks, L, Hs, B, T = ctx.n_stacks, ctx.L, ctx.Hs, ctx.B, ctx.T
        per = 1 + 8 * L
        st = ctx.saved_tensors
        tensors, acts = st[:n_stacks * per], st[n_stacks * per:]
        fslots = None
        if ctx.has_fslots:
            fslots, acts = acts[-1], acts[:-1]
        params = [list(tensors[s * per + 1:(s + 1) * per]) for s in range(n_stacks)]
        xs = [tensors[s * per].contiguous() for s in range(n_stacks)]

        def layer_io(l, s):
            out, gts = acts[(l * n_stacks + s) * 2], acts[(l * n_stacks + s) * 2 + 1]
            inp = xs[s] if l == 0 else acts[((l - 1) * n_stacks + s) * 2]
            return inp, out, gts

        dev = params[0][0].device
        new = lambda *shape: torch.empty(*shape, dtype=torch.float32, device=dev)
        out_grads = [None] * (n_stacks * per)
        sunk = [False] * (n_stacks * per)
        douts, dhns = [], []
        cat_lo, cat_hi = ctx.cat
        dcat = None
        if cat_hi > cat_lo:
            g = grads[2 * cat_lo]
            dcat = (torch.zeros(B, T, sum(2 * Hs[s] for s in range(cat_lo, cat_hi)), dtype=torch.float32, device=dev) if g is None
                    else _req(g.contiguous(), "dout"))
        off = 0
        for s in range(n_stacks):
            g, gh = grads[2 * s], grads[2 * s + 1]
            if dcat is not None and cat_lo <= s < cat_hi:
                douts.append(dcat[..., off:off + 2 * Hs[s]])
                off += 2 * Hs[s]
            else:
                douts.append(torch.zeros(B, T, 2 * Hs[s], dtype=torch.float32, device=dev) if g is None
                             else _req(g.contiguous(), "dout"))
            dhns.append(None if gh is None else _req(gh.contiguous(), "dh_n"))
        dgx = [[new(B, T, 6 * Hs[s]) for s in range(n_stacks)] for _ in range(L)]
        dgh = [[new(2, B, T, 3 * Hs[s]) for s in range(n_stacks)] for _ in range(L)]
        dh = [[new(2, B, Hs[s]) for s in range(n_stacks)] for _ in range(L)]
        dbp = [[new(2, B, 4, Hs[s]) for s in range(n_stacks)] for _ in range(L)]
        direct_whh = all(h % 16 == 0 for h in Hs) and all(p.is_contiguous() for prm in params for p in prm)
        wht = [[[None if direct_whh else new(Hs[s], 3 * Hs[s]) for _ in (0, 1)] for s in range(n_stacks)] for _ in range(L)]
        need_dx = [[l > 0 or ctx.needs_input_grad[5 + s * per] for s in range(n_stacks)] for l in range(L)]
        dinp = [[torch.empty_like(layer_io(l, s)[0]) if need_dx[l][s] else None for s in range(n_stacks)] for l in range(L)]
        for s in range(n_stacks):
            for l in range(L):
                for d in (0, 1):
                    w_ih, w_hh = params[s][(2 * l + d) * 4], params[s][(2 * l + d) * 4 + 1]
                    base = s * per + 1 + (2 * l + d) * 4
                    for j, prm in enumerate(params[s][(2 * l + d) * 4:(2 * l + d) * 4 + 4]):
                        sink = _take_sink(prm)
                        out_grads[base + j] = sink if sink is not None else torch.empty_like(prm)
                        sunk[base + j] = sink is not None
        main = cur_stream()
        groups = _stream_groups(Hs, B)
        cur = {s: douts[s] for s in range(n_stacks)}
        prec = ctx.prec
        wfq = ctx.wfq or {}
        if ctx.wfq_ev is not None:
            main.wait_event(ctx.wfq_ev)
        NSL = _CHUNK_WINDOWS + 1
        bslots = amax_slots(2 * L * n_stacks * NSL, dev) if fslots is not None else None
        one = amax_one(dev)

        def bslot(l, s, d, j=-1):
            return None if bslots is None else bslots.data_ptr() + 8 * (((l * n_stacks + s) * 2 + d) * NSL + 1 + j)

        def fslot_x(l, s):
            return None if fslots is None else (fslots.data_ptr() + 8 * s if (l == 0 and not (ctx.unit_mask >> s) & 1) else one)

        def fslot_w(l, s, d):
            return None if fslots is None else ctx.wslot[(l, s, d)]

        def chunk_plan(l, idxs):
            if bslots is None or len({Hs[i] for i in idxs}) != 1 or 2 * len(idxs) > M3T_MAX_SCANS or not any(need_dx[l][s] for s in idxs):
                return None
            H = Hs[idxs[0]]
            if H % 64 != 0 or any(need_dx[l][s] and layer_io(l, s)[0].shape[-1] % 64 != 0 for s in idxs) or not direct_whh:
                return None
            fl = _scan_flags(dev) | prec | _lib.M3T_SCAN_WHH | _lib.M3T_SCAN_WIDE
            if not lib().m3t_gru_scan_progress_ok(2 * len(idxs), H, B, T, fl, 1):
                return None
            tb = _chunk_bounds(B, T, backward=True)
            return tb if (tb is not None and len(tb) + 1 <= _CHUNK_WINDOWS) else None

        def dx_pieces(l, idxs, tb, need, scan_stream):
            wg = wgs[1]
            ctr = _progress_counters(dev)
            ev_end = torch.cuda.Event()
            ev_end.record(scan_stream)
            lo, hi = [0] + tb, tb + [T]
            n = len(tb)
            with on_stream(wg):
                ended = False
                for dirn, k, w, second in _arrivals(tb, T):
                    if k is None:
                        if not ended:
                            wg.wait_event(ev_end)
                            ended = True
                    else:
                        _wait_progress(ctr, dirn, need[dirn * n + k])
                    d = 1 - dirn
                    j = w if dirn == 0 else n - w
                    by_shape = {}
                    for si in idxs:
                        if need_dx[l][si]:
                            I = layer_io(l, si)[0].shape[-1]
                            by_shape.setdefault(I, []).append((dgx[l][si], d * 3 * Hs[si], params[si][(2 * l + d) * 4], 0, dinp[l][si], 0, None,
                                                               second, bslot(l, si, d, j), fslot_w(l, si, d)))
                    for I, probs in by_shape.items():
                        H = Hs[idxs[0]]
                        sgemm_window_batch(probs, 0, B, hi[w] - lo[w], T, lo[w], I, 3 * H, 6 * H, I, I, prec=prec)
                ev = torch.cuda.Event()
                ev.record(wg)
            scan_stream.wait_event(ev)
            for si in idxs:
                if need_dx[l][si]:
                    cur[si] = dinp[l][si]

        def start_marks(idxs):
            if not SCAN_FIRST[0] or bslots is None or len({Hs[i] for i in idxs}) != 1 or 2 * len(idxs) > M3T_MAX_SCANS or T < 64 or not direct_whh:
                return None
            fl = _scan_flags(dev) | prec | _lib.M3T_SCAN_WHH | _lib.M3T_SCAN_WIDE
            if not lib().m3t_gru_scan_progress_ok(2 * len(idxs), Hs[idxs[0]], B, T, fl, 1):
                return None
            return [8, T - 8]

        held = {}

        def release_held(key, started):
            fn = held.pop(key, None)
            if fn is None:
                return
            if started is not None:
                ctr_, need_ = started
                with on_stream(wgs[0]):
                    _wait_progress(ctr_, 0, need_[0])
                    _wait_progress(ctr_, 1, need_[2])
            fn()

        def level_scan(l, idxs, after=None, wide=False, progress=None):
            descs = []
            for s in idxs:
                H = Hs[s]
                inp, out, gts = layer_io(l, s)
                for d in (0, 1):
                    w_hh = params[s][(2 * l + d) * 4 + 1]
                    if not direct_whh:
                        _lib.check(lib().m3t_transpose(_p(w_hh), 3 * H, H, H, _p(wht[l][s][d]), 3 * H, _stream()),
                                   "m3t_transpose")
                    base = s * per + 1 + (2 * l + d) * 4
                    descs.append(GruBwdDesc(_vp(cur[s]), _vp(out), _vp(gts, d * B * T * 4 * H),
                                            _vp(w_hh if direct_whh else wht[l][s][d]),
                                            _vp(dhns[s], (2 * l + d) * B * H) if dhns[s] is not None else None,
                                            _vp(dgx[l][s]), _vp(dgh[l][s], d * B * T * 3 * H), _vp(dh[l][s], d * B * H),
                                            _vp(dbp[l][s], d * B * 4 * H), _vp(out_grads[base + 2]), _vp(out_grads[base + 3]),
                                            H, d, out.stride(1), d * H, 6 * H, d * 3 * H, bslot(l, s, d),
                                            _vp(wfq[(l, s, d)]) if (l, s, d) in wfq else None))
            chain = _ws_tag(dev)
            sm = None
            if progress is None and chain in held:
                sm = start_marks(idxs)
            need = _scan_bwd(descs, B, T, prec | (_lib.M3T_SCAN_WHH if direct_whh else 0) | _lib.M3T_SCAN_WIDE, after,
                             None if (progress is None and sm is None) else (_progress_counters(dev), progress if progress is not None else sm))
            if progress is not None:
                pending[(l, tuple(idxs))] = (progress, need)
            release_held(chain, (_progress_counters(dev), need) if sm is not None else None)
            if RANGE_PROBE[0] is not None:
                for s in idxs:
                    for d in (0, 1):
                        _probe_range("dgx l%d s%d d%d H%d" % (l, s, d, Hs[s]), dgx[l][s].view(B * T, 6 * Hs[s])[:, d * 3 * Hs[s]:(d + 1) * 3 * Hs[s]])
                        _probe_range("dgh l%d s%d d%d H%d" % (l, s, d, Hs[s]), dgh[l][s][d].view(B * T, 3 * Hs[s]))

        pending = {}

        def level_dx(l, idxs):
            pg = pending.pop((l, tuple(idxs)), None)
            if pg is not None:
                dx_pieces(l, idxs, pg[0], pg[1], cur_stream())
                return
            for s in idxs:
                H = Hs[s]
                inp, out, gts = layer_io(l, s)
                I = inp.shape[-1]
                if need_dx[l][s]:
                    for d in (0, 1):
                        sgemm(0, 0, B * T, I, 3 * H, dgx[l][s], d * 3 * H, 6 * H, params[s][(2 * l + d) * 4], 0, I,
                              dinp[l][s], 0, I, accumulate=(d == 1), prec=prec, amax=(bslot(l, s, d), fslot_w(l, s, d)))
                    cur[s] = dinp[l][s]

        wgs = wgrad_streams(dev)
        rr = [0]

        def _level_dw(l, idxs, pool):
            for s in idxs:
                H = Hs[s]
                inp, out, gts = layer_io(l, s)
                I = inp.shape[-1]
                for d in (0, 1):
                    base = s * per + 1 + (2 * l + d) * 4
                    dw_ih, dw_hh = out_grads[base:base + 2]
                    goff = d * B * T * 3 * H
                    with (on_stream(pool[rr[0] % len(pool)]) if pool is not None else _NULL):
                        if T > 1:
                            a_off, b_off = (1, 0) if d == 0 else (0, 1)
                            sgemm(1, 0, 3 * H, H, B * (T - 1), dgh[l][s], goff, 3 * H, out, d * H, out.stride(1), dw_hh, 0, H,
                                  seg=(T - 1, T, a_off, b_off), prec=prec, amax=(bslot(l, s, d), one if bslots is not None else None))
                        else:
                            dw_hh.zero_()
                    rr[0] += 1
                    with (on_stream(pool[rr[0] % len(pool)]) if pool is not None else _NULL):
                        sgemm(1, 0, 3 * H, I, B * T, dgx[l][s], d * 3 * H, 6 * H, inp, 0, I, dw_ih, 0, I, prec=prec,
                              amax=(bslot(l, s, d), fslot_x(l, s)))
                    rr[0] += 1

        def level_dw(l, idxs, spread=False, wg_i=0):
            if spread:
                _level_dw(l, idxs, [cur_stream(), wgs[1]])
            else:
                with on_stream(wgs[wg_i]):
                    _level_dw(l, idxs, None)

        light_idxs = groups[1][1] if (LIGHT_DW_STREAM1[0] and ctx.concurrent and _interleaved(groups)) else None

        for w_ in wgs:
            w_.wait_stream(main)

        def level_gemms(l, idxs, last=False):
            level_dx(l, idxs)
            ev = torch.cuda.Event()
            ev.record(cur_stream())
            wg_i = 1 if (light_idxs is not None and list(idxs) == list(light_idxs)) else 0
            for w_ in (wgs if last else [wgs[wg_i]]):
                w_.wait_event(ev)
            if last or not SCAN_FIRST[0]:
                level_dw(l, idxs, spread=last, wg_i=wg_i)
            else:
                held[_ws_tag(dev)] = lambda: level_dw(l, idxs, spread=False, wg_i=wg_i)

        if ctx.concurrent and _interleaved(groups):
            heavy, light = groups[0][1], groups[1][1]
            side = side_stream(dev)
            side.wait_stream(main)
            _FENCED[0] = True
            try:
                for l in range(L - 1, -1, -1):
                    ev_al = None
                    if ALIGN_LIGHT[0] and _ALIGN_BWD and l < L - 1:
                        ev_al = torch.cuda.Event()
                        ev_al.record(main)
                    level_scan(l, heavy, None, True, chunk_plan(l, heavy))
                    with on_stream(side):
                        level_scan(l, light, ev_al)
                    level_gemms(l, heavy, last=(l == 0))
                    with on_stream(side):
                        level_gemms(l, light, last=(l == 0))
            finally:
                _FENCED[0] = False
            main.wait_stream(side)
        elif _interleaved(groups):
            heavy, light = groups[0][1], groups[1][1]
            side = side_stream(dev)
            side.wait_stream(main)
            ev_light = None
            _FENCED[0] = True
            try:
                if L == 2:
                    level_scan(1, heavy, None)
                    ev_h1 = torch.cuda.Event()
                    ev_h1.record(main)
                    level_gemms(1, heavy)
                    with on_stream(side):
                        level_scan(1, light, ev_h1)
                        ev_l1 = torch.cuda.Event()
                        ev_l1.record(side)
                        level_gemms(1, light)
                    level_scan(0, heavy, ev_l1)
                    ev_h0 = torch.cuda.Event()
                    ev_h0.record(main)
                    level_gemms(0, heavy, last=True)
                    with on_stream(side):
                        level_scan(0, light, ev_h0)
                        level_gemms(0, light, last=True)
                else:
                  for l in range(L - 1, -1, -1):
                    level_scan(l, heavy, ev_light)
                    ev_heavy = torch.cuda.Event()
                    ev_heavy.record(main)
                    level_gemms(l, heavy)
                    with on_stream(side):
                        level_scan(l, light, ev_heavy)
                        ev_light = torch.cuda.Event()
                        ev_light.record(side)
                        level_gemms(l, light)
            finally:
                _FENCED[0] = False
            main.wait_stream(side)
        else:
            for kind, idxs in groups:
                stream = main
                if kind == "side":
                    stream = side_stream(dev)
                    stream.wait_stream(main)
                with on_stream(stream):
                    for l in range(L - 1, -1, -1):
                        level_scan(l, idxs, progress=chunk_plan(l, idxs) if (kind == "main" and len(groups) == 1) else None)
                        level_gemms(l, idxs)
            for kind, _ in groups:
                if kind == "side":
                    main.wait_stream(side_stream(dev))
        for key_ in list(held):
            release_held(key_, None)
        weights_sunk = all(sunk[s * per + 1 + (2 * l + d) * 4 + j] for s in range(n_stacks) for l in range(L) for d in (0, 1) for j in (0, 1))
        if weights_sunk:
            for l in range(L):
                for s in range(n_stacks):
                    for t in (dgx[l][s], dgh[l][s]) + tuple(layer_io(l, s)[:2]):
                        for w_ in wgs:
                            t.record_stream(w_)
            for t in (bslots, fslots):
                if t is not None:
                    for w_ in wgs:
                        t.record_stream(w_)
            _WGRAD_PENDING[(dev.type, dev.index)] = True
        else:
            for w_ in wgs:
                main.wait_stream(w_)
        for s in range(n_stacks):
            out_grads[s * per] = dinp[0][s]
        return (None, None, None, None, None) + tuple(None if sunk[i] else g for i, g in enumerate(out_grads))


def multi_bigru(stacks, cat=None):
    L = stacks[0][2]
    flat = []
    for x, prm, l in stacks:
        if l != L:
            raise M3THipError("grouped GRU stacks must have the same depth")
        flat.append(x)
        flat.extend(prm)
    lo, hi = cat if cat is not None else (0, 0)
    unit_mask = sum(1 << i for i, (x, _, _) in enumerate(stacks) if _is_unit(x))
    res = _MultiBiGRU.apply(len(stacks), L, lo, hi, unit_mask, *flat)
    for i in range(len(stacks)):
        if res[2 * i].numel():
            res[2 * i]._m3t_unit = res[2 * i]._version + 1
    return [(res[2 * i], res[2 * i + 1]) for i in range(len(stacks))]


class _AttFuse(torch.autograd.Function):

    @staticmethod
    def forward(ctx, s_v, s_a, x_v, x_a):
        s_v, s_a = _req(s_v.contiguous(), "s_v"), _req(s_a.contiguous(), "s_a")
        x_v, x_a = _req(x_v.contiguous(), "x_v"), _req(x_a.contiguous(), "x_a")
        D = x_v.shape[-1]
        rows = x_v.numel() // D
        if x_a.shape != x_v.shape or s_v.numel() != rows or s_a.numel() != rows:
            raise M3THipError("att_fuse: shape mismatch")
        f = torch.empty_like(x_v)
        with _Timed("att_fuse_fwd_kernel", 1, 0, nbytes=4.0 * rows * (3 * D + 2)):
            _lib.check(lib().m3t_att_fuse_fwd(_p(s_v), _p(s_a), _p(x_v), _p(x_a), _p(f), rows, D, _stream()), "m3t_att_fuse_fwd")
        ctx.save_for_backward(s_v, s_a, x_v, x_a)
        return f

    @staticmethod
    def backward(ctx, df):
        s_v, s_a, x_v, x_a = ctx.saved_tensors
        df = _req(df.contiguous(), "df")
        D = x_v.shape[-1]
        rows = x_v.numel() // D
        ds_v, ds_a = torch.empty_like(s_v), torch.empty_like(s_a)
        dx_v, dx_a = torch.empty_like(x_v), torch.empty_like(x_a)
        with _Timed("att_fuse_bwd_kernel", 1, 0, nbytes=4.0 * rows * (5 * D + 4)):
            _lib.check(lib().m3t_att_fuse_bwd(_p(df), _p(s_v), _p(s_a), _p(x_v), _p(x_a), _p(ds_v), _p(ds_a), _p(dx_v),
                                              _p(dx_a), rows, D, _stream()), "m3t_att_fuse_bwd")
        return ds_v, ds_a, dx_v, dx_a


def att_fuse(s_v, s_a, x_v, x_a):
    return _AttFuse.apply(s_v, s_a, x_v, x_a)


class _VALoss(torch.autograd.Function):
    @staticmethod
    def forward(ctx, y_hat, valence, arousal, class_expr, expr_valid, iv, ia, n_expr, w_v, w_a, expr_w, use_mse):
        y = _req(y_hat.contiguous(), "y_hat")
        Cc = y.shape[-1]
        rows = y.numel() // Cc
        val = _req(valence.contiguous().float(), "valence")
        aro = _req(arousal.contiguous().float(), "arousal")
        cls = vld = None
        if n_expr > 0:
            cls = class_expr.contiguous().long()
            vld = expr_valid.contiguous().to(torch.uint8)
            if not cls.is_cuda or not vld.is_cuda:
                raise M3THipError("labels must be device tensors")
        stats = torch.empty(8, dtype=torch.float32, device=y.device)
        dy = torch.empty_like(y)
        ws = workspace(y.device)
        with _Timed("va_loss_kernels", 3, 0, nbytes=4.0 * rows * (3 * Cc + 3 * 2 + Cc) + (3.0 * rows * 9 if n_expr > 0 else 0.0)):
            rc = lib().m3t_va_loss(_p(y), rows, Cc, iv, ia, _p(val), _p(aro),
                                   C.c_void_p(cls.data_ptr()) if cls is not None else None,
                                   C.c_void_p(vld.data_ptr()) if vld is not None else None,
                                   n_expr, w_v, w_a, expr_w, int(use_mse), _p(stats), _p(dy), _p(ws), ws.numel() * 4, _stream())
        _lib.check(rc, "m3t_va_loss")
        ctx.save_for_backward(dy)
        ctx.mark_non_differentiable(stats)
        return stats[0], stats

    @staticmethod
    def backward(ctx, g_loss, g_stats):
        (dy,) = ctx.saved_tensors
        return (dy * g_loss,) + (None,) * 11


def va_loss(y_hat, valence, arousal, class_expr=None, expr_valid=None, iv=None, ia=None, n_expr=0,
            w_v=0.5, w_a=0.5, expr_w=0.8, use_mse=False):
    Cc = y_hat.shape[-1]
    iv = Cc - 2 if iv is None else iv
    ia = Cc - 1 if ia is None else ia
    return _VALoss.apply(y_hat, valence, arousal, class_expr, expr_valid, iv, ia, n_expr, float(w_v), float(w_a),
                         float(expr_w), bool(use_mse))


POOL_MODES = {"max": 0, "mean": 1, 0: 0, 1: 1}
LOSS_KINDS = {"ce": 0, "bce": 1, 0: 0, 1: 1}


def _btc(z, name):
    if z.dim() != 3 or min(z.shape) < 1:
        raise ValueError("%s must be [B, T, C] with B, T, C >= 1, got %s" % (name, tuple(z.shape)))
    return z.shape


def _cls_target(logits_shape, target, kind, device):
    B, Cc = logits_shape
    if kind == 0:
        if target.dim() != 1 or target.shape[0] != B or target.dtype != torch.int64:
            raise ValueError("cross-entropy labels must be int64 [B], got %s %s" % (target.dtype, tuple(target.shape)))
    elif tuple(target.shape) != (B, Cc) or target.dtype != torch.float32:
        raise ValueError("binary cross-entropy targets must be float32 [B, C], got %s %s" % (target.dtype, tuple(target.shape)))
    if target.device != device:
        raise M3THipError("the loss target must live on the logits' device")
    return target.contiguous()


class _TemporalPool(torch.autograd.Function):

    @staticmethod
    def forward(ctx, z, mode):
        z = _req(z.contiguous(), "z")
        B, T, Cc = z.shape
        pooled = torch.empty(B, Cc, dtype=torch.float32, device=z.device)
        arg = torch.empty(B, Cc, dtype=torch.int32, device=z.device) if mode == 0 else None
        with _Timed("tpool_fwd_kernel", 1, 0, nbytes=4.0 * B * Cc * (T + 2 - mode)):
            _lib.check(lib().m3t_tpool_fwd(_p(z), B, T, Cc, mode, _p(pooled), arg.data_ptr() if arg is not None else None, _stream()),
                       "m3t_tpool_fwd")
        ctx.mode, ctx.dims = mode, (B, T, Cc)
# ... 2199 lines not shown
```

Baseline: 2837.

## Spread persistent GRU scans over 8-row blocks to occupy more CUs

Adds a SPREAD mode for the persistent forward and backward GRU recurrence kernels. When the batch is small, each block handles 8 clips instead of 16, so more CUs run the scan in parallel. The exchange gather loads half the fragments and fills the other half with DPP lane shifts, and the poll settings are retuned for this shape. The cost is more workgroups taking part in the cross-CU handshake each step, half-empty MFMA tiles, and extra exchange-arena space. It is enabled by default only for a single-stack main group, and only when progress chunking is off.

```diff
diff --git a/include/m3t_hip.h b/include/m3t_hip.h
--- a/include/m3t_hip.h
+++ b/include/m3t_hip.h
@@ -16,6 +16,7 @@
 #define M3T_SCAN_FP32 4
 #define M3T_SCAN_FAULT 16
 #define M3T_SCAN_WIDE 32
+#define M3T_SCAN_SPREAD 64
 #define M3T_BF16 2
 #define M3T_GEMM_BACKGROUND 1
 #define M3T_GEMM_BF16 2
diff --git a/m3f.pytorch_amd/csrc/gru_persist.hip b/m3f.pytorch_amd/csrc/gru_persist.hip
--- a/m3f.pytorch_amd/csrc/gru_persist.hip
+++ b/m3f.pytorch_amd/csrc/gru_persist.hip
@@ -273,11 +273,12 @@
 }
 typedef _Float16 pf16x8 __attribute__((ext_vector_type(8)));
 
-template <int NC, bool F16 = false, int UW = 1>
+template <int NC, bool F16 = false, int UW = 1, int RB = 16>
 __global__ __launch_bounds__(NT) void gru_persist_fwd6_kernel(FwdGroup g, FragPtrs fp, ExPtrs ex, int B, int T, int G, int nrb,
                                                               unsigned* err) {
     constexpr bool CO = UW == 2;
     constexpr int ROWS = 16, KS = NC / 2, NTERM = F16 ? 2 : 3;
+    static_assert(RB == 16 || (RB == 8 && F16), "row blocks: 16 clips, or 8 in the fp16x3 form (the gather deals the units over lane bit 3 for 8 rows)");
     constexpr int H = 128 * NC, nch = H >> 4;
     constexpr int RED_FLOATS = 2 * NW * UW * 3 * ROWS * (UB + 1);
     __shared__ float red_s[UW == 1 ? RED_FLOATS : 1];
@@ -291,7 +292,7 @@
     const m3t_gru_fwd_desc d = g.d[s];
     const int tu = UW == 1 ? 0 : (tid >> 8);
     const int ub = ubw * UW + tu;
-    const int j0 = ub * UB, r0 = rb * ROWS;
+    const int j0 = ub * UB, r0 = rb * RB;
 
     pbf16x8 wf[UW][KS][3][NTERM];
     float winv = 1.f;
@@ -359,7 +360,8 @@
     const bool pw = tid < ROWS * UB * UW;
     const int prow = (ti >> 1) & 15, pu = ((ti >> 5) & 1) * 8 + 2 * ((ti >> 6) & 3) + (ti & 1);
     const int pb = r0 + prow, pj = j0 + pu;
-    const bool pok = pw && pb < B;
+    const bool plive = pw && prow < RB;
+    const bool pok = plive && pb < B;
     float br = 0.f, bz = 0.f, bn = 0.f, hprev = 0.f;
     if (pw) { br = d.b_hh[pj]; bz = d.b_hh[H + pj]; bn = d.b_hh[2 * H + pj]; }
 
@@ -369,7 +371,8 @@
     const size_t grp = (size_t)rb * nch * TILE;
     const size_t pub = grp + (size_t)ubw * UW * TILE + tid;
     const int q = lane >> 4;
-    const size_t lane_off = (size_t)(wave + NW * (q >> 1)) * TILE + 2 * ((q & 1) * 16 + (lane & 15));
+    const size_t lane_off = RB < ROWS ? (size_t)(wave + NW * (q >> 1)) * TILE + 2 * ((q & 1) * 16 + (lane & 7)) + 64 * ((lane >> 3) & 1)
+                                      : (size_t)(wave + NW * (q >> 1)) * TILE + 2 * ((q & 1) * 16 + (lane & 15));
     bool dead = false;
     int poll_delay = ex.poll_fixed >= 0 ? ex.poll_fixed : POLL_DELAY_INIT;
     __shared__ unsigned poll_fail[2];
@@ -385,7 +388,7 @@
     float xrA, xzA, xnA, xrB, xzB, xnB;
     const int hrow = CO ? (ti >> 4) : prow, hun = CO ? (ti & 15) : pu;
     const int hb = r0 + hrow, hj = j0 + hun;
-    const bool hok = pw && hb < B;
+    const bool hok = pw && hrow < RB && hb < B;
     const int hg = 64 * ((hun >> 1) & 3) + 2 * (hrow + 16 * (hun >> 3)) + (hun & 1);
     constexpr int SLOTS = 272;
     const int slot_h = tu * SLOTS + hg + (hg >> 4), slot_c = tu * SLOTS + ti + (ti >> 4);
@@ -883,10 +886,11 @@
     }
 }
 
-template <int NC, bool PROF = false>
+template <int NC, bool PROF = false, int RB = 16>
 __global__ __launch_bounds__(NT) void gru_persist_bwd3q_kernel(BwdGroup g, FragPtrs fp, ExPtrs ex, int B, int T, int G, int nrb,
                                                              unsigned* err) {
     constexpr int ROWS = 16, NP = NC / 2;
+    static_assert(RB == 16 || (RB == 8 && !PROF), "row blocks: 16 clips, or 8 (the gather deals the units over lane bit 3 for 8 rows)");
     constexpr int H = 128 * NC, H3 = 3 * H, nchh = H >> 4;
     __shared__ float red[2][NW][2][ROWS][UB + 1];
     const int tid = threadIdx.x, lane = tid & 63, wave = tid >> 6;
@@ -896,7 +900,7 @@
     const m3t_gru_bwd_desc d = g.d[s];
     const int tu = tid >> 8;
     const int ub = ubw * 2 + tu;
-    const int j0 = ub * UB, r0 = rb * ROWS;
+    const int j0 = ub * UB, r0 = rb * RB;
 
     pu32x4 wb[2][3][NP][2];
     float winv[2];
@@ -917,7 +921,8 @@
     const int ti = tid & 255;
     const int prow = ti & 15, pu = 8 * ((ti >> 4) & 1) + (ti >> 5);
     const int pb = r0 + prow, pj = j0 + pu;
-    const bool pok = pb < B;
+    const bool plive = prow < RB;
+    const bool pok = plive && pb < B;
     float dh_carry = 0.f, z_next = 0.f;
     float sb_r = 0.f, sb_z = 0.f, sb_n = 0.f, sb_nr = 0.f;
     float amx = 0.f;
@@ -928,7 +933,8 @@
     const size_t slot = ex.slot[s];
     const size_t grp = (size_t)rb * nchh * TILE;
     const size_t pub = grp + (size_t)ubw * 2 * TILE + tid;
-    const size_t lane_src = (size_t)(2 * wave + (lane >> 5)) * TILE + ((lane >> 4) & 1) * 16 + (lane & 15);
+    const size_t lane_src = RB < ROWS ? (size_t)(2 * wave + (lane >> 5)) * TILE + ((lane >> 4) & 1) * 16 + (lane & 7) + 32 * ((lane >> 3) & 1)
+                                      : (size_t)(2 * wave + (lane >> 5)) * TILE + ((lane >> 4) & 1) * 16 + (lane & 15);
     bool dead = false;
     int poll_delay = ex.poll_fixed >= 0 ? ex.poll_fixed : POLL_DELAY_INIT;
     __shared__ unsigned poll_fail[2];
@@ -948,7 +954,7 @@
     f32x4 g4A, g4B;
     const int hrow = ti >> 4, hun = ti & 15;
     const int hb = r0 + hrow, hj = j0 + hun;
-    const bool hok = hb < B;
+    const bool hok = hrow < RB && hb < B;
     const int hg = (hun & 7) * 32 + (hun >> 3) * 16 + hrow;
     constexpr int SLOTS = 272;
     const int slot_h = tu * SLOTS + hg + (hg >> 4), slot_c = tu * SLOTS + ti + (ti >> 4);
@@ -1071,26 +1077,27 @@
     return e ? atoi(e) : dflt;
 }
 
-struct Shape { int nc, rt, G, nrb, grid, active, slot_map; };
+struct Shape { int nc, rt, G, nrb, grid, active, slot_map, rb; };
 
 template <typename D>
-bool level_shape(const D* d, int n, int B, Shape& sh, int uw = 1) {
+bool level_shape(const D* d, int n, int B, Shape& sh, int uw = 1, bool spread = false) {
     const int maxh = d[0].H;
     if (maxh % 128 != 0 || maxh > 512) return false;
     for (int i = 1; i < n; ++i)
         if (d[i].H != maxh) return false;
     sh.nc = maxh / 128;
     sh.rt = 0;
+    const bool rb8 = spread && n * cdiv(B, 8) * (maxh / 16) <= device_cus();
     for (int rt = 1; rt <= 2; ++rt) {
         if (uw > 1 && rt > 1) break;
         const int members = maxh / 16 / uw;
-        const int nrb = cdiv(B, 16 * rt), G = n * nrb, active = G * members;
+        const int nrb = rb8 ? cdiv(B, 8) : cdiv(B, 16 * rt), G = n * nrb, active = G * members;
         if (active <= device_cus()) {
 #ifndef M3T_SCAN_L2_MODE
 #define M3T_SCAN_L2_MODE 2
 #endif
             constexpr int l2 = M3T_SCAN_L2_MODE;
-            sh.rt = rt; sh.nrb = nrb; sh.G = G; sh.active = active;
+            sh.rt = rt; sh.nrb = nrb; sh.G = G; sh.active = active; sh.rb = rb8 ? 8 : 16 * rt;
             sh.slot_map = (l2 == 1 || (l2 == 2 && G % 8 == 0) || (uw > 1 && G <= 8)) ? 1 : 0;
             sh.grid = sh.slot_map ? 8 * cdiv(G, 8) * members : active;
             break;
@@ -1448,6 +1455,25 @@
     return ((flags & M3T_SCAN_WIDE) && fwd_is_f16(g, B, T, flags) && (sh.nc == 4 || sh.nc == 2) && sh.rt == 1 && wide_enabled()) ? 2 : 1;
 }
 
+static bool spread_exchange_ok(const Shape& s8, int n, int H, int kind, size_t gran_bytes, bool launching) {
+    if ((size_t)n * 2 * s8.nrb * (H / 16) * 256 * gran_bytes > ARENA_SIZE[kind]) return false;
+    return !launching || (g_arena != nullptr && g_arena_bytes >= ARENA_BYTES && ((uintptr_t)g_arena % 16) == 0);
+}
+static bool fwd_spread(const FwdGroup& g, int B, int T, int flags, int uw, Shape& sh, bool launching) {
+    if (!(flags & M3T_SCAN_SPREAD) || !fwd_is_f16(g, B, T, flags)) return false;
+    Shape s8;
+    if (!level_shape(g.d, g.n, B, s8, uw, true) || s8.rb != 8 || !spread_exchange_ok(s8, g.n, g.d[0].H, 1, 8, launching)) return false;
+    sh = s8;
+    return true;
+}
+static bool bwd_spread(const BwdGroup& g, int B, int flags, Shape& sh, bool launching) {
+    if (!(flags & M3T_SCAN_SPREAD)) return false;
+    Shape s8;
+    if (!level_shape(g.d, g.n, B, s8, 2, true) || s8.rb != 8 || !spread_exchange_ok(s8, g.n, g.d[0].H, 3, 16, launching)) return false;
+    sh = s8;
+    return true;
+}
+
 static int persist_fwd_launch_impl(const FwdGroup& g, const FragPtrs& fp, int B, int T, int flags, hipStream_t s);
 int persist_fwd_launch(const FwdGroup& g, const FragPtrs& fp, int B, int T, int flags, hipStream_t s) {
     ProgressTxn txn;
@@ -1460,6 +1486,7 @@
     if (!level_shape(g.d, g.n, B, sh) || !ensure_err_word()) return M3T_EINVAL;
     const int uw = fwd_uw(g, B, T, flags, sh);
     if (uw > 1 && !level_shape(g.d, g.n, B, sh, uw)) return M3T_EINVAL;
+    if (!persist_progress_armed()) fwd_spread(g, B, T, flags, uw, sh, true);
     {
         if (uw == 1 && !sh.slot_map && sh.G < 8 && fwd_is_f16(g, B, T, flags)) {
             sh.slot_map = 1;
@@ -1474,6 +1501,10 @@
         ex.poll_fixed = persist_fwd_uses_x6(g, B, T, flags) ? -1 : (sh.nc == 1 ? 0 : 12);
         ex.poll_align = persist_fwd_uses_x6(g, B, T, flags) ? 0 : 1;
         if (persist_fwd_uses_x6(g, B, T, flags) && !g.bf16 && (flags & M3T_GEMM_F16X3) && m3t_f16x3_enabled() && sh.nc == 2) ex.poll_align = 1;
+        if (sh.rb == 8) {
+            ex.poll_fixed = sh.nc == 2 ? 8 : 12;
+            ex.poll_align = sh.nc == 2 ? 1 : 0;
+        }
     }
     const bool x6 = persist_fwd_uses_x6(g, B, T, flags);
     if (persist_progress_armed()) {
@@ -1513,10 +1544,15 @@
             if (uw == 2) {
                 const size_t need = (size_t)2 * NW * 2 * 3 * 16 * (UB + 1) * sizeof(float)
                                     + (size_t)2 * 2 * 272 * 36;
-                const FwdKernel kk = sh.nc == 2 ? gru_persist_fwd6_kernel<2, true, 2> : gru_persist_fwd6_kernel<4, true, 2>;
+                const FwdKernel kk = sh.rb == 8 ? (sh.nc == 2 ? gru_persist_fwd6_kernel<2, true, 2, 8> : gru_persist_fwd6_kernel<4, true, 2, 8>)
+                                                : (sh.nc == 2 ? gru_persist_fwd6_kernel<2, true, 2> : gru_persist_fwd6_kernel<4, true, 2>);
                 const size_t dyn = exclusive_lds(kk, sh.active, need);
                 if (dyn < need) return M3T_EINVAL;
                 hipLaunchKernelGGL(kk, dim3(sh.grid), dim3(NT), dyn, s, g, fp, ex, B, T, sh.G, sh.nrb, g_err_dev);
+            }
+            else if (sh.rb == 8) {
+                const FwdKernel kk = sh.nc == 2 ? gru_persist_fwd6_kernel<2, true, 1, 8> : gru_persist_fwd6_kernel<4, true, 1, 8>;
+                hipLaunchKernelGGL(kk, dim3(sh.grid), dim3(NT), exclusive_lds(kk, sh.active), s, g, fp, ex, B, T, sh.G, sh.nrb, g_err_dev);
             }
             else if (sh.nc == 2) hipLaunchKernelGGL((gru_persist_fwd6_kernel<2, true>), dim3(sh.grid), dim3(NT), exclusive_lds(gru_persist_fwd6_kernel<2, true>, sh.active), s, g, fp, ex, B, T, sh.G, sh.nrb, g_err_dev);
             else hipLaunchKernelGGL((gru_persist_fwd6_kernel<4, true>), dim3(sh.grid), dim3(NT), exclusive_lds(gru_persist_fwd6_kernel<4, true>, sh.active), s, g, fp, ex, B, T, sh.G, sh.nrb, g_err_dev);
@@ -1565,6 +1601,7 @@
     const int uw = p3 ? 2 : 1;
     if (uw > 1) {
         if (!level_shape(g.d, g.n, B, sh, uw)) return M3T_EINVAL;
+        if (!persist_progress_armed()) bwd_spread(g, B, flags, sh, true);
         ex.slot_map = sh.slot_map;
     }
     if (persist_progress_armed()) {
@@ -1595,7 +1632,8 @@
             }
             { const int e = persist_take_after(s); if (e) return e; }
             persist_record_start(s);
-            const BwdKernel kq = sh.nc == 2 ? gru_persist_bwd3q_kernel<2> : (ex.prof ? gru_persist_bwd3q_kernel<4, true> : gru_persist_bwd3q_kernel<4>);
+            const BwdKernel kq = sh.rb == 8 ? (sh.nc == 2 ? gru_persist_bwd3q_kernel<2, false, 8> : gru_persist_bwd3q_kernel<4, false, 8>)
+                                 : sh.nc == 2 ? gru_persist_bwd3q_kernel<2> : (ex.prof ? gru_persist_bwd3q_kernel<4, true> : gru_persist_bwd3q_kernel<4>);
             const size_t need = (size_t)2 * 2 * 272 * 40;
             const size_t dyn = exclusive_lds(kq, sh.active, need);
             if (dyn < need) return M3T_EINVAL;
@@ -1701,6 +1739,7 @@
         const bool p3 = !b16 && persist_bwd_uses_x6(g, B, T, flags) && (flags & M3T_GEMM_F16X3) && m3t_f16x3_enabled() && bwd3p_enabled() &&
                         wide256 && (sh.nc == 4 || sh.nc == 2) && (unsigned long long)T + 1 < 0xffffffull;
         if (p3 && !level_shape(g.d, g.n, B, sh, 2)) return 0;
+        if (p3) bwd_spread(g, B, flags, sh, false);
         return sh.active;
     }
     FwdGroup g;
@@ -1708,7 +1747,9 @@
     g.n = n; g.bf16 = (flags & M3T_BF16) ? 1 : 0;
     for (int i = 0; i < n; ++i) { g.d[i].H = H; g.d[i].w_hh = reinterpret_cast<const float*>(16); }
     if (solo_fwd_ok(g, B, T, flags) || !level_shape(g.d, g.n, B, sh)) return 0;
-    if (fwd_uw(g, B, T, flags, sh) == 2 && !level_shape(g.d, g.n, B, sh, 2)) return 0;
+    const int uw = fwd_uw(g, B, T, flags, sh);
+    if (uw == 2 && !level_shape(g.d, g.n, B, sh, 2)) return 0;
+    fwd_spread(g, B, T, flags, uw, sh, false);
     return sh.active;
 }
 }
diff --git a/m3f.pytorch_amd/csrc/gru_persist_bwd3q_step.inc b/m3f.pytorch_amd/csrc/gru_persist_bwd3q_step.inc
--- a/m3f.pytorch_amd/csrc/gru_persist_bwd3q_step.inc
+++ b/m3f.pytorch_amd/csrc/gru_persist_bwd3q_step.inc
@@ -13,6 +13,13 @@
 #pragma unroll
             for (int m = 0; m < NP; ++m) {
                 const u32x4* q = src + (size_t)m * NW * 2 * TILE;
+                if (RB < ROWS)
+                    asm volatile("global_load_dwordx4 %0, %4, off sc1\n\t"
+                                 "global_load_dwordx4 %1, %4, off offset:1024 sc1\n\t"
+                                 "global_load_dwordx4 %2, %4, off offset:2048 sc1\n\t"
+                                 "global_load_dwordx4 %3, %4, off offset:3072 sc1"
+                                 : "=&v"(v[m][0]), "=&v"(v[m][2]), "=&v"(v[m][4]), "=&v"(v[m][6]) : "v"(q) : "memory");
+                else
                 asm volatile("global_load_dwordx4 %0, %8, off sc1\n\t"
                              "global_load_dwordx4 %1, %8, off offset:512 sc1\n\t"
                              "global_load_dwordx4 %2, %8, off offset:1024 sc1\n\t"
@@ -30,7 +37,7 @@
 #pragma unroll
             for (int m = 0; m < NP; ++m)
 #pragma unroll
-                for (int e = 0; e < 8; ++e) {
+                for (int e = 0; e < 8; e += (RB < ROWS ? 2 : 1)) {
                     asm volatile("" : "+v"(v[m][e]));
                     ok = ok && ((v[m][e].w & 0xffffffu) == tag);
                 }
@@ -44,6 +51,13 @@
         acc[0] = acc[1] = (f32x4){0.f, 0.f, 0.f, 0.f};
 #pragma unroll
         for (int m = 0; m < NP; ++m) {
+            if (RB < ROWS) {
+#pragma unroll
+                for (int e = 0; e < 8; e += 2)
+#pragma unroll
+                    for (int gt = 0; gt < 3; ++gt)
+                        v[m][e + 1][gt] = (unsigned)__builtin_amdgcn_update_dpp(0, (int)v[m][e][gt], 0x128, 0xf, 0xf, false);
+            }
             f32x4 at[2];
             at[0] = at[1] = (f32x4){0.f, 0.f, 0.f, 0.f};
 #pragma unroll
@@ -121,7 +135,7 @@
         }
         float psc, pisc;
         m3t_f16_scale(mxb, psc, pisc);
-        if (step + 1 < T && !(step == ex.fault_step && blockIdx.x == 0)) {
+        if (step + 1 < T && (RB == ROWS || plive) && !(step == ex.fault_step && blockIdx.x == 0)) {
             u32x4 gq;
             gq.x = bwd3p_split(p0 * psc); gq.y = bwd3p_split(p1 * psc); gq.z = bwd3p_split(p2 * psc);
             gq.w = ((ex.tag_base + (unsigned)step + 1u) & 0xffffffu) | ((__float_as_uint(psc) >> 23) << 24);
diff --git a/m3f.pytorch_amd/csrc/gru_persist_fwd6_step.inc b/m3f.pytorch_amd/csrc/gru_persist_fwd6_step.inc
--- a/m3f.pytorch_amd/csrc/gru_persist_fwd6_step.inc
+++ b/m3f.pytorch_amd/csrc/gru_persist_fwd6_step.inc
@@ -17,6 +17,11 @@
 #pragma unroll
                 for (int k = 0; k < KS; ++k) {
                     const unsigned long long* qp = src + (size_t)(2 * k) * NW * TILE;
+                    if (RB < ROWS)
+                        asm volatile("global_load_dwordx4 %0, %2, off sc1\n\t"
+                                     "global_load_dwordx4 %1, %2, off offset:1024 sc1"
+                                     : "=&v"(v[k][0]), "=&v"(v[k][2]) : "v"(qp) : "memory");
+                    else
                     asm volatile("global_load_dwordx4 %0, %4, off sc1\n\t"
                                  "global_load_dwordx4 %1, %4, off offset:512 sc1\n\t"
                                  "global_load_dwordx4 %2, %4, off offset:1024 sc1\n\t"
@@ -29,7 +34,7 @@
 #pragma unroll
                 for (int k = 0; k < KS; ++k)
 #pragma unroll
-                    for (int jp = 0; jp < 4; ++jp) {
+                    for (int jp = 0; jp < 4; jp += (RB < ROWS ? 2 : 1)) {
                         asm volatile("" : "+v"(v[k][jp]));
                         ok = ok && ((v[k][jp].y >> 16) == tag) && ((v[k][jp].w >> 16) == tag);
                     }
@@ -41,6 +46,15 @@
             M3T_STAMP(1);
             if (F16) {
                 pf16x8 F1[KS], F2[KS];
+                if (RB < ROWS) {
+#pragma unroll
+                    for (int k = 0; k < KS; ++k)
+#pragma unroll
+                        for (int jp = 0; jp < 4; jp += 2) {
+                            v[k][jp + 1].x = (unsigned)__builtin_amdgcn_update_dpp(0, (int)v[k][jp].x, 0x128, 0xf, 0xf, false);
+                            v[k][jp + 1].z = (unsigned)__builtin_amdgcn_update_dpp(0, (int)v[k][jp].z, 0x128, 0xf, 0xf, false);
+                        }
+                }
 #pragma unroll
                 for (int k = 0; k < KS; ++k) {
                     pu32x4 a1, a2;
@@ -143,7 +157,7 @@
             float c_xr = CUR(xr), c_xz = CUR(xz), c_xn = CUR(xn);
             if (CO) { const f32x4 x4 = sx[PARV * UW * SLOTS + slot_c]; c_xr = x4[0]; c_xz = x4[1]; c_xn = x4[2]; }
             const GateFwd c = gru_cell_fwd(c_xr, c_xz, c_xn, hr, hz, hn, hprev);
-            if (step + 1 < T && !(step == ex.fault_step && blockIdx.x == 0)) {
+            if (step + 1 < T && (RB == ROWS || plive) && !(step == ex.fault_step && blockIdx.x == 0)) {
                 const float hv = pok ? (g.bf16 ? rbf(c.h) : c.h) : 0.f;
                 unsigned long long gq;
                 if (F16) {
diff --git a/m3f.pytorch_amd/m3t/_lib.py b/m3f.pytorch_amd/m3t/_lib.py
--- a/m3f.pytorch_amd/m3t/_lib.py
+++ b/m3f.pytorch_amd/m3t/_lib.py
@@ -18,6 +18,7 @@
 M3T_SCAN_WHH = 8
 M3T_SCAN_FAULT = 16
 M3T_SCAN_WIDE = 32
+M3T_SCAN_SPREAD = 64
 M3T_MAX_SCANS = 8
 M3T_JPEG_TRUNC, M3T_JPEG_CODE, M3T_JPEG_RST, M3T_JPEG_EXTRA = 1, 2, 4, 8
 
diff --git a/m3f.pytorch_amd/m3t/ops.py b/m3f.pytorch_amd/m3t/ops.py
--- a/m3f.pytorch_amd/m3t/ops.py
+++ b/m3f.pytorch_amd/m3t/ops.py
@@ -679,6 +679,10 @@
 SCAN_FP32 = [False]
 
 
+SPREAD = [os.environ.get("M3T_SCAN_SPREAD", "1") != "0"]
+SPREAD_BWD0 = [os.environ.get("M3T_SCAN_SPREAD_BWD0", "1") != "0"]
+
+
 _FENCED = [False]
 
 
@@ -988,7 +992,7 @@
 
         alone = not _interleaved(groups) and all(kind == "main" for kind, _ in groups)
 
-        def level_fwd(l, idxs, scan, after=None, wide=False, progress=None):
+        def level_fwd(l, idxs, scan, after=None, wide=False, progress=None, spread=False):
             descs = []
             for s in idxs:
                 H = Hs[s]
@@ -1004,7 +1008,8 @@
                                                 _vp(gates[l][s], d * B * T * 4 * H), _vp(h_ns[s], (2 * l + d) * B * H),
                                                 H, d, 6 * H, d * 3 * H, outs[l][s].stride(1), d * H))
             if scan:
-                return _scan_fwd(descs, B, T, prec | (_lib.M3T_SCAN_WIDE if (wide or FORCE_WIDE_FWD[0]) else 0), after,
+                return _scan_fwd(descs, B, T, prec | (_lib.M3T_SCAN_WIDE if (wide or FORCE_WIDE_FWD[0]) else 0)
+                                 | (_lib.M3T_SCAN_SPREAD if spread else 0), after,
                                  None if progress is None else (_progress_counters(dev), progress))
 
         def chunk_plan(idxs, wide):
@@ -1125,7 +1130,8 @@
                     for l in range(L):
                         if l == 0 or tb is None:
                             level_fwd(l, idxs, False)
-                        need = level_fwd(l, idxs, True, progress=tb if l + 1 < L else None)
+                        need = level_fwd(l, idxs, True, progress=tb if l + 1 < L else None,
+                                         spread=SPREAD[0] and kind == "main" and alone and len(idxs) == 1)
                         if tb is not None and l + 1 < L:
                             proj_pieces(l + 1, idxs, tb, need, stream)
             for kind, _ in groups:
@@ -1327,7 +1333,7 @@
                     _wait_progress(ctr_, 1, need_[2])
             fn()
 
-        def level_scan(l, idxs, after=None, wide=False, progress=None):
+        def level_scan(l, idxs, after=None, wide=False, progress=None, spread=False):
             descs = []
             for s in idxs:
                 H = Hs[s]
@@ -1347,9 +1353,10 @@
                                             _vp(wfq[(l, s, d)]) if (l, s, d) in wfq else None))
             chain = _ws_tag(dev)
             sm = None
-            if progress is None and chain in held:
+            if progress is None and chain in held and not spread:
                 sm = start_marks(idxs)
-            need = _scan_bwd(descs, B, T, prec | (_lib.M3T_SCAN_WHH if direct_whh else 0) | _lib.M3T_SCAN_WIDE, after,
+            need = _scan_bwd(descs, B, T, prec | (_lib.M3T_SCAN_WHH if direct_whh else 0) | _lib.M3T_SCAN_WIDE
+                             | (_lib.M3T_SCAN_SPREAD if spread else 0), after,
                              None if (progress is None and sm is None) else (_progress_counters(dev), progress if progress is not None else sm))
             if progress is not None:
                 pending[(l, tuple(idxs))] = (progress, need)
@@ -1492,7 +1499,9 @@
                     stream.wait_stream(main)
                 with on_stream(stream):
                     for l in range(L - 1, -1, -1):
-                        level_scan(l, idxs, progress=chunk_plan(l, idxs) if (kind == "main" and len(groups) == 1) else None)
+                        level_scan(l, idxs, progress=chunk_plan(l, idxs) if (kind == "main" and len(groups) == 1) else None,
+                                   spread=(SPREAD[0] and kind == "main" and len(groups) == 1 and len(idxs) == 1
+                                           and (l == L - 1 or SPREAD_BWD0[0])))
                         level_gemms(l, idxs)
             for kind, _ in groups:
                 if kind == "side":
```

Result: faster. 2977 (median of 6 runs) (+4.9%).
